# Ascend-Research/HeadPoseEstimation-WHENet

Hardware: AMD Instinct MI355X
Metric: head crops/sec (224x224) (higher is better)
Workload: dtype f16

## Files before the change

headposeestimation-whenet_amd/csrc/capi.cpp:

```cpp
#include <algorithm>
#include <chrono>
#include <cstdio>
#include <cstring>
#include <fstream>
#include <memory>
#include <mutex>
#include <new>
#include <exception>
#include <string>
#include <thread>
#include <utility>
#include <vector>

#include "engine.h"
#include "engine_internal.h"

constexpr int MAX_INFLIGHT_ENGINES = 4;
struct whenet_ctx {
    whenet::Engine* engine = nullptr;
    std::vector<whenet::Engine*> replicas;
    std::vector<char> snapshot;
    int device_id = 0, dtype = WHENET_F32;
    int inflight = 1;
    size_t next = 0;
    int fanout_min = 256, fanout_chunk = 128, fanout_stage = 2, fanout_depth = 2;
    int fanout_calib_calls = 0;
    double fanout_calib_rate[2] = {0.0, 0.0};
    int fanout_chosen = -1;
    std::vector<whenet::Engine*> fan;
    int fanout_engines = 2;
    std::vector<std::pair<std::string, long>> options;
    whenet::Engine& at(size_t i) { return i == 0 ? *engine : *replicas[i - 1]; }
    whenet::Engine& fan_at(size_t i) {
        if (i == 0) return *engine;
        if (i - 1 < replicas.size()) return *replicas[i - 1];
        return *fan[i - 1 - replicas.size()];
    }
    int fan_count() {
        const int want = std::max(inflight, std::min(fanout_engines, 4));
        while (1 + int(replicas.size()) + int(fan.size()) < want) {
            std::unique_ptr<whenet::Engine> r(new whenet::Engine(snapshot.data(), snapshot.size(), device_id, dtype));
            for (const auto& kv : options) r->set_option(kv.first, kv.second);
            fan.push_back(r.release());
        }
        return want;
    }
    whenet::Engine& take() {
        whenet::Engine& e = at(next % size_t(inflight));
        next = (next + 1) % size_t(inflight);
        return e;
    }
};

namespace {

thread_local std::string g_create_error;

struct HostRegistry {
    std::mutex mu;
    std::vector<std::pair<uintptr_t, uintptr_t>> held;
    bool acquire(const void* p, size_t nbytes, hipError_t* err) {
        const uintptr_t page = 4096, lo = reinterpret_cast<uintptr_t>(p) & ~(page - 1),
                        hi = (reinterpret_cast<uintptr_t>(p) + nbytes + page - 1) & ~(page - 1);
        std::lock_guard<std::mutex> lock(mu);
        for (const auto& r : held)
            if (lo < r.second && r.first < hi) {
                *err = hipErrorUnknown;
                return false;
            }
        *err = hipHostRegister(const_cast<void*>(p), nbytes, hipHostRegisterDefault);
        if (*err != hipSuccess) {
            (void)hipGetLastError();
            return false;
        }
        held.emplace_back(lo, hi);
        return true;
    }
    void release(const void* p, size_t nbytes) {
        const uintptr_t page = 4096, lo = reinterpret_cast<uintptr_t>(p) & ~(page - 1),
                        hi = (reinterpret_cast<uintptr_t>(p) + nbytes + page - 1) & ~(page - 1);
        std::lock_guard<std::mutex> lock(mu);
        (void)hipHostUnregister(const_cast<void*>(p));
        for (size_t i = 0; i < held.size(); ++i)
            if (held[i].first == lo && held[i].second == hi) {
                held.erase(held.begin() + long(i));
                break;
            }
    }
};
HostRegistry g_host_registry;

template <typename F>
int guarded(whenet_t* h, F&& fn) {
    if (h == nullptr || h->engine == nullptr) return WHENET_EINVAL;
    try {
        fn(*h->engine);
        return WHENET_OK;
    } catch (const whenet::Error& e) {
        h->engine->last_error = e.what();
        return e.code;
    } catch (const std::bad_alloc&) {
        h->engine->last_error = "out of host memory";
        return WHENET_ENOMEM;
    } catch (const std::exception& e) {
        h->engine->last_error = e.what();
        return WHENET_EHIP;
    } catch (...) {
        h->engine->last_error = "unknown error";
        return WHENET_EHIP;
    }
}

int create_impl(const void* blob, size_t nbytes, int device_id, int dtype, whenet_t** out) {
    if (out == nullptr) return WHENET_EINVAL;
    *out = nullptr;
    try {
        std::unique_ptr<whenet::Engine> e(new whenet::Engine(blob, nbytes, device_id, dtype));
        whenet_t* h = new whenet_t;
        h->engine = e.release();
        h->snapshot.assign(static_cast<const char*>(blob), static_cast<const char*>(blob) + nbytes);
        h->device_id = device_id;
        h->dtype = dtype;
        *out = h;
        return WHENET_OK;
    } catch (const whenet::Error& e) {
        g_create_error = e.what();
        return e.code;
    } catch (const std::bad_alloc&) {
        g_create_error = "out of host memory";
        return WHENET_ENOMEM;
    } catch (const std::exception& e) {
        g_create_error = e.what();
        return WHENET_EHIP;
    } catch (...) {
        g_create_error = "unknown error";
        return WHENET_EHIP;
    }
}

}

extern "C" {
#pragma GCC visibility push(default)

int whenet_create(const char* snapshot_path, int device_id, int dtype, whenet_t** out) {
    if (snapshot_path == nullptr || out == nullptr) {
        g_create_error = "whenet_create: NULL argument";
        return WHENET_EINVAL;
    }
    std::vector<char> blob;
    try {
        std::ifstream f(snapshot_path, std::ios::binary | std::ios::ate);
        if (!f) {
            g_create_error = std::string("cannot open snapshot '") + snapshot_path + "'";
            return WHENET_ENOENT;
        }
        const std::streamoff sz = f.tellg();
        if (sz < 0 || !f.seekg(0) || uint64_t(sz) > (uint64_t(1) << 32)) {
            g_create_error = std::string("snapshot '") + snapshot_path + "' is not a readable regular file";
            return WHENET_EIO;
        }
        blob.resize(size_t(sz));
        if (sz > 0 && !f.read(blob.data(), std::streamsize(sz))) {
            g_create_error = std::string("cannot read snapshot '") + snapshot_path + "'";
            return WHENET_EIO;
        }
    } catch (const std::bad_alloc&) {
        g_create_error = "out of host memory";
        return WHENET_ENOMEM;
    } catch (const std::exception& e) {
        g_create_error = std::string("cannot read snapshot '") + snapshot_path + "': " + e.what();
        return WHENET_EIO;
    } catch (...) {
        g_create_error = std::string("cannot read snapshot '") + snapshot_path + "'";
        return WHENET_EIO;
    }
    return create_impl(blob.data(), blob.size(), device_id, dtype, out);
}

int whenet_create_from_memory(const void* snapshot, size_t nbytes, int device_id, int dtype, whenet_t** out) {
    if (snapshot == nullptr || out == nullptr) {
        g_create_error = "whenet_create_from_memory: NULL argument";
        return WHENET_EINVAL;
    }
    return create_impl(snapshot, nbytes, device_id, dtype, out);
}

int whenet_create_postproc(int device_id, whenet_t** out) {
    if (out == nullptr) {
        g_create_error = "whenet_create_postproc: NULL argument";
        return WHENET_EINVAL;
    }
    *out = nullptr;
    try {
        std::unique_ptr<whenet::Engine> e(new whenet::Engine(device_id));
        whenet_t* h = new whenet_t;
        h->engine = e.release();
        h->device_id = device_id;
        *out = h;
        return WHENET_OK;
    } catch (const whenet::Error& e) {
        g_create_error = e.what();
        return e.code;
    } catch (const std::bad_alloc&) {
        g_create_error = "out of host memory";
        return WHENET_ENOMEM;
    } catch (const std::exception& e) {
        g_create_error = e.what();
        return WHENET_EHIP;
    } catch (...) {
        g_create_error = "unknown error";
        return WHENET_EHIP;
    }
}

void whenet_destroy(whenet_t* h) {
    if (h == nullptr) return;
    try {
        for (whenet::Engine* e : h->replicas) delete e;
        for (whenet::Engine* e : h->fan) delete e;
        delete h->engine;
    } catch (...) {
    }
    delete h;
}

const char* whenet_last_error(const whenet_t* h) {
    if (h == nullptr || h->engine == nullptr) return g_create_error.c_str();
    return h->engine->last_error.c_str();
}

int whenet_get_info(const whenet_t* h, whenet_info_t* out) {
    if (h == nullptr || h->engine == nullptr || out == nullptr) return WHENET_EINVAL;
    h->engine->get_info(out);
    return WHENET_OK;
}

int whenet_set_option(whenet_t* h, const char* key, long value) {
    if (key == nullptr) return WHENET_EINVAL;
    return guarded(h, [&](whenet::Engine& e) {
        const std::string k = key;
        if (k == "inflight") {
            WHENET_REQUIRE(value >= 1 && value <= MAX_INFLIGHT_ENGINES, WHENET_EINVAL, "inflight must be 1..4");
            WHENET_REQUIRE(!h->snapshot.empty() || value == 1, WHENET_EINVAL, "inflight: this handle has no network");
            e.release_aux_streams();
            for (whenet::Engine* r : h->replicas) r->release_aux_streams();
            for (whenet::Engine* r : h->fan) delete r;
            h->fan.clear();
            while (int(h->replicas.size()) + 1 > value) {
                delete h->replicas.back();
                h->replicas.pop_back();
            }
            while (int(h->replicas.size()) + 1 < value) {
                std::unique_ptr<whenet::Engine> r(
                    new whenet::Engine(h->snapshot.data(), h->snapshot.size(), h->device_id, h->dtype));
                for (const auto& kv : h->options) r->set_option(kv.first, kv.second);
                h->replicas.push_back(r.release());
            }
            h->inflight = int(value);
            h->next = 0;
            const long lanes = value > 1 ? 1 : 2;
            e.set_option("device_lanes", lanes);
            for (whenet::Engine* r : h->replicas) r->set_option("device_lanes", lanes);
            e.set_option("concurrent", value > 1);
            for (whenet::Engine* r : h->replicas) r->set_option("concurrent", value > 1);
            return;
        }
        if (k == "fanout_min" || k == "fanout_chunk" || k == "fanout_stage" || k == "fanout_depth" || k == "fanout_engines") {
            if (k == "fanout_engines") {
                WHENET_REQUIRE(value >= 1 && value <= MAX_INFLIGHT_ENGINES, WHENET_EINVAL, "fanout_engines must be 1..4");
                h->fanout_engines = int(value);
                for (whenet::Engine* r : h->fan) delete r;
                h->fan.clear();
                return;
            }
            if (k == "fanout_min") {
                WHENET_REQUIRE(value >= 0, WHENET_EINVAL, "fanout_min must be >= 0 (0 = never)");
                h->fanout_min = int(std::min<long>(value, 1 << 30));
            } else if (k == "fanout_chunk") {
                WHENET_REQUIRE(value >= 1 && value <= 4096, WHENET_EINVAL, "fanout_chunk must be 1..4096");
                h->fanout_chunk = int(value);
            } else if (k == "fanout_stage") {
                WHENET_REQUIRE(value >= -1 && value <= 3, WHENET_EINVAL,
                               "fanout_stage must be -1 (calibrate 0 against 1), 0 (pinned staging), 1 (the runtime's pageable path) or 2 (registered, default)");
                h->fanout_stage = int(value);
                h->fanout_calib_calls = 0;
                h->fanout_calib_rate[0] = h->fanout_calib_rate[1] = 0.0;
            } else {
                WHENET_REQUIRE(value >= 1 && value <= WHENET_MAX_INFLIGHT, WHENET_EINVAL, "fanout_depth must be 1..4");
                h->fanout_depth = int(value);
            }
            return;
        }
        e.set_option(k, value);
        for (whenet::Engine* r : h->replicas) r->set_option(k, value);
        for (whenet::Engine* r : h->fan) r->set_option(k, value);
        h->options.emplace_back(k, value);
    });
}

int whenet_forward_u8(whenet_t* h, const uint8_t* crops, int n, float* ypr, int32_t* argmax, float* logits) {
    return guarded(h, [&](whenet::Engine& e) {
        bool pending = e.has_pending();
        for (whenet::Engine* r : h->replicas) pending = pending || r->has_pending();
        if (h->fanout_min <= 0 || n < h->fanout_min || n <= h->fanout_chunk || pending || h->snapshot.empty()) {
            e.forward_host(crops, n, ypr, argmax, logits);
            return;
        }
        WHENET_REQUIRE(crops != nullptr && ypr != nullptr, WHENET_EINVAL, "crops and ypr must not be NULL");
        const int chunk = h->fanout_chunk;
        int stage = h->fanout_stage;
        const bool calibrating = stage < 0;
        if (calibrating)
            stage = h->fanout_calib_calls < 6 ? 1 - (h->fanout_calib_calls & 1) : (h->fanout_calib_rate[1] >= h->fanout_calib_rate[0] ? 1 : 0);
        const auto t_start = std::chrono::steady_clock::now();
        const int nfan = h->fan_count();
        const int lanes = nfan > 1 ? 1 : 2;
        if (stage == 2 || stage == 3) {
            const bool shared_copy_stream = stage == 2;
            whenet::detail::DeviceGuard guard(h->device_id);
            const size_t nbytes = size_t(n) * 150528;
            hipError_t re = hipSuccess;
            const bool registered = g_host_registry.acquire(crops, nbytes, &re);
            if (registered || re == hipErrorHostMemoryAlreadyRegistered) {
                h->fanout_chosen = stage;
                struct Pending { int eng, ticket, off; };
                std::vector<Pending> q;
                size_t head = 0;
                std::vector<int> outstanding(size_t(nfan), 0);
                const hipStream_t copy_on = shared_copy_stream ? h->engine->copy_stream_handle() : nullptr;
                hipEvent_t prev = nullptr;
                auto collect_head = [&] {
                    const Pending& p = q[head++];
                    const size_t o = size_t(p.off);
                    h->fan_at(size_t(p.eng)).collect(p.ticket, ypr + o * 3, argmax ? argmax + o * 3 : nullptr, logits ? logits + o * 252 : nullptr);
                    --outstanding[size_t(p.eng)];
                };
                std::exception_ptr err;
                try {
                    int off = 0, c = 0;
                    while (off < n) {
                        const int want = c < 2 && chunk >= 32 ? chunk / 2 : chunk;
                        const int cnt = std::min(want, n - off), ei = c % nfan;
                        while (outstanding[size_t(ei)] >= h->fanout_depth) collect_head();
                        whenet::Engine& eng = h->fan_at(size_t(ei));
                        const int ticket = eng.submit(crops + size_t(off) * 150528, cnt, 1, lanes, copy_on, shared_copy_stream ? nullptr : prev);
                        if (!shared_copy_stream) prev = eng.copied_event(ticket);
                        q.push_back(Pending{ei, ticket, off});
                        ++outstanding[size_t(ei)];
                        off += cnt;
                        ++c;
                    }
                    while (head < q.size()) collect_head();
                } catch (...) {
                    err = std::current_exception();
                    for (int i = 0; i < nfan; ++i) {
                        try { h->fan_at(size_t(i)).abandon_submissions(); } catch (...) {}
                    }
                }
                if (registered) g_host_registry.release(crops, nbytes);
                if (err) std::rethrow_exception(err);
                return;
            }
            stage = 1;
        }
        h->fanout_chosen = stage;
        const int nthreads = nfan;
        const int nchunks = (n + chunk - 1) / chunk;
        std::vector<std::exception_ptr> errs;
        errs.resize(static_cast<size_t>(nthreads));
        auto drive = [&](int t) {
            whenet::Engine& eng = h->fan_at(size_t(t));
            struct Pending { int ticket, off; };
            std::vector<Pending> q;
            size_t head = 0;
            auto collect_one = [&] {
                const Pending& p = q[head++];
                const size_t o = size_t(p.off);
                eng.collect(p.ticket, ypr + o * 3, argmax ? argmax + o * 3 : nullptr, logits ? logits + o * 252 : nullptr);
            };
            try {
                for (int c = t; c < nchunks; c += nthreads) {
                    if (q.size() - head >= size_t(h->fanout_depth)) collect_one();
                    const int off = c * chunk, cnt = std::min(chunk, n - off);
                    q.push_back(Pending{eng.submit(crops + size_t(off) * 150528, cnt, stage, lanes), off});
                }
                while (head < q.size()) collect_one();
            } catch (...) {
                errs[size_t(t)] = std::current_exception();
                try {
                    eng.abandon_submissions();
                } catch (...) {
                }
            }
        };
        std::vector<std::thread> workers;
        workers.reserve(size_t(nthreads));
        int started = 1;
        try {
            for (int t = 1; t < nthreads; ++t, ++started) workers.emplace_back(drive, t);
        } catch (...) {
        }
        drive(0);
        for (int t = started; t < nthreads; ++t) drive(t);
        for (std::thread& w : workers) w.join();
        for (const std::exception_ptr& ep : errs)
            if (ep) std::rethrow_exception(ep);
        if (calibrating && h->fanout_calib_calls < 6) {
            if (h->fanout_calib_calls >= 2) {
                const double sec = std::chrono::duration<double>(std::chrono::steady_clock::now() - t_start).count();
                h->fanout_calib_rate[stage] = std::max(h->fanout_calib_rate[stage], double(n) / (sec > 0 ? sec : 1e-9));
            }
            ++h->fanout_calib_calls;
        }
    });
}

int whenet_forward_f32(whenet_t* h, const float* image, int n, float* ypr, int32_t* argmax, float* logits) {
    return guarded(h, [&](whenet::Engine& e) { e.forward_host_f32(image, n, ypr, argmax, logits); });
}

int whenet_forward_u8_device(whenet_t* h, const uint8_t* d_crops, int n, float* d_ypr, int32_t* d_argmax,
                             float* d_logits, void* stream) {
    return guarded(h, [&](whenet::Engine& e) {
        whenet::Engine& eng = (stream != nullptr) ? e : h->take();
        eng.forward_device(d_crops, n, d_ypr, d_argmax, d_logits, static_cast<hipStream_t>(stream));
    });
}

int whenet_sync(whenet_t* h) {
    return guarded(h, [&](whenet::Engine& e) {
        e.sync();
        for (whenet::Engine* r : h->replicas) r->sync();
        for (whenet::Engine* r : h->fan) r->sync();
    });
}

int whenet_submit_u8(whenet_t* h, const uint8_t* crops, int n, int* ticket) {
    if (ticket == nullptr) return WHENET_EINVAL;
    return guarded(h, [&](whenet::Engine&) {
        const size_t idx = h->next % size_t(h->inflight);
        *ticket = h->take().submit(crops, n) * MAX_INFLIGHT_ENGINES + int(idx);
    });
}

int whenet_frame_rects(int frame_h, int frame_w, const float* bboxes, int k, int32_t* rects) {
    if (frame_h <= 0 || frame_w <= 0 || k < 0 || (k > 0 && (bboxes == nullptr || rects == nullptr))) return WHENET_EINVAL;
    for (int i = 0; i < k; ++i) whenet::frame_box_rect(frame_h, frame_w, bboxes + 4 * i, rects + 4 * i);
    return WHENET_OK;
}

int whenet_normalise_table(float lut[768]) {
    if (lut == nullptr) return WHENET_EINVAL;
    whenet::normalise_table(reinterpret_cast<float (*)[256]>(lut));
    return WHENET_OK;
}

int whenet_submit_frame(whenet_t* h, const uint8_t* frame, int frame_h, int frame_w, int channel_order,
                        const int32_t* rects, int k, int* ticket) {
    if (ticket == nullptr || (channel_order != WHENET_RGB && channel_order != WHENET_BGR)) return WHENET_EINVAL;
    return guarded(h, [&](whenet::Engine&) {
        const size_t idx = h->next % size_t(h->inflight);
        *ticket = h->take().submit_frame(frame, frame_h, frame_w, channel_order == WHENET_BGR, rects, k) *
                      MAX_INFLIGHT_ENGINES + int(idx);
    });
}

int whenet_op_crop_resize(whenet_t* h, const uint8_t* frame, int frame_h, int frame_w, int channel_order,
                          const int32_t* rects, int k, uint8_t* crops) {
    if (channel_order != WHENET_RGB && channel_order != WHENET_BGR) return WHENET_EINVAL;
    return guarded(h, [&](whenet::Engine& e) {
        e.op_crop_resize(frame, frame_h, frame_w, channel_order == WHENET_BGR, rects, k, crops);
    });
}

int whenet_yolo_eval(whenet_t* h, const float* const* feats, const int* grid_h, const int* grid_w, int num_layers,
                     const float* anchors, int num_anchors, int num_classes, float image_h, float image_w,
                     float score_threshold, float iou_threshold, int max_boxes, float* boxes, float* scores,
                     int32_t* classes, int32_t* index, int* count, float* all_boxes, float* all_scores) {
    if (count == nullptr) return WHENET_EINVAL;
    return guarded(h, [&](whenet::Engine& e) {
        *count = e.yolo_eval(feats, grid_h, grid_w, num_layers, anchors, num_anchors, num_classes, image_h, image_w,
                             score_threshold, iou_threshold, max_boxes, boxes, scores, classes, index, all_boxes,
                             all_scores);
    });
}

int whenet_collect(whenet_t* h, int ticket, float* ypr, int32_t* argmax, float* logits) {
    return guarded(h, [&](whenet::Engine&) {
        const int idx = ticket % MAX_INFLIGHT_ENGINES;
        WHENET_REQUIRE(ticket >= 0 && idx < h->inflight, WHENET_EINVAL, "unknown ticket " + std::to_string(ticket));
        h->at(size_t(idx)).collect(ticket / MAX_INFLIGHT_ENGINES, ypr, argmax, logits);
    });
}

int whenet_profile(whenet_t* h, const uint8_t* d_crops, int n, int iters, whenet_launch_stat_t* stats, int cap,
                   int* count) {
    return guarded(h, [&](whenet::Engine& e) {
        for (whenet::Engine* r : h->replicas) r->sync();
        const int c = e.profile(d_crops, n, iters, stats, cap);
        if (count) *count = c;
    });
}

int whenet_op_stem(whenet_t* h, const uint8_t* crops, int n, float* out) {
    return guarded(h, [&](whenet::Engine& e) { e.op_stem(crops, n, out); });
}

int whenet_op_block(whenet_t* h, int index, const float* in, int n, float* expand_out, float* dw_out, float* gate,
                    float* out) {
    return guarded(h, [&](whenet::Engine& e) { e.op_block(index, in, n, expand_out, dw_out, gate, out); });
}

int whenet_op_block_range(whenet_t* h, int first, int last, const float* in, int n, float* out) {
    return guarded(h, [&](whenet::Engine& e) { e.op_block_range(first, last, in, n, out); });
}

int whenet_op_head(whenet_t* h, const float* in, int n, float* feat, float* logits, float* ypr, int32_t* argmax) {
    return guarded(h, [&](whenet::Engine& e) { e.op_head(in, n, feat, logits, ypr, argmax); });
}

int whenet_op_decode(whenet_t* h, const float* logits, int n, float* ypr, int32_t* argmax) {
    return guarded(h, [&](whenet::Engine& e) { e.op_decode(logits, n, ypr, argmax); });
}

int whenet_block_spec(int index, int32_t out[8]) {
    if (out == nullptr) return WHENET_EINVAL;
    try {
        const auto blocks = whenet::make_blocks();
        if (index < 1 || index > int(blocks.size())) return WHENET_EINVAL;
        const whenet::BlockSpec& b = blocks[size_t(index - 1)];
        const int32_t v[8] = {b.k, b.s, b.expand, b.cin, b.cout, b.h_in, b.h_out, b.se_reduced()};
        std::memcpy(out, v, sizeof(v));
        return WHENET_OK;
    } catch (...) {
        return WHENET_ENOMEM;
    }
}

int whenet_dw_plan(int dtype, int index, int32_t out[12]) {
    if (out == nullptr || (dtype != WHENET_F32 && dtype != WHENET_F16)) return WHENET_EINVAL;
    try {
        const auto blocks = whenet::make_blocks();
        if (index < 1 || index > int(blocks.size())) return WHENET_EINVAL;
        const whenet::BlockSpec& b = blocks[size_t(index - 1)];
        const whenet::DwPlan p = whenet::plan_dw(dtype, b.k, b.s, b.h_in, b.h_out, b.cexp());
        const int32_t v[12] = {p.threads, p.CV, p.TH, p.NSX, p.tiles_x, p.tiles_y, p.chunks, p.IH, p.IW,
                               int32_t(p.lds_bytes), b.pad_before(), b.cexp()};
        std::memcpy(out, v, sizeof(v));
        return WHENET_OK;
    } catch (...) {
        return WHENET_EINVAL;
    }
}

int whenet_front_plan(int dtype, int index, int32_t out[12]) {
    if (out == nullptr || (dtype != WHENET_F32 && dtype != WHENET_F16)) return WHENET_EINVAL;
    try {
        const auto blocks = whenet::make_blocks();
        if (index < 2 || index > int(blocks.size())) return WHENET_EINVAL;
        const whenet::BlockSpec& b = blocks[size_t(index - 1)];
        const whenet::FrontPlan p = whenet::plan_front(dtype, b.k, b.s, b.h_in, b.h_out, b.cexp());
        const int32_t v[12] = {p.threads, p.CC, p.TH, p.NSX, p.tiles_x, p.tiles_y, p.chunks, p.EH, p.EW,
                               int32_t(p.lds_bytes), p.w_off, b.cexp()};
        std::memcpy(out, v, sizeof(v));
        return WHENET_OK;
    } catch (...) {
        return WHENET_EINVAL;
    }
}

int whenet_device_alloc(whenet_t* h, size_t nbytes, void** d_ptr) {
    if (d_ptr == nullptr) return WHENET_EINVAL;
    return guarded(h, [&](whenet::Engine& e) { *d_ptr = e.dev_alloc(nbytes); });
}

int whenet_device_free(whenet_t* h, void* d_ptr) {
    return guarded(h, [&](whenet::Engine& e) { e.dev_free(d_ptr); });
}

int whenet_memcpy_h2d(whenet_t* h, void* d_dst, const void* src, size_t nbytes) {
    return guarded(h, [&](whenet::Engine& e) { e.h2d(d_dst, src, nbytes); });
}

int whenet_memcpy_d2h(whenet_t* h, void* dst, const void* d_src, size_t nbytes) {
    return guarded(h, [&](whenet::Engine& e) { e.d2h(dst, d_src, nbytes); });
}
// ... 4 lines not shown
```

headposeestimation-whenet_amd/csrc/engine.cpp:

```cpp
#include "engine_internal.h"

#include <mutex>

#include <algorithm>
#include <cstdlib>
#include <cmath>
#include <cstring>

namespace whenet {

using namespace detail;

void* Engine::upload_bytes(const void* p, size_t nbytes) {
    void* d = nullptr;
    WHENET_HIP_CHECK(hipMalloc(&d, nbytes ? nbytes : 16));
    weight_allocs_.push_back(d);
    if (nbytes) WHENET_HIP_CHECK(hipMemcpy(d, p, nbytes, hipMemcpyHostToDevice));
    return d;
}

template <typename T> T* Engine::upload(const std::vector<T>& v) {
    return static_cast<T*>(upload_bytes(v.data(), v.size() * sizeof(T)));
}

DevPw Engine::upload_pw(const HostPw& h) {
    DevPw d;
    d.K = h.K;
    d.N = h.N;
    d.KS = h.KS;
    d.NTILES = h.NTILES;
    d.wp = upload_bytes(h.packed.data(), h.packed.size());
    if (!h.packed_split.empty()) {
        d.wps = upload_bytes(h.packed_split.data(), h.packed_split.size());
        d.KSs = h.KS_split;
        d.wsi = h.wsi;
    }
    d.wdense = upload(h.dense);
    d.bias = upload(h.bias);
    return d;
}

Engine::Engine(const void* snapshot, size_t nbytes, int device_id, int dtype)
    : device_(device_id), dtype_(dtype == WHENET_F32S ? WHENET_F32 : dtype), split_(dtype == WHENET_F32S) {
    HostModel m = build_host_model(parse_snapshot(snapshot, nbytes), dtype_, split_);
    params_backbone_ = m.params_backbone;
    params_heads_ = m.params_heads;
    n_tensors_ = m.n_tensors;

    open_device(device_id);
    DeviceGuard guard(device_);
    has_model_ = true;

    d_lut_ = static_cast<float*>(upload_bytes(&m.lut[0][0], sizeof(m.lut)));
    d_stem_w_ = upload(m.stem_w);
    d_stem_b_ = upload(m.stem_b);
    {
        StemDwTable t;
        build_stemdw_table(m.stem_w.data(), &m.lut[0][0], &t);
        d_stemdw_tab_ = static_cast<StemDwTable*>(upload_bytes(&t, sizeof(t)));
    }
    for (const HostBlock& hb : m.blocks) {
        DevBlock b;
        b.spec = hb.spec;
        if (hb.spec.has_expand()) b.expand = upload_pw(hb.expand);
        b.dw.k = hb.dw.k;
        b.dw.C = hb.dw.C;
        b.dw.w = upload(hb.dw.w);
        b.dw.bias = upload(hb.dw.bias);
        b.dw.plan = plan_dw(dtype_, hb.spec.k, hb.spec.s, hb.spec.h_in, hb.spec.h_out, hb.dw.C);
        b.se.C = hb.se.C;
        b.se.R = hb.se.R;
        b.se.w1t = upload(hb.se.w1t);
        b.se.b1 = upload(hb.se.b1);
        b.se.w2 = upload(hb.se.w2);
        b.se.w2c = upload(hb.se.w2c);
        b.se.b2 = upload(hb.se.b2);
        if (split_ && !hb.se.excite.packed_split.empty()) {
            b.se.w2p = upload_bytes(hb.se.excite.packed_split.data(), hb.se.excite.packed_split.size());
            b.se.KSr = hb.se.excite.KS_split;
            b.se.w2_wsi = hb.se.excite.wsi;
        } else if (dtype_ == WHENET_F16 && !hb.se.excite.packed.empty()) {
            b.se.w2p = upload_bytes(hb.se.excite.packed.data(), hb.se.excite.packed.size());
            b.se.KSr = hb.se.excite.KS;
        }
        b.project = upload_pw(hb.project);
        partial_per_crop_ = std::max(partial_per_crop_, size_t(b.dw.plan.ntiles()) * b.dw.C);
        if (hb.spec.has_expand()) {
            b.fplan = plan_front(dtype_, hb.spec.k, hb.spec.s, hb.spec.h_in, hb.spec.h_out, hb.dw.C);
            partial_per_crop_ = std::max(partial_per_crop_, size_t(b.fplan.ntiles()) * b.dw.C);
            partial_per_crop_ = std::max(partial_per_crop_, size_t(b.fplan.ntiles()) * size_t(b.fplan.chunks) *
                                                                size_t(se_padded_r(b.se.R)));
            if (dtype_ == WHENET_F16) {
                b.f2plan = plan_front2(hb.spec.k, hb.spec.s, hb.spec.h_in, hb.spec.h_out, hb.dw.C);
                b.f2_preferred = front2_preferred(hb.spec.k, hb.spec.s, hb.spec.h_in, hb.dw.C);
                b.dw.wt = upload(pack_dw_toeplitz(hb.dw.w, hb.spec.k, hb.spec.s, hb.dw.C, b.f2plan.xs));
                partial_per_crop_ = std::max(partial_per_crop_, size_t(b.f2plan.ntiles()) * b.dw.C);
                partial_per_crop_ = std::max(partial_per_crop_, size_t(b.f2plan.ntiles()) * size_t(b.f2plan.chunks) *
                                                                    size_t(se_padded_r(b.se.R)));
            }
            if (split_ && front2s_supported(hb.spec.k, hb.spec.s, hb.spec.h_in, hb.spec.cin)) {
                b.f2s_supported = true;
                b.f2splan = plan_front2s(hb.spec.k, hb.spec.s, hb.spec.h_in, hb.spec.h_out, hb.dw.C, &b.f2s_tm);
                b.f2s_preferred = front2s_preferred(hb.spec.k, hb.spec.s, hb.spec.h_in, hb.dw.C);
                b.dw.wts = upload(pack_dw_toeplitz_s(hb.dw.w, hb.spec.k, hb.spec.s, hb.dw.C, b.f2s_tm, &b.dw.wts_wsi));
                partial_per_crop_ = std::max(partial_per_crop_, size_t(b.f2splan.ntiles()) * size_t(b.f2splan.chunks) *
                                                                    size_t(se_padded_r(b.se.R)));
            }
            b.f7_supported = front7_supported(hb.spec.k, hb.spec.s, hb.spec.h_in, hb.spec.cin);
            if (b.f7_supported) {
                if (dtype_ == WHENET_F16) b.dw.wt7 = upload(pack_dw_toeplitz(hb.dw.w, hb.spec.k, 1, hb.dw.C, 4 - hb.spec.k / 2));
                b.f7_chunks = front7_plan_for(dtype_, hb.spec.cin, hb.dw.C, 64).chunks;
                partial_per_crop_ = std::max(partial_per_crop_, size_t(b.f7_chunks) * size_t(se_padded_r(b.se.R)));
            }
        }
        if (mb7_supported(dtype_, hb.spec.k, hb.spec.s, hb.spec.h_in, hb.spec.cin, hb.dw.C, hb.se.R, hb.spec.cout, hb.spec.has_skip())) {
            std::vector<half_t> w1p, w2p;
            pack_mb7_se(hb.se.w1t, hb.se.w2, hb.se.C, hb.se.R, &w1p, &w2p);
            b.mb7.wds = upload(pack_mb7_taps(hb.dw.w, hb.spec.k, hb.dw.C));
            b.mb7.w1p = upload(w1p);
            b.mb7.w2p = upload(w2p);
            b.mb7.ok = true;
        }
        blocks_.push_back(b);
    }
    head_ = upload_pw(m.head);
    fold12_pw_ = upload_pw(m.fold12);
    d_fold12_w32_ = upload(m.fold12_w32);
    d_dense_w_ = upload(m.dense_w);
    d_dense_b_ = upload(m.dense_b);
    WHENET_HIP_CHECK(hipDeviceSynchronize());
}

void Engine::open_device(int device_id) {
    int count = 0;
    hipError_t e = hipGetDeviceCount(&count);
    if (e != hipSuccess || count <= 0)
        throw Error(WHENET_ENODEV, std::string("no HIP device visible (") + hipGetErrorString(e) +
                                       "); libwhenet_hip has no CPU fallback");
    WHENET_REQUIRE(device_id >= 0 && device_id < count, WHENET_ENODEV,
                   "device_id " + std::to_string(device_id) + " out of range (" + std::to_string(count) + " devices)");
    DeviceGuard guard(device_id);
    WHENET_HIP_CHECK(hipGetDeviceProperties(&prop_, device_id));
    WHENET_REQUIRE(std::strstr(prop_.gcnArchName, "gfx950") != nullptr, WHENET_ENODEV,
                   std::string("device is ") + prop_.gcnArchName + "; this library carries gfx950 code only");
    num_cus_ = prop_.multiProcessorCount;

    WHENET_HIP_CHECK(hipStreamCreateWithFlags(&stream_, hipStreamNonBlocking));
    WHENET_HIP_CHECK(hipEventCreateWithFlags(&fork_ev_, hipEventDisableTiming));
    for (int i = 0; i < MAX_LANES - 1; ++i) {
        hipEvent_t ev = nullptr;
        WHENET_HIP_CHECK(hipEventCreateWithFlags(&ev, hipEventDisableTiming));
        join_ev_.push_back(ev);
    }
}

Engine::Engine(int device_id) : device_(device_id), dtype_(WHENET_F32) { open_device(device_id); }

void Engine::require_model() const {
    WHENET_REQUIRE(has_model_, WHENET_EINVAL, "this handle was created without a network (whenet_create_postproc)");
}

Engine::~Engine() {
    (void)hipSetDevice(device_);
    if (stream_) (void)hipStreamSynchronize(stream_);
    if (copy_stream_) (void)hipStreamSynchronize(copy_stream_);
    for (auto& kv : graphs_) (void)hipGraphExecDestroy(kv.second);
    graphs_.clear();
    auto free_slot_buffers = [](Slot& s) {
        if (s.h_in) (void)hipHostFree(s.h_in);
        if (s.h_ypr) (void)hipHostFree(s.h_ypr);
        if (s.h_amax) (void)hipHostFree(s.h_amax);
        if (s.h_logits) (void)hipHostFree(s.h_logits);
        if (s.d_in) (void)hipFree(s.d_in);
        if (s.d_ypr) (void)hipFree(s.d_ypr);
        if (s.d_amax) (void)hipFree(s.d_amax);
        if (s.d_logits) (void)hipFree(s.d_logits);
        if (s.h_frame) (void)hipHostFree(s.h_frame);
        if (s.d_frame) (void)hipFree(s.d_frame);
        if (s.h_plan) (void)hipHostFree(s.h_plan);
        if (s.d_plan) (void)hipFree(s.d_plan);
        if (s.copied) (void)hipEventDestroy(s.copied);
        if (s.done) (void)hipEventDestroy(s.done);
    };
    for (Slot& s : slots_) free_slot_buffers(s);
    free_slot_buffers(host_slot_);
    if (hout_ypr_) (void)hipHostFree(hout_ypr_);
    if (hout_amax_) (void)hipHostFree(hout_amax_);
    if (hout_logits_) (void)hipHostFree(hout_logits_);
    void* arena[] = {x0_, x1_, e_, d_, hc_, partial_, gate_, hcount_, in_u8_, o_ypr_, o_amax_, o_logits_, in_f32_, yolo_scratch_};
    for (void* p : arena)
        if (p) (void)hipFree(p);
    for (void* p : weight_allocs_) (void)hipFree(p);
    for (hipStream_t st : lane_streams_) { (void)hipStreamSynchronize(st); (void)hipStreamDestroy(st); }
    for (hipEvent_t ev : join_ev_) (void)hipEventDestroy(ev);
    if (fork_ev_) (void)hipEventDestroy(fork_ev_);
    if (stream_) (void)hipStreamDestroy(stream_);
    if (copy_stream_) (void)hipStreamDestroy(copy_stream_);
}

void Engine::set_option(const std::string& key, long value) {
    DeviceGuard guard(device_);
    if (key == "graph") {
        use_graph_ = value != 0;
    } else if (key == "pw_impl") {
        WHENET_REQUIRE(value == 0 || value == 1, WHENET_EINVAL, "pw_impl must be 0 (MFMA) or 1 (check kernel)");
        pw_impl_ = int(value);
        sync();
        drop_graphs();
    } else if (key == "fuse_front") {
        fuse_front_ = value != 0;
        sync();
        drop_graphs();
    } else if (key == "se_fuse") {
        WHENET_REQUIRE(value >= 0 && value <= 3, WHENET_EINVAL,
                       "se_fuse must be 0 (never), 1 (where the prologue form pays), 2 (prologue form on every block) or 3 (1 + the matrix-core form on blocks 7-16, default)");
        se_fuse_ = int(value);
        sync();
        drop_graphs();
    } else if (key == "front_impl") {
        WHENET_REQUIRE(value >= 0 && value <= 2, WHENET_EINVAL,
                       "front_impl must be 0 (front.hip everywhere), 1 (per layer, default) or 2 (front2.hip / front2s.hip wherever they exist)");
        front_impl_ = int(value);
        sync();
        drop_graphs();
    } else if (key == "f2s_mask") {
        WHENET_REQUIRE(value >= -1 && value < (1 << 17), WHENET_EINVAL, "f2s_mask must be -1 or a bit mask of blocks 2..12");
        f2s_mask_ = int(value);
        sync();
        drop_graphs();
    } else if (key == "head_fuse") {
        head_fuse_ = value != 0;
        sync();
        drop_graphs();
    } else if (key == "concurrent") {
        xcd_always_ = value != 0;
        sync();
        drop_graphs();
    } else if (key == "xcd_map") {
        WHENET_REQUIRE(value >= 0 && value <= 7, WHENET_EINVAL, "xcd_map must be a bit mask 0..7 (1 = front / front2, 2 = front7, 4 = head7)");
        xcd_map_ = int(value);
        sync();
        drop_graphs();
    } else if (key == "mb7") {
        mb7_ = value != 0;
        sync();
        drop_graphs();
    } else if (key == "front7") {
        front7_ = value != 0;
        sync();
        drop_graphs();
    } else if (key == "fold12") {
        fold12_ = value != 0;
        sync();
        drop_graphs();
    } else if (key == "stem_fuse") {
        stem_fuse_ = value != 0;
        sync();
        drop_graphs();
    } else if (key == "poison") {
        poison_ = value != 0;
    } else if (key == "lanes" || key == "device_lanes") {
        WHENET_REQUIRE(value >= 1 && value <= MAX_LANES, WHENET_EINVAL, "lanes must be 1..8");
        lanes_ = int(value);
        if (key == "lanes") host_lanes_ = int(value);
        sync();
        drop_graphs();
    } else if (key == "split_heads") {
        split_heads_ = value != 0;
        sync();
        drop_graphs();
    } else if (key == "lane_graphs") {
        lane_graphs_ = value != 0;
        sync();
        drop_graphs();
    } else if (key == "pw_staged") {
        pw_staged_ = value != 0;
        sync();
        drop_graphs();
    } else if (key == "split_pw") {
        WHENET_REQUIRE(split_ || value == 0, WHENET_EINVAL, "split_pw: the handle was not created as WHENET_F32S");
        split_pw_ = value != 0;
        sync();
        drop_graphs();
    } else if (key == "host_pinned_max") {
        WHENET_REQUIRE(value >= 0 && value <= 4096, WHENET_EINVAL, "host_pinned_max must be 0..4096");
        sync();
        host_pinned_max_ = int(value);
    } else if (key == "se_fuse_tiny") {
        WHENET_REQUIRE(value >= 0 && value <= 64, WHENET_EINVAL, "se_fuse_tiny must be 0..64");
        se_fuse_tiny_ = int(value);
        sync();
        drop_graphs();
    } else if (key == "host_lanes") {
        WHENET_REQUIRE(value >= 1 && value <= MAX_LANES, WHENET_EINVAL, "host_lanes must be 1..8");
        host_lanes_ = int(value);
    } else if (key == "min_lane_crops") {
        WHENET_REQUIRE(value >= 1, WHENET_EINVAL, "min_lane_crops must be >= 1");
        min_lane_crops_ = int(value);
        sync();
        drop_graphs();
    } else if (key == "repeat") {
        WHENET_REQUIRE(value >= 1 && value <= 16, WHENET_EINVAL, "repeat must be 1..16");
        repeat_ = int(value);
        sync();
        drop_graphs();
    } else {
        throw Error(WHENET_EINVAL, "unknown option '" + key + "'");
    }
}

void Engine::get_info(whenet_info_t* out) const {
    std::memset(out, 0, sizeof(*out));
    out->abi_version = WHENET_ABI_VERSION;
    out->dtype = dtype_;
    out->device_id = device_;
    out->compute_units = num_cus_;
    out->params_backbone = params_backbone_;
    out->params_heads = params_heads_;
    out->n_tensors = n_tensors_;
    {
        int k = 1 + 2;
        for (const DevBlock& b : blocks_) {
            const BlockSchedule bs = block_schedule(b);
            if (bs.use_mb7) { k += 1; continue; }
            k += bs.fused ? 1 : (b.spec.has_expand() ? 2 : 1);
            k += bs.se_fused ? 1 : 2;
        }
        if (fold12_active()) k -= 1;
        if (stem_fuse_active()) k -= 1;
        out->n_kernels_per_forward = k;
    }
    out->macs_per_crop = 384857312;
    out->arena_bytes = int64_t(arena_bytes_);
    out->capacity = cap_;
    out->graph_enabled = use_graph_ ? 1 : 0;
    copy_name(out->device_name, sizeof(out->device_name), prop_.name);
    copy_name(out->arch, sizeof(out->arch), prop_.gcnArchName);
}

void Engine::drop_graphs() {
    for (auto& kv : graphs_) (void)hipGraphExecDestroy(kv.second);
    graphs_.clear();
}

void Engine::release_arena() {
    void** arena[] = {&x0_, &x1_, &e_, &d_, &hc_, reinterpret_cast<void**>(&partial_), reinterpret_cast<void**>(&gate_), reinterpret_cast<void**>(&hcount_),
                      reinterpret_cast<void**>(&in_u8_), reinterpret_cast<void**>(&o_ypr_),
                      reinterpret_cast<void**>(&o_amax_), reinterpret_cast<void**>(&o_logits_)};
    for (void** p : arena) {
        if (*p) (void)hipFree(*p);
        *p = nullptr;
    }
    cap_ = 0;
    arena_bytes_ = 0;
}

void Engine::ensure_capacity(int n) {
    WHENET_REQUIRE(n >= 1, WHENET_EINVAL, "n must be >= 1");
    if (n <= cap_) return;
    WHENET_HIP_CHECK(hipStreamSynchronize(stream_));
    drop_graphs();
    release_arena();
    const size_t N = size_t(n), es = esz();
    size_t total = 0;
    auto alloc = [&](size_t bytes) {
        void* p = nullptr;
        hipError_t e = hipMalloc(&p, bytes);
        if (e != hipSuccess) {
            release_arena();
            throw Error(WHENET_ENOMEM, "activation arena for n=" + std::to_string(n) + ": " + hipGetErrorString(e));
        }
        total += bytes;
        return p;
    };
    x0_ = alloc(N * X_ELEMS * es);
    x1_ = alloc(N * X_ELEMS * es);
    e_ = alloc(N * E_ELEMS * es);
    d_ = alloc(N * D_ELEMS * es);
    hc_ = alloc(N * HC_ELEMS * es);
    partial_ = static_cast<float*>(alloc(N * partial_per_crop_ * sizeof(float)));
    gate_ = static_cast<float*>(alloc(N * 1152 * sizeof(float)));
    hcount_ = static_cast<unsigned*>(alloc(N * sizeof(unsigned)));
    WHENET_HIP_CHECK(hipMemsetAsync(hcount_, 0, N * sizeof(unsigned), stream_));
    WHENET_HIP_CHECK(hipStreamSynchronize(stream_));
    in_u8_ = static_cast<uint8_t*>(alloc(N * IN_BYTES));
    o_ypr_ = static_cast<float*>(alloc(N * 3 * sizeof(float)));
    o_amax_ = static_cast<int32_t*>(alloc(N * 3 * sizeof(int32_t)));
    o_logits_ = static_cast<float*>(alloc(N * N_LOGITS * sizeof(float)));
    cap_ = n;
    arena_bytes_ = total;
}

namespace {

struct Rec {
    LaunchRecorder* rec;
    hipStream_t s;
    int repeat = 1;
    template <typename F>
    void operator()(const std::string& layer, const char* kind, const std::string& kernel, double bytes, double flops,
                    F&& fn) {
        if (!rec) {
            for (int i = 0; i < repeat; ++i) fn();
            return;
        }
        if (rec->first_pass) {
            LaunchRecorder::Entry e;
            e.layer = layer;
            e.kind = kind;
            e.kernel = kernel;
            e.bytes = bytes;
            e.flops = flops;
            WHENET_HIP_CHECK(hipEventCreate(&e.stop));
            rec->entries.push_back(e);
        }
        LaunchRecorder::Entry& e = rec->entries.at(rec->cursor++);
        fn();
        WHENET_HIP_CHECK(hipEventRecord(e.stop, s));
    }
};

}

Engine::BlockSchedule Engine::block_schedule(const DevBlock& b, int n) const {
    BlockSchedule r;
    r.fused = fuse_front_ && b.spec.has_expand() && pw_impl_ == 0;
    r.use_f7 = r.fused && front_impl_ == 1 && front7_ && b.f7_supported;
    r.use_mb7 = r.use_f7 && mb7_ && dtype_ == WHENET_F16 && b.mb7.ok;
    r.use_f2 = r.fused && !r.use_f7 && dtype_ == WHENET_F16 && (front_impl_ == 2 || (front_impl_ == 1 && b.f2_preferred));
    const bool f2s_pick = f2s_mask_ >= 0 ? ((f2s_mask_ >> b.spec.index) & 1) != 0 : b.f2s_preferred;
    r.use_f2s = r.fused && !r.use_f7 && split_ && split_pw_ && b.f2s_supported && b.expand.wps != nullptr &&
                (front_impl_ == 2 || (front_impl_ == 1 && f2s_pick));
    r.se_in_front = r.fused;
    r.se_ntiles = r.use_f7 ? 1 : (r.use_f2 ? b.f2plan.ntiles() : (r.use_f2s ? b.f2splan.ntiles() : (r.fused ? b.fplan.ntiles() : b.dw.plan.ntiles())));
    r.se_chunks = r.use_f7 ? b.f7_chunks : (r.use_f2 ? b.f2plan.chunks : (r.use_f2s ? b.f2splan.chunks : b.fplan.chunks));
    const bool se_pays = b.project.K < 320 && r.se_ntiles * r.se_chunks <= 24;
    const bool tiny = !single_stage_call_ && n > 0 && n <= se_fuse_tiny_ && b.project.K < 1152;
    r.se_mfma = r.se_in_front && pw_impl_ == 0 && se_fuse_ == 3 && pw_staged_ && b.project.K >= 320 && b.se.w2p != nullptr &&
                (dtype_ == WHENET_F16 || (split_ && split_pw_));
    r.se_fused = r.se_in_front && pw_impl_ == 0 && (se_fuse_ == 2 || r.se_mfma || ((se_fuse_ == 1 || se_fuse_ == 3) && (se_pays || tiny)));
    return r;
}

bool Engine::fold12_active() const {
    if (!(fold12_ && fuse_front_ && pw_impl_ == 0 && blocks_.size() >= 2)) return false;
    if (dtype_ == WHENET_F16) return front_impl_ == 2 || (front_impl_ == 1 && blocks_[1].f2_preferred);
    const BlockSchedule b2 = block_schedule(blocks_[1]);
    return split_ && split_pw_ && fold12_pw_.wps != nullptr && b2.fused && !b2.use_f2s && !b2.use_f7;
}

bool Engine::stem_fuse_active() const {
    if (!(stem_fuse_ && !blocks_.empty())) return false;
    const DevBlock& b = blocks_[0];
    return !b.spec.has_expand() && !b.spec.has_skip() &&
           stemdw_supported(dtype_, b.dw.plan, b.spec.k, b.spec.s, b.spec.h_in, b.spec.cexp());
}

void* Engine::enqueue_blocks(int first, int last, const View& v, void* cur, int n, hipStream_t s, LaunchRecorder* rec,
                             bool b1_dw_done) {
    const bool fold = fold12_active() && first <= 1 && last >= 2;
    for (int i = first; i <= last; ++i) {
        void* nxt = (cur == v.x0) ? v.x1 : v.x0;
        enqueue_block(blocks_[size_t(i - 1)], v, cur, nxt, n, s, rec, fold && i <= 2 ? i : 0, b1_dw_done && i == 1);
        cur = nxt;
    }
    return cur;
}

void Engine::enqueue_block(const DevBlock& b, const View& v, const void* in, void* out, int n, hipStream_t s,
                           LaunchRecorder* rec, int fold, bool dw_done) {
    Rec R{rec, s, repeat_};
    const BlockSpec& sp = b.spec;
    const std::string p = "b" + std::to_string(sp.index);
    const double es = double(esz());
    const int hw_in = sp.h_in * sp.h_in, hw_out = sp.h_out * sp.h_out;
    const int cexp = sp.cexp();
    const void* dw_in = in;
    const BlockSchedule bs = block_schedule(b, n);
    const bool fused = bs.fused, use_f2 = bs.use_f2, se_in_front = bs.se_in_front, se_fused = bs.se_fused;
    const int se_ntiles = bs.se_ntiles, se_chunks = bs.se_chunks;
    WHENET_REQUIRE(fold == 0 || (fold == 1 && !fused && sp.index == 1) ||
                       (fold == 2 && sp.index == 2 && (use_f2 || (split_ && fused && !bs.use_f2s && !bs.use_f7))), WHENET_EINVAL,
                   "fold12: block outside the folded pair");
    if (bs.use_mb7) {
        WHENET_REQUIRE(fold == 0, WHENET_EINVAL, "mb7: block outside the 7 x 7 stage");
        Mb7Args a{};
        a.x = in;
        a.wep = b.expand.wp;
        a.be = b.expand.bias;
        a.wds = b.mb7.wds;
        a.bd = b.dw.bias;
        a.w1p = b.mb7.w1p;
        a.b1 = b.se.b1;
        a.w2p = b.mb7.w2p;
        a.b2 = b.se.b2;
        a.wpp = b.project.wp;
        a.bp = b.project.bias;
        a.out = out;
        if (single_stage_call_) {
            a.dbg_dw = v.d;
            a.dbg_gate = v.gate;
        }
        a.k = sp.k;
        a.Cout = sp.cout;
        a.skip = sp.has_skip();
        a.n = n;
        R(p + "/mbconv", "mbconv", kernel_name_mb7(sp.k, sp.cout, a.skip).c_str(),
          double(n) * (hw_in * sp.cin * (a.skip ? 2 : 1) + hw_out * sp.cout) * es,
          2.0 * n * (double(hw_in) * sp.cin * cexp + double(hw_out) * sp.k * sp.k * cexp + double(hw_out) * cexp * sp.cout),
          [&] { launch_mb7(a, s); });
        return;
    }
    if (bs.use_f7) {
        Front7Args a{};
        a.dtype = dtype_;
        a.x = in;
        a.wep = b.expand.wp;
        a.be = b.expand.bias;
        a.wdt = dtype_ == WHENET_F16 ? static_cast<const void*>(b.dw.wt7) : static_cast<const void*>(b.dw.w);
        a.bd = b.dw.bias;
        a.out = v.d;
        a.rpart = v.partial;
        a.w1t = b.se.w1t;
        a.R = b.se.R;
        a.k = sp.k;
        a.Cin = sp.cin;
        a.Cexp = cexp;
        a.NTe = b.expand.NTILES;
        a.split = split_ && split_pw_ && b.expand.wps != nullptr;
        a.weps = b.expand.wps;
        a.wsi = b.expand.wsi;
        a.n = n;
        a.xcd_grouped = xcd_grouped(2, n);
        a.plan = front7_plan_for(dtype_, sp.cin, cexp, n);
        R(p + "/front", "front", kernel_name_front7(dtype_, sp.k, a.plan, a.split).c_str(), double(n) * (hw_in * sp.cin + hw_out * cexp) * es,
          2.0 * n * (double(hw_in) * sp.cin * cexp + double(hw_out) * sp.k * sp.k * cexp), [&] { launch_front7(a, s); });
    } else if (use_f2) {
        Front2Args a{};
        a.x = in;
        a.wep = b.expand.wp;
        a.be = b.expand.bias;
        a.wdt = b.dw.wt;
        a.bd = b.dw.bias;
        a.out = v.d;
        a.rpart = v.partial;
        a.w1t = b.se.w1t;
        a.R = b.se.R;
        a.k = sp.k;
        a.s = sp.s;
        a.H = sp.h_in;
        a.Ho = sp.h_out;
        a.Cin = sp.cin;
        a.Cexp = cexp;
        a.pad = sp.pad_before();
        a.KSe = b.expand.KS;
        a.NTe = b.expand.NTILES;
        if (fold == 2) {
            a.wep = d_fold12_w32_;
            a.be = fold12_pw_.bias;
            a.Cin = fold12_pw_.K;
            a.KSe = fold12_pw_.KS;
            a.NTe = fold12_pw_.NTILES;
            a.in_gate = static_cast<const float*>(v.gate);
        }
        a.n = n;
        a.xcd_grouped = xcd_grouped(1, n);
        a.plan = b.f2plan;
        a.plan.threads = front2_threads(b.f2plan, n);
        R(p + "/front", "front", kernel_name_front2(sp.k, sp.s, a.KSe, a.plan.threads, a.plan.xs, a.in_gate != nullptr).c_str(),
          double(n) * (hw_in * a.Cin + hw_out * cexp) * es,
          2.0 * n * (double(hw_in) * a.Cin * cexp + double(hw_out) * sp.k * sp.k * cexp), [&] { launch_front2(a, s); });
    } else if (bs.use_f2s) {
        Front2sArgs a{};
        a.x = in;
        a.weps = b.expand.wps;
        a.be = b.expand.bias;
        a.wdt = b.dw.wts;
        a.bd = b.dw.bias;
        a.out = v.d;
        a.rpart = v.partial;
        a.w1t = b.se.w1t;
        a.R = b.se.R;
        a.k = sp.k;
        a.s = sp.s;
        a.H = sp.h_in;
        a.Ho = sp.h_out;
        a.Cin = sp.cin;
        a.Cexp = cexp;
        a.pad = sp.pad_before();
        a.KSe = b.expand.KSs;
        a.NTe = b.expand.NTILES;
        a.wsi = b.expand.wsi;
        a.wsi_d = b.dw.wts_wsi;
        a.tm = b.f2s_tm;
        a.n = n;
        a.plan = b.f2splan;
        R(p + "/front", "front", kernel_name_front2s(sp.k, sp.s, a.KSe, a.plan.threads, a.tm, false).c_str(),
          double(n) * (hw_in * sp.cin + hw_out * cexp) * es,
          2.0 * n * (double(hw_in) * sp.cin * cexp + double(hw_out) * sp.k * sp.k * cexp), [&] { launch_front2s(a, s); });
    } else if (fused) {
        FrontArgs a{};
        a.x = in;
        a.wep = b.expand.wp;
        a.be = b.expand.bias;
        a.wd = b.dw.w;
        a.bd = b.dw.bias;
        a.out = v.d;
        a.rpart = v.partial;
        a.w1t = b.se.w1t;
        a.R = b.se.R;
        a.k = sp.k;
        a.s = sp.s;
        a.H = sp.h_in;
        a.Ho = sp.h_out;
        a.Cin = sp.cin;
        a.Cexp = cexp;
        a.pad = sp.pad_before();
        a.KSe = b.expand.KS;
        a.NTe = b.expand.NTILES;
        a.split = split_ && split_pw_ && b.expand.wps != nullptr;
        a.weps = b.expand.wps;
        a.KSes = b.expand.KSs;
        a.wsi = b.expand.wsi;
        if (fold == 2) {
            a.weps = fold12_pw_.wps;
            a.be = fold12_pw_.bias;
            a.Cin = fold12_pw_.K;
            a.KSe = fold12_pw_.KS;
            a.KSes = fold12_pw_.KSs;
            a.NTe = fold12_pw_.NTILES;
            a.wsi = fold12_pw_.wsi;
            a.in_gate = static_cast<const float*>(v.gate);
        }
        a.n = n;
        a.xcd_grouped = xcd_grouped(1, n);
        a.plan = b.fplan;
        a.plan.threads = front_threads(b.fplan, n);
        R(p + "/front", "front", kernel_name_front(dtype_, sp.k, sp.s, a.plan.threads).c_str(), double(n) * (hw_in * a.Cin + hw_out * cexp) * es,
          2.0 * n * (double(hw_in) * a.Cin * cexp + double(hw_out) * sp.k * sp.k * cexp),
          [&] { launch_front(a, dtype_, s); });
    } else if (sp.has_expand()) {
        PwArgs a{};
        a.a = in;
        a.wp = b.expand.wp;
        a.wdense = b.expand.wdense;
        a.bias = b.expand.bias;
        a.out = v.e;
        a.M = n * hw_in;
        a.K = b.expand.K;
        a.N = b.expand.N;
        a.KS = b.expand.KS;
        a.NTILES = b.expand.NTILES;
        set_split(a, b.expand);
        a.HW = hw_in;
        a.act = ACT_SWISH;
        R(p + "/expand", "pw", kernel_name_pw(a, dtype_, pw_impl_, num_cus_).c_str(), double(a.M) * (a.K + a.N) * es,
          2.0 * a.M * a.K * a.N, [&] { launch_pw(a, dtype_, pw_impl_, num_cus_, s); });
        dw_in = v.e;
    }
    if (!fused && !dw_done) {
        DwArgs a{};
        a.in = dw_in;
        a.out = fold == 1 ? out : v.d;
        a.w = b.dw.w;
        a.bias = b.dw.bias;
        a.partial = v.partial;
        a.k = sp.k;
        a.s = sp.s;
        a.H = sp.h_in;
        a.Ho = sp.h_out;
        a.C = cexp;
        a.pad = sp.pad_before();
        a.n = n;
        a.plan = b.dw.plan;
        R(p + "/dw", "dw", kernel_name_dw(dtype_, sp.k, sp.s), double(n) * (hw_in + hw_out) * cexp * es,
          2.0 * n * hw_out * sp.k * sp.k * cexp, [&] { launch_dw(a, dtype_, s); });
    }
    SeFuse sef{};
    if (se_fused) {
        sef.rpart = v.partial;
        sef.b1 = b.se.b1;
        sef.w2c = b.se.w2c;
        sef.b2 = b.se.b2;
        sef.np = se_ntiles * se_chunks;
        sef.R = b.se.R;
        sef.RP = se_padded_r(b.se.R);
        sef.inv_hw = 1.0f / float(hw_out);
        if (bs.se_mfma) {
            sef.w2p = b.se.w2p;
            sef.KSr = b.se.KSr;
            sef.w2_wsi = b.se.w2_wsi;
        }
    } else if (se_in_front) {
        SeExciteArgs a{};
        a.rpart = v.partial;
        a.np = se_ntiles * se_chunks;
        a.inv_hw = 1.0f / float(hw_out);
        a.b1 = b.se.b1;
        a.w2c = b.se.w2c;
        a.b2 = b.se.b2;
        a.gate = v.gate;
        a.gate_f16 = dtype_ == WHENET_F16;
        a.C = b.se.C;
        a.R = b.se.R;
        a.n = n;
        R(p + "/se", "se", ("whenet_se_excite_kernel<" + std::to_string(se_padded_r(a.R)) + ">").c_str(),
          double(n) * (a.np * se_padded_r(a.R) + a.C) * 4.0 + double(a.C) * se_padded_r(a.R) * 4.0, 2.0 * n * a.C * a.R,
          [&] { launch_se_excite(a, s); });
    } else {
        SeArgs a{};
        a.partial = v.partial;
        a.ntiles = se_ntiles;
        a.inv_hw = 1.0f / float(hw_out);
        a.w1t = b.se.w1t;
        a.b1 = b.se.b1;
        a.w2c = b.se.w2c;
        a.b2 = b.se.b2;
        a.gate = v.gate;
        a.gate_f16 = dtype_ == WHENET_F16 && fold != 1;
        a.C = b.se.C;
        a.R = b.se.R;
        a.n = n;
        R(p + "/se", "se", ("whenet_se_kernel<" + std::to_string(se_padded_r(a.R)) + ">").c_str(), double(n) * (a.ntiles + 1) * a.C * 4.0 + 2.0 * a.C * a.R * 4.0,
          4.0 * n * a.C * a.R, [&] { launch_se(a, s); });
    }
    if (fold != 1) {
        PwArgs a{};
        a.a = v.d;
        a.wp = b.project.wp;
        a.wdense = b.project.wdense;
        a.bias = b.project.bias;
        a.gate = se_fused ? nullptr : v.gate;
        a.se = sef;
        a.res = sp.has_skip() ? in : nullptr;
        a.out = out;
        a.M = n * hw_out;
        a.K = b.project.K;
        a.N = b.project.N;
        a.KS = b.project.KS;
        a.NTILES = b.project.NTILES;
        set_split(a, b.project);
        a.HW = hw_out;
        a.act = ACT_NONE;
        R(p + "/project", "pw", kernel_name_pw(a, dtype_, pw_impl_, num_cus_).c_str(),
          double(a.M) * (a.K + a.N + (sp.has_skip() ? a.N : 0)) * es, 2.0 * a.M * a.K * a.N,
          [&] { launch_pw(a, dtype_, pw_impl_, num_cus_, s); });
    }
}

void Engine::enqueue_forward(const View& v, const uint8_t* d_in, int n, float* d_ypr, int32_t* d_amax, float* d_logits,
                             hipStream_t s, LaunchRecorder* rec, const float* d_in_f32) {
    Rec R{rec, s, repeat_};
    const double es = double(esz());
    const bool stemdw = stem_fuse_active() && d_in_f32 == nullptr;
    if (stemdw) {
        const DevBlock& b1 = blocks_[0];
        const bool fold = fold12_active() && blocks_.size() >= 2;
        StemDwArgs a{};
        a.dtype = dtype_;
        a.w = d_stem_w_;
        a.lut = d_lut_;
        a.in = d_in;
        a.out = fold ? v.x1 : v.d;
        a.tab = d_stemdw_tab_;
        a.bias = d_stem_b_;
        a.wd = b1.dw.w;
        a.bd = b1.dw.bias;
        a.partial = v.partial;
        a.n = n;
        R("stem+b1/dw", "stem", kernel_name_stemdw(dtype_), double(n) * (IN_BYTES + X_ELEMS * es), 2.0 * n * (10838016.0 + 112.0 * 112 * 9 * 32),
          [&] { launch_stemdw(a, s); });
    } else {
        StemArgs a{d_in, v.x0, d_stem_w_, d_stem_b_, d_lut_, n};
        a.in_f32 = d_in_f32;
        R("stem", "stem", kernel_name_stem(dtype_), double(n) * (IN_BYTES + X_ELEMS * es), 2.0 * n * 10838016.0,
          [&] { launch_stem(a, dtype_, s); });
    }
    void* cur = enqueue_blocks(1, int(blocks_.size()), v, v.x0, n, s, rec, stemdw);
    const bool fuse_head = head_fuse_ && pw_impl_ == 0 && split_heads_ && head7_supported(dtype_, head_.K, head_.N, 49) &&
                           partial_per_crop_ >= size_t(heads_split()) * N_LOGITS;
    if (fuse_head) {
        Head7Args a{};
        a.dtype = dtype_;
        a.x = cur;
        a.wep = head_.wp;
        a.bias = head_.bias;
        a.feat = reinterpret_cast<float*>(v.hc);
        a.K = head_.K;
        a.N = head_.N;
        a.NTILES = head_.NTILES;
        a.split = split_ && split_pw_ && head_.wps != nullptr;
        a.weps = head_.wps;
        a.wsi = head_.wsi;
        a.n = n;
        a.xcd_grouped = xcd_grouped(4, n);
        R("head", "pw", kernel_name_head7(dtype_, n, a.split).c_str(), double(n) * (49.0 * a.K * es + a.N * 4.0), 2.0 * n * 49.0 * a.K * a.N,
          [&] { launch_head7(a, s); });
        HeadsArgs hargs{};
        hargs.feat_in = reinterpret_cast<const float*>(v.hc);
        hargs.w = d_dense_w_;
        hargs.b = d_dense_b_;
        hargs.logits = d_logits;
        hargs.ypr = d_ypr;
        hargs.argmax = d_amax;
        hargs.n = n;
        R("heads", "heads", "whenet_heads_split_kernel<float, true>", double(n) * ((FEAT + N_LOGITS + 6) * 4.0) + double(FEAT) * N_LOGITS * 4.0,
          2.0 * n * FEAT * N_LOGITS, [&] { launch_heads_split(hargs, v.partial, v.hcount, dtype_, s); });
        return;
    }
    {
        PwArgs a{};
        a.a = cur;
        a.wp = head_.wp;
        a.wdense = head_.wdense;
        a.bias = head_.bias;
        a.out = v.hc;
        a.M = n * 49;
        a.K = head_.K;
        a.N = head_.N;
        a.KS = head_.KS;
        a.NTILES = head_.NTILES;
        set_split(a, head_);
        a.HW = 49;
        a.act = ACT_SWISH;
        R("head", "pw", kernel_name_pw(a, dtype_, pw_impl_, num_cus_).c_str(), double(a.M) * (a.K + a.N) * es,
          2.0 * a.M * a.K * a.N, [&] { launch_pw(a, dtype_, pw_impl_, num_cus_, s); });
    }
    {
        HeadsArgs a{};
        a.x = v.hc;
        a.w = d_dense_w_;
        a.b = d_dense_b_;
        a.logits = d_logits;
        a.ypr = d_ypr;
        a.argmax = d_amax;
        a.n = n;
        const bool split = split_heads_ && partial_per_crop_ >= size_t(heads_split()) * N_LOGITS;
        const std::string hname = std::string(split ? "whenet_heads_split_kernel<" : "whenet_heads_kernel<") +
                                  (dtype_ == WHENET_F16 ? "_Float16" : "float") + (split ? ", false>" : ">");
        R("heads", "heads", hname.c_str(),
          double(n) * (HC_ELEMS * es + (N_LOGITS + 6) * 4.0) + double(FEAT) * N_LOGITS * 4.0, 2.0 * n * FEAT * N_LOGITS,
          [&] {
              if (split) launch_heads_split(a, v.partial, v.hcount, dtype_, s);
              else launch_heads(a, dtype_, s);
          });
    }
}

hipStream_t Engine::lane_stream(int i) {
    while (int(lane_streams_.size()) <= i) {
        hipStream_t st = nullptr;
        WHENET_HIP_CHECK(hipStreamCreateWithFlags(&st, hipStreamNonBlocking));
        lane_streams_.push_back(st);
    }
    return lane_streams_[size_t(i)];
}

void Engine::release_aux_streams() {
    DeviceGuard guard(device_);
    sync();
    drop_graphs();
    for (hipStream_t st : lane_streams_) (void)hipStreamDestroy(st);
    lane_streams_.clear();
    if (copy_stream_) (void)hipStreamDestroy(copy_stream_);
    copy_stream_ = nullptr;
}

hipStream_t Engine::copy_stream() {
    if (!copy_stream_) WHENET_HIP_CHECK(hipStreamCreateWithFlags(&copy_stream_, hipStreamNonBlocking));
    return copy_stream_;
}

Engine::View Engine::view(int crop_off) const {
    const size_t o = size_t(crop_off), es = esz();
    View v;
    v.x0 = static_cast<char*>(x0_) + o * X_ELEMS * es;
    v.x1 = static_cast<char*>(x1_) + o * X_ELEMS * es;
    v.e = static_cast<char*>(e_) + o * E_ELEMS * es;
    v.d = static_cast<char*>(d_) + o * D_ELEMS * es;
    v.hc = static_cast<char*>(hc_) + o * HC_ELEMS * es;
    v.partial = partial_ + o * partial_per_crop_;
    v.hcount = hcount_ + o;
    v.gate = gate_ + o * 1152;
    return v;
}

int Engine::lanes_for(int n, int want) const {
    int lanes = want > 0 ? std::min(want, MAX_LANES) : lanes_;
    while (lanes > 1 && n / lanes < min_lane_crops_) --lanes;
    return lanes;
}

void Engine::enqueue_lanes(const uint8_t* d_in, int n, float* d_ypr, int32_t* d_amax, float* d_logits, hipStream_t s, int want) {
    const int lanes = lanes_for(n, want);
    if (lanes <= 1) {
        enqueue_forward(view(0), d_in, n, d_ypr, d_amax, d_logits, s, nullptr);
        return;
    }
    WHENET_HIP_CHECK(hipEventRecord(fork_ev_, s));
    int off = 0;
    for (int i = 0; i < lanes; ++i) {
        const int cnt = n / lanes + (i < n % lanes ? 1 : 0);
        hipStream_t st = (i == 0) ? s : lane_stream(i - 1);
        if (i > 0) WHENET_HIP_CHECK(hipStreamWaitEvent(st, fork_ev_, 0));
        enqueue_forward(view(off), d_in + size_t(off) * IN_BYTES, cnt, d_ypr + size_t(off) * 3,
                        d_amax ? d_amax + size_t(off) * 3 : nullptr, d_logits ? d_logits + size_t(off) * N_LOGITS : nullptr,
                        st, nullptr);
        if (i > 0) {
            WHENET_HIP_CHECK(hipEventRecord(join_ev_[size_t(i - 1)], st));
            WHENET_HIP_CHECK(hipStreamWaitEvent(s, join_ev_[size_t(i - 1)], 0));
        }
        off += cnt;
    }
}

template <typename F>
hipGraphExec_t Engine::cached_graph(const GraphKey& key, hipStream_t s, F&& fn) {
    auto it = graphs_.find(key);
    if (it != graphs_.end()) return it->second;
    if (graphs_.size() >= size_t(MAX_GRAPHS)) {
        sync_streams(s);
        WHENET_HIP_CHECK(hipStreamSynchronize(stream_));
        drop_graphs();
    }
    hipGraph_t graph = nullptr;
    WHENET_HIP_CHECK(hipStreamBeginCapture(s, hipStreamCaptureModeRelaxed));
    try {
        fn();
    } catch (...) {
        (void)hipStreamEndCapture(s, &graph);
        if (graph) (void)hipGraphDestroy(graph);
        throw;
    }
    WHENET_HIP_CHECK(hipStreamEndCapture(s, &graph));
    hipGraphExec_t exec = nullptr;
    hipError_t e = hipGraphInstantiate(&exec, graph, nullptr, nullptr, 0);
    (void)hipGraphDestroy(graph);
    if (e != hipSuccess) throw Error(WHENET_EHIP, std::string("hipGraphInstantiate: ") + hipGetErrorString(e));
    graphs_.emplace(key, exec);
    return exec;
}

void Engine::poison_arena(int n, hipStream_t s) {
    const size_t N = size_t(n), es = esz();
    WHENET_HIP_CHECK(hipMemsetAsync(x0_, 0xff, N * X_ELEMS * es, s));
    WHENET_HIP_CHECK(hipMemsetAsync(x1_, 0xff, N * X_ELEMS * es, s));
    WHENET_HIP_CHECK(hipMemsetAsync(e_, 0xff, N * E_ELEMS * es, s));
    WHENET_HIP_CHECK(hipMemsetAsync(d_, 0xff, N * D_ELEMS * es, s));
    WHENET_HIP_CHECK(hipMemsetAsync(hc_, 0xff, N * HC_ELEMS * es, s));
    WHENET_HIP_CHECK(hipMemsetAsync(partial_, 0xff, N * partial_per_crop_ * sizeof(float), s));
    WHENET_HIP_CHECK(hipMemsetAsync(gate_, 0xff, N * 1152 * sizeof(float), s));
}

void Engine::run_forward(const uint8_t* d_in, int n, float* d_ypr, int32_t* d_amax, float* d_logits, hipStream_t s, int want) {
    if (poison_) poison_arena(n, s);
    if (!use_graph_) {
        enqueue_lanes(d_in, n, d_ypr, d_amax, d_logits, s, want);
        return;
    }
    const int lanes = lanes_for(n, want);
    if (lanes > 1) (void)lane_stream(lanes - 2);
    if (lane_graphs_ && lanes > 1) {
        WHENET_HIP_CHECK(hipEventRecord(fork_ev_, s));
        int off = 0;
        for (int i = 0; i < lanes; ++i) {
            const int cnt = n / lanes + (i < n % lanes ? 1 : 0);
            hipStream_t st = (i == 0) ? s : lane_stream(i - 1);
            const uint8_t* in_i = d_in + size_t(off) * IN_BYTES;
            float* ypr_i = d_ypr + size_t(off) * 3;
            int32_t* am_i = d_amax ? d_amax + size_t(off) * 3 : nullptr;
            float* lg_i = d_logits ? d_logits + size_t(off) * N_LOGITS : nullptr;
            hipGraphExec_t g = cached_graph(GraphKey{cnt, off, in_i, ypr_i, am_i, lg_i}, st, [&] {
                enqueue_forward(view(off), in_i, cnt, ypr_i, am_i, lg_i, st, nullptr);
            });
            if (i > 0) WHENET_HIP_CHECK(hipStreamWaitEvent(st, fork_ev_, 0));
            WHENET_HIP_CHECK(hipGraphLaunch(g, st));
            if (i > 0) {
                WHENET_HIP_CHECK(hipEventRecord(join_ev_[size_t(i - 1)], st));
                WHENET_HIP_CHECK(hipStreamWaitEvent(s, join_ev_[size_t(i - 1)], 0));
            }
            off += cnt;
        }
        return;
    }
    hipGraphExec_t g = cached_graph(GraphKey{n, -lanes, d_in, d_ypr, d_amax, d_logits}, s,
                                    [&] { enqueue_lanes(d_in, n, d_ypr, d_amax, d_logits, s, lanes); });
    WHENET_HIP_CHECK(hipGraphLaunch(g, s));
}

void Engine::forward_device(const uint8_t* d_crops, int n, float* d_ypr, int32_t* d_argmax, float* d_logits,
                            hipStream_t stream) {
    DeviceGuard guard(device_);
    require_model();
    WHENET_REQUIRE(d_crops != nullptr && d_ypr != nullptr, WHENET_EINVAL, "crops and ypr must not be NULL");
    WHENET_REQUIRE((reinterpret_cast<uintptr_t>(d_crops) & 3) == 0, WHENET_EINVAL, "crops must be 4-byte aligned");
    ensure_capacity(n);
    run_forward(d_crops, n, d_ypr, d_argmax, d_logits, stream ? stream : stream_);
}

void Engine::forward_host(const uint8_t* crops, int n, float* ypr, int32_t* argmax, float* logits) {
    DeviceGuard guard(device_);
    require_model();
    WHENET_REQUIRE(crops != nullptr && ypr != nullptr, WHENET_EINVAL, "crops and ypr must not be NULL");
    ensure_capacity(n);
    const size_t N = size_t(n);
    if (n <= host_pinned_max_) {
        Slot& sl = host_slot_;
        ensure_slot(sl, std::max(n, std::min(host_pinned_max_, 16)));
        std::memcpy(sl.h_in, crops, N * IN_BYTES);
        WHENET_HIP_CHECK(hipMemcpyAsync(sl.d_in, sl.h_in, N * IN_BYTES, hipMemcpyHostToDevice, stream_));
        run_forward(sl.d_in, n, sl.d_ypr, sl.d_amax, sl.d_logits, stream_, host_lanes_);
        WHENET_HIP_CHECK(hipMemcpyAsync(sl.h_ypr, sl.d_ypr, N * 3 * sizeof(float), hipMemcpyDeviceToHost, stream_));
        if (argmax) WHENET_HIP_CHECK(hipMemcpyAsync(sl.h_amax, sl.d_amax, N * 3 * sizeof(int32_t), hipMemcpyDeviceToHost, stream_));
        if (logits)
            WHENET_HIP_CHECK(hipMemcpyAsync(sl.h_logits, sl.d_logits, N * N_LOGITS * sizeof(float), hipMemcpyDeviceToHost, stream_));
        WHENET_HIP_CHECK(hipStreamSynchronize(stream_));
        std::memcpy(ypr, sl.h_ypr, N * 3 * sizeof(float));
        if (argmax) std::memcpy(argmax, sl.h_amax, N * 3 * sizeof(int32_t));
        if (logits) std::memcpy(logits, sl.h_logits, N * N_LOGITS * sizeof(float));
        return;
    }
    ensure_host_out(n);
    WHENET_HIP_CHECK(hipMemcpyAsync(in_u8_, crops, N * IN_BYTES, hipMemcpyHostToDevice, stream_));
    run_forward(in_u8_, n, o_ypr_, o_amax_, o_logits_, stream_, host_lanes_);
    WHENET_HIP_CHECK(hipMemcpyAsync(hout_ypr_, o_ypr_, N * 3 * sizeof(float), hipMemcpyDeviceToHost, stream_));
    if (argmax) WHENET_HIP_CHECK(hipMemcpyAsync(hout_amax_, o_amax_, N * 3 * sizeof(int32_t), hipMemcpyDeviceToHost, stream_));
    if (logits)
        WHENET_HIP_CHECK(hipMemcpyAsync(hout_logits_, o_logits_, N * N_LOGITS * sizeof(float), hipMemcpyDeviceToHost, stream_));
    WHENET_HIP_CHECK(hipStreamSynchronize(stream_));
    std::memcpy(ypr, hout_ypr_, N * 3 * sizeof(float));
    if (argmax) std::memcpy(argmax, hout_amax_, N * 3 * sizeof(int32_t));
    if (logits) std::memcpy(logits, hout_logits_, N * N_LOGITS * sizeof(float));
}

void Engine::ensure_host_out(int n) {
    if (n <= hout_cap_) return;
    static std::mutex mu;
    std::lock_guard<std::mutex> lock(mu);
    WHENET_HIP_CHECK(hipStreamSynchronize(stream_));
    if (hout_ypr_) (void)hipHostFree(hout_ypr_);
    if (hout_amax_) (void)hipHostFree(hout_amax_);
    if (hout_logits_) (void)hipHostFree(hout_logits_);
    hout_ypr_ = nullptr; hout_amax_ = nullptr; hout_logits_ = nullptr;
    hout_cap_ = 0;
    const size_t N = size_t(std::max(n, 256));
    WHENET_HIP_CHECK(hipHostMalloc(reinterpret_cast<void**>(&hout_ypr_), N * 3 * sizeof(float), hipHostMallocDefault));
    WHENET_HIP_CHECK(hipHostMalloc(reinterpret_cast<void**>(&hout_amax_), N * 3 * sizeof(int32_t), hipHostMallocDefault));
    WHENET_HIP_CHECK(hipHostMalloc(reinterpret_cast<void**>(&hout_logits_), N * N_LOGITS * sizeof(float), hipHostMallocDefault));
    hout_cap_ = int(N);
}

void Engine::forward_host_f32(const float* x, int n, float* ypr, int32_t* argmax, float* logits) {
    DeviceGuard guard(device_);
    require_model();
    WHENET_REQUIRE(x != nullptr && ypr != nullptr, WHENET_EINVAL, "image and ypr must not be NULL");
    ensure_capacity(n);
    const size_t N = size_t(n);
    if (n > in_f32_cap_) {
        WHENET_HIP_CHECK(hipStreamSynchronize(stream_));
        if (in_f32_) (void)hipFree(in_f32_);
        in_f32_ = nullptr;
        in_f32_cap_ = 0;
        hipError_t e = hipMalloc(reinterpret_cast<void**>(&in_f32_), N * IN_BYTES * sizeof(float));
        if (e != hipSuccess) throw Error(WHENET_ENOMEM, std::string("float input buffer: ") + hipGetErrorString(e));
        in_f32_cap_ = n;
    }
    if (poison_) {
        poison_arena(n, stream_);
        WHENET_HIP_CHECK(hipMemsetAsync(in_f32_, 0xff, size_t(in_f32_cap_) * IN_BYTES * sizeof(float), stream_));
    }
    WHENET_HIP_CHECK(hipMemcpyAsync(in_f32_, x, N * IN_BYTES * sizeof(float), hipMemcpyHostToDevice, stream_));
    enqueue_forward(view(0), nullptr, n, o_ypr_, o_amax_, o_logits_, stream_, nullptr, in_f32_);
    WHENET_HIP_CHECK(hipMemcpyAsync(ypr, o_ypr_, N * 3 * sizeof(float), hipMemcpyDeviceToHost, stream_));
    if (argmax) WHENET_HIP_CHECK(hipMemcpyAsync(argmax, o_amax_, N * 3 * sizeof(int32_t), hipMemcpyDeviceToHost, stream_));
    if (logits)
        WHENET_HIP_CHECK(hipMemcpyAsync(logits, o_logits_, N * N_LOGITS * sizeof(float), hipMemcpyDeviceToHost, stream_));
    WHENET_HIP_CHECK(hipStreamSynchronize(stream_));
}

void Engine::sync_streams(hipStream_t s) {
    WHENET_HIP_CHECK(hipStreamSynchronize(s));
    for (hipStream_t st : lane_streams_) WHENET_HIP_CHECK(hipStreamSynchronize(st));
}

void Engine::sync() {
    DeviceGuard guard(device_);
    WHENET_HIP_CHECK(hipStreamSynchronize(stream_));
    if (copy_stream_) WHENET_HIP_CHECK(hipStreamSynchronize(copy_stream_));
    for (hipStream_t st : lane_streams_) WHENET_HIP_CHECK(hipStreamSynchronize(st));
}

void Engine::ensure_slot(Slot& s, int n) {
    if (!s.copied) {
        WHENET_HIP_CHECK(hipEventCreateWithFlags(&s.copied, hipEventDisableTiming));
        WHENET_HIP_CHECK(hipEventCreateWithFlags(&s.done, hipEventDisableTiming));
    }
    if (n <= s.capacity) return;
    if (s.h_in) (void)hipHostFree(s.h_in);
// ... 165 lines not shown
```

headposeestimation-whenet_amd/csrc/engine.h:

```cpp
#pragma once

#include <map>
#include <memory>
#include <string>
#include <tuple>
#include <vector>

#include "common.h"
#include "kernels.h"
#include "snapshot.h"

namespace whenet {

struct DevPw {
    int K = 0, N = 0, KS = 0, NTILES = 0;
    void* wp = nullptr;
    void* wps = nullptr;
    int KSs = 0;
    float wsi = 1.0f;
    float* wdense = nullptr;
    float* bias = nullptr;
};
struct DevDw {
    int k = 0, C = 0;
    float* w = nullptr;
    float* bias = nullptr;
    half_t* wt = nullptr;
    half_t* wt7 = nullptr;
    float* wts = nullptr;
    float wts_wsi = 1.0f;
    DwPlan plan;
};
struct DevSe {
    int C = 0, R = 0;
    float *w1t = nullptr, *b1 = nullptr, *w2 = nullptr, *b2 = nullptr;
    float* w2c = nullptr;
    void* w2p = nullptr;
    int KSr = 0;
    float w2_wsi = 1.0f;
};
struct DevMb7 {
    bool ok = false;
    half_t *wds = nullptr, *w1p = nullptr, *w2p = nullptr;
};
struct DevBlock {
    BlockSpec spec;
    DevPw expand;
    DevDw dw;
    FrontPlan fplan;
    Front2Plan f2plan;
    bool f2_preferred = false;
    Front2Plan f2splan;
    int f2s_tm = 2;
    bool f2s_supported = false, f2s_preferred = false;
    bool f7_supported = false;
    int f7_chunks = 1;
    DevSe se;
    DevPw project;
    DevMb7 mb7;
};

struct LaunchRecorder {
    struct Entry {
        std::string layer, kind, kernel;
        double bytes = 0, flops = 0;
        hipEvent_t stop = nullptr;
        double total_ms = 0;
    };
    std::vector<Entry> entries;
    hipEvent_t start = nullptr;
    size_t cursor = 0;
    bool first_pass = true;
};

constexpr int MAX_LANES = 8;

class Engine {
  public:
    Engine(const void* snapshot, size_t nbytes, int device_id, int dtype);
    explicit Engine(int device_id);
    ~Engine();
    Engine(const Engine&) = delete;
    Engine& operator=(const Engine&) = delete;

    void set_option(const std::string& key, long value);
    void get_info(whenet_info_t* out) const;

    void forward_host(const uint8_t* crops, int n, float* ypr, int32_t* argmax, float* logits);
    void forward_host_f32(const float* x, int n, float* ypr, int32_t* argmax, float* logits);
    void forward_device(const uint8_t* d_crops, int n, float* d_ypr, int32_t* d_argmax, float* d_logits,
                        hipStream_t stream);
    void sync();
    void release_aux_streams();
    int submit(const uint8_t* crops, int n, int stage = 0, int want_lanes = 0, hipStream_t copy_on = nullptr, hipEvent_t copy_after = nullptr);
    hipStream_t copy_stream_handle();
    hipEvent_t copied_event(int ticket) const;
    void abandon_submissions();
    bool has_pending() const {
        for (const Slot& s : slots_)
            if (s.busy) return true;
        return false;
    }
    int submit_frame(const uint8_t* frame, int fh, int fw, int swap_rb, const int32_t* rects, int k);
    void op_crop_resize(const uint8_t* frame, int fh, int fw, int swap_rb, const int32_t* rects, int k,
                        uint8_t* crops_out);
    void collect(int ticket, float* ypr, int32_t* argmax, float* logits);
    int profile(const uint8_t* d_crops, int n, int iters, whenet_launch_stat_t* stats, int cap);

    void op_stem(const uint8_t* crops, int n, float* out);
    int yolo_eval(const float* const* feats, const int* grid_h, const int* grid_w, int num_layers, const float* anchors,
                  int num_anchors, int num_classes, float image_h, float image_w, float score_threshold,
                  float iou_threshold, int max_boxes, float* boxes, float* scores, int32_t* classes, int32_t* index,
                  float* all_boxes, float* all_scores);
    void op_block(int index, const float* in, int n, float* expand_out, float* dw_out, float* gate, float* out);
    void op_block_range(int first, int last, const float* in, int n, float* out);
    void op_head(const float* in, int n, float* feat, float* logits, float* ypr, int32_t* argmax);
    void op_decode(const float* logits, int n, float* ypr, int32_t* argmax);

    void* dev_alloc(size_t nbytes);
    void dev_free(void* p);
    void h2d(void* d, const void* s, size_t nbytes);
    void d2h(void* d, const void* s, size_t nbytes);

    std::string last_error;

  private:
    struct Slot {
        int capacity = 0, n = 0, ticket = -1;
        bool busy = false;
        uint8_t* h_in = nullptr;
        uint8_t* d_in = nullptr;
        float *h_ypr = nullptr, *d_ypr = nullptr;
        int32_t *h_amax = nullptr, *d_amax = nullptr;
        float *h_logits = nullptr, *d_logits = nullptr;
        hipEvent_t copied = nullptr, done = nullptr;
        size_t frame_cap = 0;
        uint8_t *h_frame = nullptr, *d_frame = nullptr;
        int plan_cap = 0;
        int32_t *h_plan = nullptr, *d_plan = nullptr;
    };

    template <typename T> T* upload(const std::vector<T>& v);
    void* upload_bytes(const void* p, size_t nbytes);
    DevPw upload_pw(const HostPw& h);
    void set_split(PwArgs& a, const DevPw& w) const {
        a.staged = pw_staged_;
        a.split = split_ && split_pw_ && w.wps != nullptr;
        a.wps = w.wps;
        a.KSs = w.KSs;
        a.wsi = w.wsi;
    }
    bool split_ = false;
    bool split_pw_ = true;
    bool pw_staged_ = true;
    void ensure_capacity(int n);
    void release_arena();
    void drop_graphs();
    size_t esz() const { return dtype_ == WHENET_F16 ? 2 : 4; }

    struct View {
        void *x0, *x1, *e, *d, *hc;
        float *partial, *gate;
        unsigned* hcount;
    };
    View view(int crop_off) const;
    void enqueue_forward(const View& v, const uint8_t* d_in, int n, float* d_ypr, int32_t* d_amax, float* d_logits,
                         hipStream_t s, LaunchRecorder* rec, const float* d_in_f32 = nullptr);
    void enqueue_block(const DevBlock& b, const View& v, const void* in, void* out, int n, hipStream_t s,
                       LaunchRecorder* rec, int fold = 0, bool dw_done = false);
    void* enqueue_blocks(int first, int last, const View& v, void* cur, int n, hipStream_t s, LaunchRecorder* rec,
                         bool b1_dw_done = false);
    bool stem_fuse_active() const;
    bool fold12_active() const;
    struct BlockSchedule {
        bool fused = false, use_f2 = false, use_f2s = false, use_f7 = false, se_in_front = false, se_fused = false, se_mfma = false;
        bool use_mb7 = false;
        int se_ntiles = 1, se_chunks = 1;
    };
    BlockSchedule block_schedule(const DevBlock& b, int n = 0) const;
    int se_fuse_tiny_ = 0;
    int f2s_mask_ = -1;
    bool single_stage_call_ = false;
    int lanes_for(int n, int want) const;
    void enqueue_lanes(const uint8_t* d_in, int n, float* d_ypr, int32_t* d_amax, float* d_logits, hipStream_t s, int want = 0);
    void run_forward(const uint8_t* d_in, int n, float* d_ypr, int32_t* d_amax, float* d_logits, hipStream_t s, int want = 0);
    void poison_arena(int n, hipStream_t s);
    void ensure_slot(Slot& s, int n);
    hipStream_t lane_stream(int i);
    using GraphKey = std::tuple<int, int, const void*, void*, void*, void*>;
    template <typename F>
    hipGraphExec_t cached_graph(const GraphKey& key, hipStream_t s, F&& fn);
    void sync_streams(hipStream_t s);
    hipStream_t copy_stream();
    void ensure_slot_frame(Slot& s, size_t frame_bytes, int k);
    Slot* free_slot();

    void open_device(int device_id);
    void require_model() const;
    bool has_model_ = false;
    int device_ = 0, dtype_ = WHENET_F32, num_cus_ = 256;
    bool use_graph_ = true;
    int pw_impl_ = 0;
    int repeat_ = 1;
    bool split_heads_ = true;
    bool fuse_front_ = true;
    int se_fuse_ = 1;
    int front_impl_ = 1;
    bool poison_ = false;
    bool head_fuse_ = true;
    bool front7_ = true;
    bool mb7_ = false;
    int xcd_map_ = 7;
    bool xcd_always_ = false;
    bool xcd_grouped(int bit, int n) const {
        return (xcd_map_ & bit) != 0 && (xcd_always_ || n >= 128);
    }
    bool stem_fuse_ = true;
    bool fold12_ = true;
    int lanes_ = 2;
    bool lane_graphs_ = false;
    int min_lane_crops_ = 16;
    int host_lanes_ = 2;
    std::vector<hipStream_t> lane_streams_;
    std::vector<hipEvent_t> join_ev_;
    hipEvent_t fork_ev_ = nullptr;
    hipStream_t stream_ = nullptr, copy_stream_ = nullptr;
    hipDeviceProp_t prop_{};
    int64_t params_backbone_ = 0, params_heads_ = 0;
    int n_tensors_ = 0;

    std::vector<void*> weight_allocs_;
    float *d_lut_ = nullptr, *d_stem_w_ = nullptr, *d_stem_b_ = nullptr;
    StemDwTable* d_stemdw_tab_ = nullptr;
    std::vector<DevBlock> blocks_;
    DevPw head_;
    DevPw fold12_pw_;
    float* d_fold12_w32_ = nullptr;
    float *d_dense_w_ = nullptr, *d_dense_b_ = nullptr;

    int cap_ = 0;
    size_t arena_bytes_ = 0;
    void *x0_ = nullptr, *x1_ = nullptr, *e_ = nullptr, *d_ = nullptr, *hc_ = nullptr;
    float *partial_ = nullptr, *gate_ = nullptr;
    unsigned* hcount_ = nullptr;
    uint8_t* in_u8_ = nullptr;
    float* in_f32_ = nullptr;
    int in_f32_cap_ = 0;
    float* o_ypr_ = nullptr;
    int32_t* o_amax_ = nullptr;
    float* o_logits_ = nullptr;
    size_t partial_per_crop_ = 0;
    unsigned char* yolo_scratch_ = nullptr;
    size_t yolo_scratch_bytes_ = 0;
    std::vector<int> yolo_counts_;

    std::map<GraphKey, hipGraphExec_t> graphs_;

    Slot slots_[WHENET_MAX_INFLIGHT];
    Slot host_slot_;
    float* hout_ypr_ = nullptr;
    int32_t* hout_amax_ = nullptr;
    float* hout_logits_ = nullptr;
    int hout_cap_ = 0;
    void ensure_host_out(int n);
    int host_pinned_max_ = 8;
    int next_ticket_ = 0;
};

}
```

headposeestimation-whenet_amd/csrc/front7.hip:

```cpp
#include "device_math.h"
#include "kernels.h"
#include "stamps.h"

#include <atomic>
#include <string>
#include <type_traits>

namespace whenet {

namespace {

constexpr int HW7 = 7;

struct F7Params {
    const void* x;
    const void* wep;
    const float* be;
    const void* wdt;
    const float* bd;
    void* out;
    float* rpart;
    const float* w1t;
    int n, Cin, Cexp, NTe, R, RPse;
    int off_w, off_stage, off_red, off_sum;
    float wsi;
    int chunks, ngroups, xcd;
};

template <int K, int KS, int G, int CC, int NTHR>
__global__ __launch_bounds__(NTHR) void whenet_front7_kernel(const F7Params p) {
    constexpr int NWAVE = NTHR / 64;
    constexpr int PAD = K / 2;
    constexpr int ROWS = HW7;
    constexpr int NT = CC / 32, NCB = CC / 16;
    constexpr int nrow = G * ROWS;
    constexpr int nstrip = (nrow + 3) / 4;

    extern __shared__ __attribute__((aligned(16))) unsigned char smem[];
    unsigned char* E = smem;
    const half8* Wl = reinterpret_cast<const half8*>(smem + p.off_w);

    const int tid = threadIdx.x;
    const int lane = tid & 63;
    const int wave = __builtin_amdgcn_readfirstlane(tid >> 6);
    const int g = lane >> 5, lm = lane & 31;
    const int Cin = p.Cin;
    int grp, chunk;
    xcd_unit(int(blockIdx.x), p.ngroups, p.chunks, grp, chunk, p.xcd != 0);
    const int c0 = chunk * CC;
    const int crop0 = grp * G;
    const int nlast = p.n - 1;

    STAMP(0);
    constexpr int nwv = KS * NT * 64;
    constexpr int WV = (nwv + NTHR - 1) / NTHR;
    half8 wstage[WV];
    {
        const half8* src = reinterpret_cast<const half8*>(p.wep);
#pragma unroll
        for (int i = 0; i < WV; ++i) {
            const int v = tid + i * NTHR;
            if (v < nwv) {
                const int ks = v / (NT * 64), r = v - ks * (NT * 64);
                wstage[i] = src[(size_t(ks) * p.NTe + (c0 >> 5)) * 64 + r];
            }
        }
    }
    auto a_offset = [&](int strip) -> unsigned {
        int R = strip * 4 + (lm >> 3);
        R = R < nrow ? R : nrow - 1;
        const int cr = (R * 37) >> 8;
        const int row = R - cr * 7;
        int gc = crop0 + cr;
        gc = gc < nlast ? gc : nlast;
        int px = lm & 7;
        px = px < 7 ? px : 6;
        return unsigned((gc * 49 + row * 7 + px) * Cin + g * 8) * 2u;
    };
    const unsigned char* xb = reinterpret_cast<const unsigned char*>(p.x);
    half8 a[KS];
    constexpr bool SPLIT = nstrip * NT <= NWAVE;
    int strip = SPLIT ? (wave < nstrip * NT ? wave % nstrip : nstrip) : wave;
    const int t_lo = SPLIT ? wave / nstrip : 0, t_hi = SPLIT ? t_lo + 1 : NT;
    constexpr bool STG = !SPLIT && nstrip <= NWAVE && nstrip * 4032 <= (G + 3) / 4 * NCB * ROWS * 64 * 16 && KS % 4 == 0;
    if (strip < nstrip) {
        if constexpr (STG) {
            constexpr int PX = 28, SEG = KS / 4;
            constexpr int rowb = KS * 32;
            unsigned char* sa = E + wave * 4032;
            const size_t last = size_t(p.n) * 49 * rowb - 16;
            const size_t base = (size_t(crop0) * 49 + size_t(strip) * PX) * rowb;
            half8 raw[SEG][4];
#pragma unroll
            for (int t = 0; t < SEG; ++t)
#pragma unroll
                for (int i = 0; i < 4; ++i) {
                    int idx = i * 64 + lane;
                    idx = idx < PX * 8 ? idx : PX * 8 - 1;
                    size_t off = base + size_t(idx >> 3) * rowb + t * 128 + (idx & 7) * 16;
                    off = off < last ? off : last;
                    raw[t][i] = *reinterpret_cast<const half8*>(xb + off);
                }
            int pf = (lm >> 3) * 7 + ((lm & 7) < 7 ? (lm & 7) : 6);
            const int rlim = nrow - strip * 4;
            if ((lm >> 3) >= rlim) pf = (rlim - 1) * 7 + 6;
#pragma unroll
            for (int t = 0; t < SEG; ++t) {
#pragma unroll
                for (int i = 0; i < 4; ++i) {
                    const int idx = i * 64 + lane;
                    if (idx < PX * 8) *reinterpret_cast<half8*>(sa + (idx >> 3) * 144 + (idx & 7) * 16) = raw[t][i];
                }
#pragma unroll
                for (int u = 0; u < 4; ++u) a[t * 4 + u] = *reinterpret_cast<const half8*>(sa + pf * 144 + u * 32 + g * 16);
            }
        } else {
            const unsigned off = a_offset(strip);
#pragma unroll
            for (int ks = 0; ks < KS; ++ks) a[ks] = *reinterpret_cast<const half8*>(xb + off + ks * 32);
        }
    }
    float bias_t[NT];
#pragma unroll
    for (int t = 0; t < NT; ++t) bias_t[t] = p.be[c0 + t * 32 + lm];
    {
        half8* dst = reinterpret_cast<half8*>(smem + p.off_w);
#pragma unroll
        for (int i = 0; i < WV; ++i) {
            const int v = tid + i * NTHR;
            if (v < nwv) dst[v] = wstage[i];
        }
    }
    lds_barrier();
    STAMP(1);

    for (; strip < nstrip; strip += NWAVE) {
        const bool more = strip + NWAVE < nstrip;
#pragma unroll
        for (int t = 0; t < NT; ++t) {
            if (t < t_lo || t >= t_hi) continue;
            float16v acc;
#pragma unroll
            for (int r = 0; r < 16; ++r) acc[r] = bias_t[t];
#pragma unroll
            for (int ks = 0; ks < KS; ++ks)
                acc = __builtin_amdgcn_mfma_f32_32x32x16_f16(a[ks], Wl[(ks * NT + t) * 64 + lane], acc, 0, 0, 0);
            const int ch = t * 32 + lm, cb = ch >> 4, cl = ch & 15;
#pragma unroll
            for (int qq = 0; qq < 4; ++qq) {
                const int R = strip * 4 + qq;
                if (R < nrow) {
                    const int cr = (R * 37) >> 8, row = R - cr * 7;
                    const int jq = cr >> 2, j = cr & 3;
                    const float2v y0 = swish2(float2v{acc[4 * qq], acc[4 * qq + 1]});
                    const float2v y1 = swish2(float2v{acc[4 * qq + 2], acc[4 * qq + 3]});
                    half4 o;
                    o[0] = half_t(y0[0]);
                    o[1] = half_t(y0[1]);
                    o[2] = half_t(y1[0]);
                    o[3] = g ? half_t(0) : half_t(y1[1]);
                    unsigned char* ep = E + ((((jq * NCB + cb) * ROWS + row) * 64 + j * 16 + (cl ^ (j << 2))) << 4) + g * 8;
                    *reinterpret_cast<half4*>(ep) = o;
                }
            }
        }
        if (more) {
            const unsigned off = a_offset(strip + NWAVE);
#pragma unroll
            for (int ks = 0; ks < KS; ++ks) a[ks] = *reinterpret_cast<const half8*>(xb + off + ks * 32);
        }
    }
    STAMP(2);

    constexpr int NJQ = (G + 3) / 4;
    constexpr int nitem = NJQ * NCB * 2;
    const int cl = lane >> 2, j = lane & 3;
    half4 A[K][2];
    float bdv = 0.f;
    auto load_taps = [&](int it) {
        const int xgl = it & 1, cb = (it >> 1) % NCB;
        const half4* src = reinterpret_cast<const half4*>(p.wdt) + (size_t((c0 >> 4) + cb) * K * 3 + (1 - xgl)) * 64 + lane;
#pragma unroll
        for (int ky = 0; ky < K; ++ky) {
            A[ky][0] = src[(ky * 3) * 64];
            A[ky][1] = src[(ky * 3 + 1) * 64];
        }
        bdv = p.bd[c0 + cb * 16 + cl];
    };
    int it = wave;
    if (it < nitem) load_taps(it);
    constexpr int W1Q = CC / 16;
    float4v w1v[W1Q];
    {
        const int jo = (tid >> 2) & 63, q = tid & 3;
        const float* wrow = p.w1t + size_t(jo < p.R ? jo : p.R - 1) * p.Cexp + c0 + q * (CC / 4);
#pragma unroll
        for (int i = 0; i < W1Q; ++i) w1v[i] = *reinterpret_cast<const float4v*>(wrow + 4 * i);
    }
    lds_barrier();
    STAMP(3);

    unsigned char* stg = smem + p.off_stage + wave * 2048;
    float* s_red = reinterpret_cast<float*>(smem + p.off_red);
    float* s_sum = reinterpret_cast<float*>(smem + p.off_sum);
    const int unit = j * 16 + (cl ^ (j << 2));
    const int jP = (lane >> 1) & 3, iP = (lane >> 3) & 3, hP = lane & 1, rP = lane >> 5;
    unsigned char* outb = reinterpret_cast<unsigned char*>(p.out);
    const unsigned row_bytes = unsigned(HW7) * unsigned(p.Cexp) * 2u;

    for (; it < nitem; it += NWAVE) {
        const int xgl = it & 1, cbq = it >> 1, cb = cbq % NCB, jq = cbq / NCB;
        const unsigned char* bp = E + ((((jq * NCB + cb) * ROWS) * 64 + unit) << 4);
        float4v acc[ROWS];
#pragma unroll
        for (int r = 0; r < ROWS; ++r) acc[r] = float4v{bdv, bdv, bdv, bdv};
#pragma unroll
        for (int er = 0; er < ROWS; ++er) {
            const half8 v = *reinterpret_cast<const half8*>(bp + er * 1024);
            const half4 b0 = {v[0], v[1], v[2], v[3]}, b1 = {v[4], v[5], v[6], v[7]};
#pragma unroll
            for (int ky = 0; ky < K; ++ky) {
                const int d = er - ky + PAD;
                if (d >= 0 && d < ROWS) {
                    acc[d] = __builtin_amdgcn_mfma_f32_4x4x4f16(A[ky][0], b0, acc[d], 0, 0, 0);
                    acc[d] = __builtin_amdgcn_mfma_f32_4x4x4f16(A[ky][1], b1, acc[d], 0, 0, 0);
                }
            }
        }
        if (it + NWAVE < nitem) load_taps(it + NWAVE);
        const int cr = jq * 4 + j;
        const bool okc = cr < G && crop0 + cr < p.n;
        float m[4];
#pragma unroll
        for (int i = 0; i < 4; ++i) m[i] = (okc && 4 * xgl + i < HW7) ? 1.f : 0.f;
        const int crP = jq * 4 + jP, oxP = 4 * xgl + iP;
        const bool okP = crP < G && crop0 + crP < p.n && oxP < HW7;
        const unsigned obase = (unsigned(crop0 + crP) * 49u + unsigned(rP) * 7u + unsigned(oxP)) * unsigned(p.Cexp) * 2u +
                               unsigned(c0 + cb * 16 + hP * 8) * 2u;
        float2v sum2 = {0.f, 0.f};
        const float2v m01 = {m[0], m[1]}, m23 = {m[2], m[3]};
        unsigned char* sw = stg + j * 32 + cl * 2;
#pragma unroll
        for (int half = 0; half < 2; ++half) {
            const int r0 = half * 4, nr = half ? 3 : 4;
#pragma unroll
            for (int r = 0; r < nr; ++r) {
                const float2v y01 = swish2(float2v{acc[r0 + r][0], acc[r0 + r][1]});
                const float2v y23 = swish2(float2v{acc[r0 + r][2], acc[r0 + r][3]});
                sum2 = y01 * m01 + sum2;
                sum2 = y23 * m23 + sum2;
                *reinterpret_cast<half_t*>(sw + (r * 4 + 0) * 128) = half_t(y01[0]);
                *reinterpret_cast<half_t*>(sw + (r * 4 + 1) * 128) = half_t(y01[1]);
                *reinterpret_cast<half_t*>(sw + (r * 4 + 2) * 128) = half_t(y23[0]);
                *reinterpret_cast<half_t*>(sw + (r * 4 + 3) * 128) = half_t(y23[1]);
            }
            wave_lds_sync();
#pragma unroll
            for (int pp = 0; pp < 2; ++pp) {
                const int rl = 2 * pp + rP;
                const half8 v = *reinterpret_cast<const half8*>(stg + (pp * 64 + lane) * 16);
                if (okP && rl < nr) *reinterpret_cast<half8*>(outb + obase + unsigned(r0 + 2 * pp) * row_bytes) = v;
            }
            wave_lds_sync();
        }
        if (cr < G) s_red[(cr * 2 + xgl) * CC + cb * 16 + cl] = sum2[0] + sum2[1];
    }
    STAMP(4);
    lds_barrier();
    STAMP(5);

#pragma unroll
    for (int i0 = 0; i0 < G * CC; i0 += NTHR) {
        const int i = i0 + tid;
        if (i < G * CC) {
            const int cr = i / CC, c = i % CC;
            s_sum[i] = s_red[(cr * 2) * CC + c] + s_red[(cr * 2 + 1) * CC + c];
        }
    }
    lds_barrier();
    {
        const int jo = (tid >> 2) & 63, q = tid & 3;
        for (int cr = tid >> 8; cr < G; cr += NTHR / 256) {
            float accr = 0.0f;
            if (jo < p.R) {
                const float* sp = s_sum + cr * CC + q * (CC / 4);
#pragma unroll
                for (int i = 0; i < W1Q; ++i) {
                    const float4v sv = *reinterpret_cast<const float4v*>(sp + 4 * i);
#pragma unroll
                    for (int e = 0; e < 4; ++e) accr = fmaf(sv[e], w1v[i][e], accr);
                }
            }
            const float pair = accr + quad_xor1(accr);
            const float tot = pair + quad_xor2(pair);
            if (q == 0 && jo < p.RPse && crop0 + cr < p.n)
                p.rpart[(size_t(crop0 + cr) * p.chunks + chunk) * p.RPse + jo] = (jo < p.R) ? tot : 0.0f;
        }
    }
    STAMP(6);
}

template <int K, int KS8, int G, int CC, int NTHR, bool SP = false>
__global__ __launch_bounds__(NTHR) void whenet_front7_f32_kernel(const F7Params p) {
    constexpr int NWAVE = NTHR / 64;
    constexpr int PAD = K / 2;
    constexpr int ROWS = HW7;
    constexpr int NT = CC / 32, NCB = CC / 16;
    constexpr int nrow = G * ROWS;
    constexpr int nstrip = (nrow + 3) / 4;

    extern __shared__ __attribute__((aligned(16))) unsigned char smem[];
    unsigned char* E = smem;
    const float4v* Wl = reinterpret_cast<const float4v*>(smem + p.off_w);

    const int tid = threadIdx.x;
    const int lane = tid & 63;
    const int wave = __builtin_amdgcn_readfirstlane(tid >> 6);
    const int g = lane >> 5, lm = lane & 31;
    const int Cin = p.Cin;
    int grp, chunk;
    xcd_unit(int(blockIdx.x), p.ngroups, p.chunks, grp, chunk, p.xcd != 0);
    const int c0 = chunk * CC;
    const int crop0 = grp * G;
    const int nlast = p.n - 1;

    constexpr int nwv = KS8 * NT * 64;
    constexpr int WV = (nwv + NTHR - 1) / NTHR;
    constexpr int KS16 = KS8 / 2;
    float4v wstage[WV];
    {
        const float4v* src = reinterpret_cast<const float4v*>(p.wep);
        const size_t w_lo = size_t(KS16) * p.NTe * 64;
#pragma unroll
        for (int i = 0; i < WV; ++i) {
            const int v = tid + i * NTHR;
            if (v < nwv) {
                if constexpr (SP) {
                    const int l = v & 63, h = (v >> 6) & 1, kt = v >> 7, ks = kt / NT, t = kt % NT;
                    wstage[i] = src[(h ? w_lo : 0) + (size_t(ks) * p.NTe + (c0 >> 5) + t) * 64 + l];
                } else {
                    const int ks = v / (NT * 64), r = v % (NT * 64);
                    wstage[i] = src[(size_t(ks) * p.NTe + (c0 >> 5)) * 64 + r];
                }
            }
        }
    }
    auto a_offset = [&](int strip) -> unsigned {
        int R = strip * 4 + (lm >> 3);
        R = R < nrow ? R : nrow - 1;
        const int cr = (R * 37) >> 8;
        const int row = R - cr * 7;
        int gc = crop0 + cr;
        gc = gc < nlast ? gc : nlast;
        int px = lm & 7;
        px = px < 7 ? px : 6;
        return unsigned((gc * 49 + row * 7 + px) * Cin + g * (SP ? 8 : 4)) * 4u;
    };
    const unsigned char* xb = reinterpret_cast<const unsigned char*>(p.x);
    using OPS = PwOps<float, true>;
    float4v a[SP ? 1 : KS8];
    OPS::P ap[SP ? KS16 : 1];
    auto load_rows = [&](unsigned off) {
        if constexpr (SP) {
            OPS::A raw[KS16];
#pragma unroll
            for (int ks = 0; ks < KS16; ++ks) raw[ks] = OPS::load_a(reinterpret_cast<const float*>(xb + off + ks * 64));
#pragma unroll
            for (int ks = 0; ks < KS16; ++ks) ap[ks] = OPS::prep(raw[ks]);
        } else {
#pragma unroll
            for (int ks = 0; ks < KS8; ++ks) a[ks] = *reinterpret_cast<const float4v*>(xb + off + ks * 32);
        }
    };
    constexpr bool SPLIT = nstrip * NT <= NWAVE;
    int strip = SPLIT ? (wave < nstrip * NT ? wave % nstrip : nstrip) : wave;
    const int t_lo = SPLIT ? wave / nstrip : 0, t_hi = SPLIT ? t_lo + 1 : NT;
    constexpr bool STG = !SPLIT && nstrip <= NWAVE && KS8 % 4 == 0;
    if (strip < nstrip) {
        if constexpr (STG) {
            constexpr int PX = 28, SEG = KS8 / 4;
            constexpr int rowb = KS8 * 32;
            unsigned char* sa = E + wave * 4032;
            const size_t last = size_t(p.n) * 49 * rowb - 16;
            const size_t base = (size_t(crop0) * 49 + size_t(strip) * PX) * rowb;
            int pf = (lm >> 3) * 7 + ((lm & 7) < 7 ? (lm & 7) : 6);
            const int rlim = nrow - strip * 4;
            if ((lm >> 3) >= rlim) pf = (rlim - 1) * 7 + 6;
            OPS::A rawsp[SP ? KS16 : 1];
#pragma unroll
            for (int t0 = 0; t0 < SEG; t0 += 3) {
                float4v raw[3][4];
#pragma unroll
                for (int tt = 0; tt < 3; ++tt)
#pragma unroll
                    for (int i = 0; i < 4; ++i) {
                        int idx = i * 64 + lane;
                        idx = idx < PX * 8 ? idx : PX * 8 - 1;
                        size_t off = base + size_t(idx >> 3) * rowb + (t0 + tt) * 128 + (idx & 7) * 16;
                        off = off < last ? off : last;
                        raw[tt][i] = *reinterpret_cast<const float4v*>(xb + off);
                    }
#pragma unroll
                for (int tt = 0; tt < 3; ++tt) {
                    const int t = t0 + tt;
#pragma unroll
                    for (int i = 0; i < 4; ++i) {
                        const int idx = i * 64 + lane;
                        if (idx < PX * 8) *reinterpret_cast<float4v*>(sa + (idx >> 3) * 144 + (idx & 7) * 16) = raw[tt][i];
                    }
                    if constexpr (SP) {
#pragma unroll
                        for (int u = 0; u < 2; ++u) {
                            rawsp[t * 2 + u].x0 = *reinterpret_cast<const float4v*>(sa + pf * 144 + u * 64 + g * 32);
                            rawsp[t * 2 + u].x1 = *reinterpret_cast<const float4v*>(sa + pf * 144 + u * 64 + g * 32 + 16);
                        }
                    } else {
#pragma unroll
                        for (int u = 0; u < 4; ++u) a[t * 4 + u] = *reinterpret_cast<const float4v*>(sa + pf * 144 + u * 32 + g * 16);
                    }
                }
            }
            if constexpr (SP) {
#pragma unroll
                for (int ks = 0; ks < KS16; ++ks) ap[ks] = OPS::prep(rawsp[ks]);
            }
        } else {
            load_rows(a_offset(strip));
        }
    }
    float bias_t[NT];
#pragma unroll
    for (int t = 0; t < NT; ++t) bias_t[t] = p.be[c0 + t * 32 + lm];
    {
        float4v* dst = reinterpret_cast<float4v*>(smem + p.off_w);
#pragma unroll
        for (int i = 0; i < WV; ++i) {
            const int v = tid + i * NTHR;
            if (v < nwv) dst[v] = wstage[i];
        }
    }
    lds_barrier();

    for (; strip < nstrip; strip += NWAVE) {
        const bool more = strip + NWAVE < nstrip;
#pragma unroll
        for (int t = 0; t < NT; ++t) {
            if (t < t_lo || t >= t_hi) continue;
            float16v acc;
#pragma unroll
            for (int r = 0; r < 16; ++r) acc[r] = 0.0f;
            if constexpr (SP) {
#pragma unroll
                for (int ks = 0; ks < KS16; ++ks) {
                    const half8 whi = __builtin_bit_cast(half8, Wl[((ks * NT + t) * 2) * 64 + lane]);
                    const half8 wlo = __builtin_bit_cast(half8, Wl[((ks * NT + t) * 2 + 1) * 64 + lane]);
                    acc = __builtin_amdgcn_mfma_f32_32x32x16_f16(ap[ks].hi, wlo, acc, 0, 0, 0);
                    acc = __builtin_amdgcn_mfma_f32_32x32x16_f16(ap[ks].lo, whi, acc, 0, 0, 0);
                    acc = __builtin_amdgcn_mfma_f32_32x32x16_f16(ap[ks].hi, whi, acc, 0, 0, 0);
                }
            } else {
#pragma unroll
                for (int ks = 0; ks < KS8; ++ks) {
                    const float4v w = Wl[(ks * NT + t) * 64 + lane];
#pragma unroll
                    for (int u = 0; u < 4; ++u) acc = __builtin_amdgcn_mfma_f32_32x32x2f32(a[ks][u], w[u], acc, 0, 0, 0);
                }
            }
            const float bias = bias_t[t];
            const int ch = t * 32 + lm, cb = ch >> 4, cl = ch & 15;
#pragma unroll
            for (int qq = 0; qq < 4; ++qq) {
                const int R = strip * 4 + qq;
                if (R < nrow) {
                    const int cr = (R * 37) >> 8, row = R - cr * 7;
                    const int jq = cr >> 2, j = cr & 3;
                    float4v o;
#pragma unroll
                    for (int r = 0; r < 4; ++r) o[r] = conv_swish<float>(SP ? fmaf(acc[4 * qq + r], p.wsi, bias) : acc[4 * qq + r] + bias);
                    if (g) o[3] = 0.f;
                    unsigned char* ep = E + ((((jq * NCB + cb) * ROWS + row) * 64 + j * 16 + (cl ^ (j << 2))) << 5) + g * 16;
                    *reinterpret_cast<float4v*>(ep) = o;
                }
            }
        }
        if (more) load_rows(a_offset(strip + NWAVE));
    }

    constexpr int NJQ = (G + 3) / 4;
    constexpr int nitem = NJQ * NCB * 2;
    const int cl = lane >> 2, j = lane & 3;
    float wt[K * K];
    float bdv = 0.f;
    auto load_taps = [&](int it) {
        const int cb = (it >> 1) % NCB;
        const float* src = reinterpret_cast<const float*>(p.wdt) + c0 + cb * 16 + cl;
#pragma unroll
        for (int q = 0; q < K * K; ++q) wt[q] = src[size_t(q) * p.Cexp];
        bdv = p.bd[c0 + cb * 16 + cl];
    };
    int it = wave;
    if (it < nitem) load_taps(it);
    constexpr int W1Q = CC / 16;
    float4v w1v[W1Q];
    {
        const int jo = (tid >> 2) & 63, q = tid & 3;
        const float* wrow = p.w1t + size_t(jo < p.R ? jo : p.R - 1) * p.Cexp + c0 + q * (CC / 4);
#pragma unroll
        for (int i = 0; i < W1Q; ++i) w1v[i] = *reinterpret_cast<const float4v*>(wrow + 4 * i);
    }
    lds_barrier();

    float* s_red = reinterpret_cast<float*>(smem + p.off_red);
    float* s_sum = reinterpret_cast<float*>(smem + p.off_sum);
    const int unit = j * 16 + (cl ^ (j << 2));
    float* outp = reinterpret_cast<float*>(p.out);

    for (; it < nitem; it += NWAVE) {
        const int xgl = it & 1, cbq = it >> 1, cb = cbq % NCB, jq = cbq / NCB;
        const unsigned char* bp = E + ((((jq * NCB + cb) * ROWS) * 64 + unit) << 5);
        float acc[ROWS][4];
#pragma unroll
        for (int r = 0; r < ROWS; ++r)
#pragma unroll
            for (int i = 0; i < 4; ++i) acc[r][i] = 0.f;
        auto rows = [&](auto xg) {
            constexpr int XG = decltype(xg)::value;
#pragma unroll
            for (int er = 0; er < ROWS; ++er) {
                const float4v lo = *reinterpret_cast<const float4v*>(bp + er * 2048);
                const float4v hi = *reinterpret_cast<const float4v*>(bp + er * 2048 + 16);
                const float in[8] = {lo[0], lo[1], lo[2], lo[3], hi[0], hi[1], hi[2], hi[3]};
#pragma unroll
                for (int ky = 0; ky < K; ++ky) {
                    const int d = er - ky + PAD;
                    if (d >= 0 && d < ROWS) {
#pragma unroll
                        for (int i = 0; i < 4; ++i)
#pragma unroll
                            for (int kx = 0; kx < K; ++kx) {
                                const int px = 4 * XG + i + kx - PAD;
                                if (px >= 0 && px < HW7) acc[d][i] = fmaf(in[px], wt[ky * K + kx], acc[d][i]);
                            }
                    }
                }
            }
        };
        if (xgl == 0) rows(std::integral_constant<int, 0>{});
        else rows(std::integral_constant<int, 1>{});
        const float bd_this = bdv;
        if (it + NWAVE < nitem) load_taps(it + NWAVE);
        const int cr = jq * 4 + j;
        const bool okc = cr < G && crop0 + cr < p.n;
        float sum = 0.f;
        float* ob = outp + (size_t(crop0 + cr) * 49 + 4 * xgl) * p.Cexp + c0 + cb * 16 + cl;
#pragma unroll
        for (int r = 0; r < ROWS; ++r)
#pragma unroll
            for (int i = 0; i < 4; ++i) {
                const float y = conv_swish<float>(acc[r][i] + bd_this);
                if (okc && 4 * xgl + i < HW7) {
                    sum += y;
                    ob[size_t(r * 7 + i) * p.Cexp] = y;
                }
            }
        if (cr < G) s_red[(cr * 2 + xgl) * CC + cb * 16 + cl] = okc ? sum : 0.f;
    }
    lds_barrier();

#pragma unroll
    for (int i0 = 0; i0 < G * CC; i0 += NTHR) {
        const int i = i0 + tid;
        if (i < G * CC) {
            const int cr = i / CC, c = i % CC;
            s_sum[i] = s_red[(cr * 2) * CC + c] + s_red[(cr * 2 + 1) * CC + c];
        }
    }
    lds_barrier();
    {
        const int jo = (tid >> 2) & 63, q = tid & 3;
        for (int cr = tid >> 8; cr < G; cr += NTHR / 256) {
            float accr = 0.0f;
            if (jo < p.R) {
                const float* sp = s_sum + cr * CC + q * (CC / 4);
#pragma unroll
                for (int i = 0; i < W1Q; ++i) {
                    const float4v sv = *reinterpret_cast<const float4v*>(sp + 4 * i);
#pragma unroll
                    for (int e = 0; e < 4; ++e) accr = fmaf(sv[e], w1v[i][e], accr);
                }
            }
            const float pair = accr + quad_xor1(accr);
            const float tot = pair + quad_xor2(pair);
            if (q == 0 && jo < p.RPse && crop0 + cr < p.n)
                p.rpart[(size_t(crop0 + cr) * p.chunks + chunk) * p.RPse + jo] = (jo < p.R) ? tot : 0.0f;
        }
    }
}

struct OncePerDevice7 {
    std::atomic<bool> done[64];
    OncePerDevice7() { for (auto& d : done) d.store(false, std::memory_order_relaxed); }
};

template <int K, int KS, int G, int CC, int NTHR, bool F32, bool SP = false>
void launch_f7(const Front7Args& a, hipStream_t stream) {
    const Front7Plan& pl = a.plan;
    F7Params p{};
    p.x = a.x;
    p.wep = SP ? a.weps : a.wep;
    p.wsi = a.wsi;
    p.be = a.be;
    p.wdt = a.wdt;
    p.bd = a.bd;
    p.out = a.out;
    p.rpart = a.rpart;
    p.w1t = a.w1t;
    p.n = a.n;  p.Cin = a.Cin;  p.Cexp = a.Cexp;  p.NTe = a.NTe;
    p.R = a.R;  p.RPse = (a.R + 3) & ~3;
    p.off_w = pl.off_w;  p.off_stage = pl.off_stage;  p.off_red = pl.off_red;  p.off_sum = pl.off_sum;
    WHENET_REQUIRE(pl.lds_bytes <= 160 * 1024, WHENET_EINVAL, "front7: the tile plan needs more than 160 KB of LDS");
    static OncePerDevice7 attr;
    int dev = 0;
    WHENET_HIP_CHECK(hipGetDevice(&dev));
    auto kern = [] {
        if constexpr (F32) return &whenet_front7_f32_kernel<K, KS, G, CC, NTHR, SP>;
        else return &whenet_front7_kernel<K, KS, G, CC, NTHR>;
    }();
    if (dev >= 0 && dev < 64 && !attr.done[dev].load(std::memory_order_acquire)) {
        WHENET_HIP_CHECK(hipFuncSetAttribute(reinterpret_cast<const void*>(kern), hipFuncAttributeMaxDynamicSharedMemorySize, 160 * 1024));
        attr.done[dev].store(true, std::memory_order_release);
    }
    p.chunks = pl.chunks;  p.ngroups = ceil_div(a.n, pl.G);  p.xcd = a.xcd_grouped ? 1 : 0;
    hipLaunchKernelGGL(kern, dim3(unsigned(p.chunks) * unsigned(p.ngroups)), dim3(NTHR), pl.lds_bytes, stream, p);
    WHENET_HIP_CHECK(hipGetLastError());
}

}

Front7Plan make_front7_plan(int dtype, int Cin, int Cexp, int G, int CC, int threads) {
    WHENET_REQUIRE((threads == 256 || threads == 512) && G >= 1 && G <= 8 && (CC == 32 || CC == 64 || CC == 128) && Cexp % CC == 0 &&
                       Cin % 16 == 0,
                   WHENET_EINVAL, "front7: bad tile plan");
    Front7Plan p;
    p.threads = threads;
    p.G = G;
    p.CC = CC;
    p.chunks = Cexp / CC;
    const bool f32 = dtype == WHENET_F32;
    const int njq = (G + 3) / 4, ncb = CC / 16, ks = Cin / (f32 ? 8 : 16), nt = CC / 32;
    const size_t e_bytes = size_t(njq) * ncb * HW7 * 64 * (f32 ? 32 : 16);
    p.off_w = int(e_bytes);
    const int w_bytes = ks * nt * 1024, stage_bytes = f32 ? 0 : (threads / 64) * 2048;
    p.off_stage = p.off_w;
    p.off_red = p.off_w + (w_bytes > stage_bytes ? w_bytes : stage_bytes);
    p.off_sum = p.off_red + G * 2 * CC * 4;
    p.lds_bytes = size_t(p.off_sum) + size_t(G) * CC * 4;
    return p;
}

Front7Plan front7_plan_for(int dtype, int Cin, int Cexp, int n) {
    const int G = (dtype == WHENET_F32 && n == 1) ? 1 : (n <= 16 ? 2 : 4);
    return make_front7_plan(dtype, Cin, Cexp, G, 64, 512);
}

bool front7_supported(int k, int s, int H, int Cin) { return (k == 3 || k == 5) && s == 1 && H == HW7 && Cin == 192; }

void launch_front7(const Front7Args& a, hipStream_t stream) {
    WHENET_REQUIRE(front7_supported(a.k, 1, HW7, a.Cin) && a.w1t != nullptr && a.R >= 1 && a.R <= 64 && a.n >= 1, WHENET_EINVAL,
                   "front7: 7 x 7 maps, 3x3 / 5x5 stride-1 kernels, Cin = 192, squeeze-excite reduce conv in the kernel");
    const int key = ((a.k * 10 + a.plan.G) * 1000 + a.plan.CC) * 1000 + a.plan.threads;
    if (a.dtype == WHENET_F32) {
        switch (key) {
#define F7_CASE32(K, G, CC, T) case ((K * 10 + G) * 1000 + CC) * 1000 + T: \
        if (a.split) launch_f7<K, 24, G, CC, T, true, true>(a, stream); else launch_f7<K, 24, G, CC, T, true>(a, stream); break;
            F7_CASE32(5, 4, 64, 512) F7_CASE32(3, 4, 64, 512)
            F7_CASE32(5, 2, 64, 512) F7_CASE32(3, 2, 64, 512)
            F7_CASE32(5, 1, 64, 512) F7_CASE32(3, 1, 64, 512)
#undef F7_CASE32
            default: throw Error(WHENET_EINVAL, "front7: no f32 instantiation for this (kernel, G, CC, lanes) plan");
        }
        return;
    }
    switch (key) {
#define F7_CASE(K, G, CC, T) case ((K * 10 + G) * 1000 + CC) * 1000 + T: launch_f7<K, 12, G, CC, T, false>(a, stream); break;
        F7_CASE(5, 4, 64, 512) F7_CASE(3, 4, 64, 512)
        F7_CASE(5, 2, 64, 512) F7_CASE(3, 2, 64, 512)
#ifdef WHENET_FRONT7_ALL_PLANS
        F7_CASE(5, 4, 64, 256) F7_CASE(3, 4, 64, 256)
        F7_CASE(5, 4, 32, 256) F7_CASE(3, 4, 32, 256)
        F7_CASE(5, 4, 32, 512) F7_CASE(3, 4, 32, 512)
        F7_CASE(5, 2, 64, 256) F7_CASE(3, 2, 64, 256)
        F7_CASE(5, 2, 32, 256) F7_CASE(3, 2, 32, 256)
        F7_CASE(5, 8, 32, 512) F7_CASE(3, 8, 32, 512)
        F7_CASE(5, 8, 64, 512) F7_CASE(3, 8, 64, 512)
        F7_CASE(5, 4, 128, 512) F7_CASE(3, 4, 128, 512)
        F7_CASE(5, 1, 64, 256) F7_CASE(3, 1, 64, 256)
#endif
#undef F7_CASE
        default: throw Error(WHENET_EINVAL, "front7: no instantiation for this (kernel, G, CC, lanes) plan");
    }
}

std::string kernel_name_front7(int dtype, int k, const Front7Plan& p, bool split) {
    return std::string(dtype == WHENET_F32 ? "whenet_front7_f32_kernel<" : "whenet_front7_kernel<") + std::to_string(k) +
           (dtype == WHENET_F32 ? ", 24, " : ", 12, ") + std::to_string(p.G) + ", " + std::to_string(p.CC) + ", " +
           std::to_string(p.threads) + (dtype == WHENET_F32 ? (split ? ", true>" : ", false>") : ">");
}

}
```

headposeestimation-whenet_amd/csrc/head7.hip:

```cpp
#include "device_math.h"
#include "kernels.h"

#include <atomic>
#include <string>

namespace whenet {

namespace {

constexpr int H7_K = 320, H7_KS = H7_K / 16, H7_HW = 49, H7_NC = 64, H7_NT = H7_NC / 32;

template <int G, int NTHR>
__global__ __launch_bounds__(NTHR) void whenet_head7_kernel(const half_t* __restrict__ x, const half_t* __restrict__ wep,
                                                            const float* __restrict__ bias, float* __restrict__ feat, int n,
                                                            int NTILES, int N, int xcd) {
    constexpr int NWAVE = NTHR / 64;
    constexpr int nstrip = 2 * G;
    constexpr int KS = H7_KS, NT = H7_NT, NC = H7_NC;
    extern __shared__ __attribute__((aligned(16))) unsigned char smem[];
    const half8* Wl = reinterpret_cast<const half8*>(smem);
    float* s_gap = reinterpret_cast<float*>(smem + KS * NT * 1024);

    const int tid = threadIdx.x;
    const int lane = tid & 63;
    const int wave = __builtin_amdgcn_readfirstlane(tid >> 6);
    const int g = lane >> 5, lm = lane & 31;
    int grp, chunk;
    xcd_unit(int(blockIdx.x), (n + G - 1) / G, N / NC, grp, chunk, xcd != 0);
    const int c0 = chunk * NC;
    const int crop0 = grp * G;
    const int nlast = n - 1;

    constexpr int nwv = KS * NT * 64;
    constexpr int WV = (nwv + NTHR - 1) / NTHR;
    half8 wstage[WV];
    {
        const half8* src = reinterpret_cast<const half8*>(wep);
#pragma unroll
        for (int i = 0; i < WV; ++i) {
            const int v = tid + i * NTHR;
            if (v < nwv) {
                const int ks = v / (NT * 64), r = v % (NT * 64);
                wstage[i] = src[(size_t(ks) * NTILES + (c0 >> 5)) * 64 + r];
            }
        }
    }
    constexpr bool SPLIT = nstrip * NT <= NWAVE;
    const int strip = SPLIT ? (wave < nstrip * NT ? wave % nstrip : nstrip) : wave;
    const int t_lo = SPLIT ? wave / nstrip : 0, t_hi = SPLIT ? t_lo + 1 : NT;
    half8 a[KS];
    if (strip < nstrip) {
        int gc = crop0 + (strip >> 1);
        gc = gc < nlast ? gc : nlast;
        int px = (strip & 1) * 32 + lm;
        px = px < H7_HW ? px : H7_HW - 1;
        const unsigned char* xr = reinterpret_cast<const unsigned char*>(x) + (size_t(gc) * H7_HW + px) * (H7_K * 2) + g * 16;
#pragma unroll
        for (int ks = 0; ks < KS; ++ks) a[ks] = *reinterpret_cast<const half8*>(xr + ks * 32);
    }
    float bias_t[NT];
#pragma unroll
    for (int t = 0; t < NT; ++t) bias_t[t] = bias[c0 + t * 32 + lm];
    {
        half8* dst = reinterpret_cast<half8*>(smem);
#pragma unroll
        for (int i = 0; i < WV; ++i) {
            const int v = tid + i * NTHR;
            if (v < nwv) dst[v] = wstage[i];
        }
    }
    lds_barrier();

    if (strip < nstrip) {
#pragma unroll
        for (int t = 0; t < NT; ++t) {
            if (t < t_lo || t >= t_hi) continue;
            float16v acc;
#pragma unroll
            for (int r = 0; r < 16; ++r) acc[r] = bias_t[t];
#pragma unroll
            for (int ks = 0; ks < KS; ++ks)
                acc = __builtin_amdgcn_mfma_f32_32x32x16_f16(a[ks], Wl[(ks * NT + t) * 64 + lane], acc, 0, 0, 0);
            float sum = 0.f;
#pragma unroll
            for (int qq = 0; qq < 4; ++qq) {
                const float2v y0 = swish2(float2v{acc[4 * qq], acc[4 * qq + 1]});
                const float2v y1 = swish2(float2v{acc[4 * qq + 2], acc[4 * qq + 3]});
                const float y[4] = {y0[0], y0[1], y1[0], y1[1]};
#pragma unroll
                for (int r = 0; r < 4; ++r) {
                    const int px = (strip & 1) * 32 + 8 * qq + 4 * g + r;
                    sum += (px < H7_HW) ? y[r] : 0.f;
                }
            }
            s_gap[(strip * 2 + g) * NC + t * 32 + lm] = sum;
        }
    }
    lds_barrier();
#pragma unroll
    for (int i0 = 0; i0 < G * NC; i0 += NTHR) {
        const int i = i0 + tid;
        if (i < G * NC) {
            const int cr = i / NC, c = i % NC;
            if (crop0 + cr < n && c0 + c < N) {
                const float* s0 = s_gap + ((2 * cr) * 2) * NC + c;
                feat[size_t(crop0 + cr) * N + c0 + c] = ((s0[0] + s0[NC]) + (s0[2 * NC] + s0[3 * NC])) * (1.0f / 49.0f);
            }
        }
    }
}

constexpr int H7F_KS = H7_K / 8, H7F_NC = 32, H7F_KG = 5, H7F_NGRP = H7F_KS / H7F_KG;

template <int G, bool SP>
__global__ __launch_bounds__(128 * G) void whenet_head7_f32_kernel(const float* __restrict__ x, const float* __restrict__ wep,
                                                                   const float* __restrict__ bias, float* __restrict__ feat, int n,
                                                                   int NTILES, int N, float wsi, int xcd) {
    constexpr int NTHR = 128 * G, nstrip = 2 * G, NC = H7F_NC, KG = H7F_KG;
    constexpr int KS = SP ? H7_K / 16 : H7F_KS;
    constexpr int NGRP = KS / KG;
    constexpr int KF = SP ? 16 : 8;
    (void)nstrip;
    extern __shared__ __attribute__((aligned(16))) unsigned char smem[];
    const float4v* Wl = reinterpret_cast<const float4v*>(smem);
    float* s_gap = reinterpret_cast<float*>(smem + H7F_KS * 1024);

    const int tid = threadIdx.x;
    const int lane = tid & 63;
    const int strip = __builtin_amdgcn_readfirstlane(tid >> 6);
    const int g = lane >> 5, lm = lane & 31;
    int grp, chunk;
    xcd_unit(int(blockIdx.x), (n + G - 1) / G, N / NC, grp, chunk, xcd != 0);
    const int c0 = chunk * NC;
    const int crop0 = grp * G;

    constexpr int nwv = H7F_KS * 64;
    static_assert(nwv % NTHR == 0, "weight staging: whole vectors per lane");
    constexpr int WV = nwv / NTHR;
    float4v wstage[WV];
    {
        const float4v* src = reinterpret_cast<const float4v*>(wep);
        const size_t w_lo = size_t(KS) * NTILES * 64;
#pragma unroll
        for (int i = 0; i < WV; ++i) {
            const int v = tid + i * NTHR;
            if constexpr (SP) wstage[i] = src[(((v >> 6) & 1) ? w_lo : 0) + (size_t(v >> 7) * NTILES + (c0 >> 5)) * 64 + (v & 63)];
            else wstage[i] = src[(size_t(v >> 6) * NTILES + (c0 >> 5)) * 64 + (v & 63)];
        }
    }
    int gc = crop0 + (strip >> 1);
    gc = gc < n - 1 ? gc : n - 1;
    int pxl = (strip & 1) * 32 + lm;
    pxl = pxl < H7_HW ? pxl : H7_HW - 1;
    const float* xr = x + (size_t(gc) * H7_HW + pxl) * H7_K + g * (KF / 2);
    using OPS = PwOps<float, SP>;
    using AF = typename OPS::A;
    AF a0[KG], a1[KG];
    auto load_group = [&](AF (&a)[KG], int grp) {
#pragma unroll
        for (int u = 0; u < KG; ++u) a[u] = OPS::load_a(xr + (grp * KG + u) * KF);
    };
    load_group(a0, 0);
    const float bias_v = bias[c0 + lm];
    {
        float4v* dst = reinterpret_cast<float4v*>(smem);
#pragma unroll
        for (int i = 0; i < WV; ++i) dst[tid + i * NTHR] = wstage[i];
    }
    lds_barrier();

    float16v acc;
#pragma unroll
    for (int r = 0; r < 16; ++r) acc[r] = 0.f;
    auto compute = [&](const AF (&a)[KG], int grp) {
#pragma unroll
        for (int u = 0; u < KG; ++u) {
            if constexpr (SP) {
                const half8 whi = __builtin_bit_cast(half8, Wl[((grp * KG + u) * 2) * 64 + lane]);
                const half8 wlo = __builtin_bit_cast(half8, Wl[((grp * KG + u) * 2 + 1) * 64 + lane]);
                const typename OPS::P pa = OPS::prep(a[u]);
                acc = __builtin_amdgcn_mfma_f32_32x32x16_f16(pa.hi, wlo, acc, 0, 0, 0);
                acc = __builtin_amdgcn_mfma_f32_32x32x16_f16(pa.lo, whi, acc, 0, 0, 0);
                acc = __builtin_amdgcn_mfma_f32_32x32x16_f16(pa.hi, whi, acc, 0, 0, 0);
            } else {
                const float4v w = Wl[(grp * KG + u) * 64 + lane];
#pragma unroll
                for (int t = 0; t < 4; ++t) acc = __builtin_amdgcn_mfma_f32_32x32x2f32(a[u].v[t], w[t], acc, 0, 0, 0);
            }
        }
    };
#pragma unroll
    for (int grp = 0; grp < NGRP; grp += 2) {
        load_group(a1, grp + 1);
        __builtin_amdgcn_sched_barrier(0);
        compute(a0, grp);
        __builtin_amdgcn_sched_barrier(0);
        if (grp + 2 < NGRP) load_group(a0, grp + 2);
        __builtin_amdgcn_sched_barrier(0);
        compute(a1, grp + 1);
        __builtin_amdgcn_sched_barrier(0);
    }
    float sum = 0.f;
#pragma unroll
    for (int r = 0; r < 16; ++r) {
        const int px = (strip & 1) * 32 + 8 * (r >> 2) + 4 * g + (r & 3);
        const float y = conv_swish<float>(SP ? fmaf(acc[r], wsi, bias_v) : acc[r] + bias_v);
        sum += (px < H7_HW) ? y : 0.f;
    }
    s_gap[(strip * 2 + g) * NC + lm] = sum;
    lds_barrier();
    if (tid < G * NC) {
        const int cr = tid / NC, c = tid % NC;
        if (crop0 + cr < n && c0 + c < N) {
            const float* s0 = s_gap + ((2 * cr) * 2) * NC + c;
            feat[size_t(crop0 + cr) * N + c0 + c] = ((s0[0] + s0[NC]) + (s0[2 * NC] + s0[3 * NC])) * (1.0f / 49.0f);
        }
    }
}

template <int G>
void launch_h7_f32(const Head7Args& a, hipStream_t stream) {
    const size_t lds = size_t(H7F_KS) * 1024 + size_t(2 * G) * 2 * H7F_NC * 4;
    if (a.split)
        hipLaunchKernelGGL((whenet_head7_f32_kernel<G, true>), dim3(unsigned(a.N / H7F_NC) * unsigned(ceil_div(a.n, G))), dim3(128 * G), lds, stream,
                           static_cast<const float*>(a.x), static_cast<const float*>(a.weps), a.bias, a.feat, a.n, a.NTILES, a.N, a.wsi, a.xcd_grouped ? 1 : 0);
    else
        hipLaunchKernelGGL((whenet_head7_f32_kernel<G, false>), dim3(unsigned(a.N / H7F_NC) * unsigned(ceil_div(a.n, G))), dim3(128 * G), lds, stream,
                           static_cast<const float*>(a.x), static_cast<const float*>(a.wep), a.bias, a.feat, a.n, a.NTILES, a.N, 1.0f, a.xcd_grouped ? 1 : 0);
    WHENET_HIP_CHECK(hipGetLastError());
}

template <int G>
void launch_h7(const Head7Args& a, hipStream_t stream) {
    constexpr int NTHR = 512;
    const size_t lds = size_t(H7_KS) * H7_NT * 1024 + size_t(2 * G) * 2 * H7_NC * 4;
    hipLaunchKernelGGL((whenet_head7_kernel<G, NTHR>), dim3(unsigned(a.N / H7_NC) * unsigned(ceil_div(a.n, G))), dim3(NTHR), lds, stream,
                       static_cast<const half_t*>(a.x), static_cast<const half_t*>(a.wep), a.bias, a.feat, a.n, a.NTILES, a.N, a.xcd_grouped ? 1 : 0);
    WHENET_HIP_CHECK(hipGetLastError());
}

}

bool head7_supported(int dtype, int K, int N, int HW) {
    return (dtype == WHENET_F16 || dtype == WHENET_F32) && K == H7_K && HW == H7_HW && N % H7_NC == 0;
}

void launch_head7(const Head7Args& a, hipStream_t stream) {
    WHENET_REQUIRE(head7_supported(a.dtype, a.K, a.N, 49) && a.n >= 1 && a.x && a.wep && a.bias && a.feat, WHENET_EINVAL,
                   "head7: the 320 -> N (multiple of 64) head conv on 7 x 7 maps");
    if (a.dtype == WHENET_F16) {
        if (a.n <= 16) launch_h7<2>(a, stream);
        else launch_h7<4>(a, stream);
    } else {
        if (a.n <= 16) launch_h7_f32<2>(a, stream);
        else launch_h7_f32<4>(a, stream);
    }
}

std::string kernel_name_head7(int dtype, int n, bool split) {
    if (dtype == WHENET_F16) return std::string("whenet_head7_kernel<") + (n <= 16 ? "2" : "4") + ", 512>";
    return std::string("whenet_head7_f32_kernel<") + (n <= 16 ? "2" : "4") + (split ? ", true>" : ", false>");
}

}
```

headposeestimation-whenet_amd/csrc/kernels.h:

```cpp
#pragma once

#include <string>
#include <vector>

#include "common.h"

namespace whenet {

struct StemArgs {
    const uint8_t* in;
    void* out;
    const float* w;
    const float* bias;
    const float* lut;
    int n;
    const float* in_f32 = nullptr;
};
void launch_stem(const StemArgs& a, int dtype, hipStream_t stream);

struct DwPlan {
    int threads = 256;
    int CV = 1;
    int TH = 1;
    int NSX = 1;
    int tiles_x = 1, tiles_y = 1, chunks = 1;
    int IH = 0, IW = 0;
    size_t lds_bytes = 0;
    int ntiles() const { return tiles_x * tiles_y; }
};
DwPlan plan_dw(int dtype, int k, int s, int H, int Ho, int C);

struct DwArgs {
    const void* in;
    void* out;
    const float* w;
    const float* bias;
    float* partial;
    int k, s, H, Ho, C, pad, n;
    DwPlan plan;
};
void launch_dw(const DwArgs& a, int dtype, hipStream_t stream);

struct SeArgs {
    const float* partial;
    int ntiles;
    float inv_hw;
    const float* w1t;
    const float* b1;
    const float* w2c;
    const float* b2;
    void* gate;
    int C, R, n;
    int gate_f16 = 0;
};
void launch_se(const SeArgs& a, hipStream_t stream);
struct SeExciteArgs {
    const float* rpart;
    int np;
    float inv_hw;
    const float* b1;
    const float* w2c;
    const float* b2;
    void* gate;
    int C, R, n;
    int gate_f16 = 0;
};
void launch_se_excite(const SeExciteArgs& a, hipStream_t stream);
int se_excite_split(int C);
int se_padded_r(int R);

enum { ACT_NONE = 0, ACT_SWISH = 1 };
struct SeFuse {
    const float* rpart = nullptr;
    const float* b1 = nullptr;
    const float* w2c = nullptr;
    const float* b2 = nullptr;
    int np = 0, R = 0, RP = 0;
    float inv_hw = 0.f;
    const void* w2p = nullptr;
    int KSr = 0;
    float w2_wsi = 1.0f;
};
struct PwArgs {
    const void* a;
    const void* wp;
    const float* wdense;
    const float* bias;
    const void* gate;
    const void* res;
    void* out;
    int M, K, N, KS, NTILES, HW, act;
    SeFuse se;
    bool split = false;
    const void* wps = nullptr;
    int KSs = 0;
    float wsi = 1.0f;
    bool staged = true;
};
void launch_pw(const PwArgs& a, int dtype, int impl, int num_cus, hipStream_t stream);

struct HeadsArgs {
    const void* x;
    const float* feat_in;
    const float* logits_in;
    const float* w;
    const float* b;
    float* feat;
    float* logits;
    float* ypr;
    int32_t* argmax;
    int n;
};
void launch_heads(const HeadsArgs& a, int dtype, hipStream_t stream);
void launch_heads_split(const HeadsArgs& a, float* part, unsigned* count, int dtype, hipStream_t stream);
int heads_split();

struct Head7Args {
    int dtype;
    const void* x;
    const void* wep;
    const float* bias;
    float* feat;
    int K, N, NTILES, n;
    bool split = false;
    const void* weps = nullptr;
    float wsi = 1.0f;
    bool xcd_grouped = false;
};
bool head7_supported(int dtype, int K, int N, int HW);
void launch_head7(const Head7Args& a, hipStream_t stream);
std::string kernel_name_head7(int dtype, int n, bool split = false);

struct StemDwTable {
    uint32_t lut[3 * 256];
    half8 whi[3][64], wlo[3][64];
};
void build_stemdw_table(const float* w , const float* lut , StemDwTable* out);

struct StemDwArgs {
    int dtype;
    const uint8_t* in;
    void* out;
    const StemDwTable* tab;
    const float* w;
    const float* lut;
    const float* bias;
    const float* wd;
    const float* bd;
    float* partial;
    int n;
};
bool stemdw_supported(int dtype, const DwPlan& p, int k, int s, int H, int C);
void launch_stemdw(const StemDwArgs& a, hipStream_t stream);
const char* kernel_name_stemdw(int dtype);

struct FrontPlan {
    int threads = 256;
    int CC = 32;
    int TH = 1, NSX = 1;
    int tiles_x = 1, tiles_y = 1, chunks = 1;
    int EH = 0, EW = 0;
    int EP = 0;
    int w_off = 0;
    size_t lds_bytes = 0;
    int ntiles() const { return tiles_x * tiles_y; }
};
FrontPlan plan_front(int dtype, int k, int s, int H, int Ho, int Cexp);
std::vector<FrontPlan> plan_front_candidates(int dtype, int k, int s, int H, int Ho, int Cexp,
                                             std::vector<double>* scores);
int front_threads(const FrontPlan& p, int n);
struct FrontArgs {
    const void* x;
    const void* wep;
    const float* be;
    const float* wd;
    const float* bd;
    void* out;
    float* rpart;
    const float* w1t;
    int R;
    int k, s, H, Ho, Cin, Cexp, pad, KSe, NTe, n;
    FrontPlan plan;
    bool split = false;
    const void* weps = nullptr;
    int KSes = 0;
    float wsi = 1.0f;
    const float* in_gate = nullptr;
    bool xcd_grouped = false;
};
void launch_front(const FrontArgs& a, int dtype, hipStream_t stream);
std::string kernel_name_front(int dtype, int k, int s, int threads);

struct Front2Plan {
    int threads = 256;
    int CC = 32;
    int TH = 7;
    int TXG = 1;
    int xs = 0;
    int tiles_x = 1, tiles_y = 1, chunks = 1;
    int EH = 0, EWp = 0;
    int RP = 0, CP = 0;
    int off_stage = 0, off_red = 0, off_sum = 0;
    size_t lds_bytes = 0;
    int ntiles() const { return tiles_x * tiles_y; }
};
Front2Plan make_front2_plan(int k, int s, int Ho, int Cexp, int CC, int TH, int TXG, int threads, int xs);
Front2Plan plan_front2(int k, int s, int H, int Ho, int Cexp);
std::vector<Front2Plan> plan_front2_candidates(int k, int s, int Ho, int Cexp);
int front2_threads(const Front2Plan& p, int n);
std::vector<half_t> pack_dw_toeplitz(const std::vector<float>& w, int k, int s, int C, int xs);
bool front2_preferred(int k, int s, int H, int Cexp);
struct Front2Args {
    const void* x;
    const void* wep;
    const float* be;
    const void* wdt;
    const float* bd;
    void* out;
    float* rpart;
    const float* w1t;
    const float* in_gate;
    int R;
    int k, s, H, Ho, Cin, Cexp, pad, KSe, NTe, n;
    Front2Plan plan;
    bool xcd_grouped = false;
};
void launch_front2(const Front2Args& a, hipStream_t stream);
std::string kernel_name_front2(int k, int s, int kse, int threads, int xs, bool gated);

struct Front2sArgs {
    const void* x;
    const void* weps;
    const float* be;
    const void* wdt;
    const float* bd;
    void* out;
    float* rpart;
    const float* w1t;
    int R;
    int k, s, H, Ho, Cin, Cexp, pad, KSe, NTe, n;
    float wsi = 1.0f;
    float wsi_d = 1.0f;
    int tm = 2;
    bool pre = false;
    Front2Plan plan;
};
bool front2s_supported(int k, int s, int H, int Cin);
bool front2s_preferred(int k, int s, int H, int Cexp);
Front2Plan make_front2s_plan(int k, int s, int Ho, int Cexp, int CC, int TH, int TXG, int threads);
Front2Plan plan_front2s(int k, int s, int H, int Ho, int Cexp, int* tm);
std::vector<Front2Plan> plan_front2s_candidates(int k, int s, int Ho, int Cexp);
std::vector<float> pack_dw_toeplitz_s(const std::vector<float>& w, int k, int s, int C, int tm, float* wsi);
void launch_front2s(const Front2sArgs& a, hipStream_t stream);
std::string kernel_name_front2s(int k, int s, int kse, int threads, int tm, bool pre);

struct Front7Plan {
    int threads = 512;
    int G = 4;
    int CC = 64;
    int chunks = 1;
    int off_w = 0, off_stage = 0, off_red = 0, off_sum = 0;
    size_t lds_bytes = 0;
};
Front7Plan make_front7_plan(int dtype, int Cin, int Cexp, int G, int CC, int threads);
Front7Plan front7_plan_for(int dtype, int Cin, int Cexp, int n);
bool front7_supported(int k, int s, int H, int Cin);
struct Front7Args {
    int dtype = WHENET_F16;
    const void* x;
    const void* wep;
    const float* be;
    const void* wdt;
    const float* bd;
    void* out;
    float* rpart;
    const float* w1t;
    int R;
    int k, Cin, Cexp, NTe, n;
    Front7Plan plan;
    bool split = false;
    const void* weps = nullptr;
    float wsi = 1.0f;
    bool xcd_grouped = false;
};
void launch_front7(const Front7Args& a, hipStream_t stream);
std::string kernel_name_front7(int dtype, int k, const Front7Plan& p, bool split = false);

struct Mb7Args {
    const void* x;
    const void* wep;
    const float* be;
    const void* wds;
    const float* bd;
    const void* w1p;
    const float* b1;
    const void* w2p;
    const float* b2;
    const void* wpp;
    const float* bp;
    void* out;
    void* dbg_dw = nullptr;
    void* dbg_gate = nullptr;
    int k, Cout, n;
    bool skip;
};
bool mb7_supported(int dtype, int k, int s, int H, int Cin, int Cexp, int R, int Cout, bool skip);
std::vector<half_t> pack_mb7_taps(const std::vector<float>& w , int k, int C);
void pack_mb7_se(const std::vector<float>& w1t , const std::vector<float>& w2 , int C, int R,
                 std::vector<half_t>* w1p, std::vector<half_t>* w2p);
void launch_mb7(const Mb7Args& a, hipStream_t stream);
std::string kernel_name_mb7(int k, int Cout, bool skip);

struct YoloLayer {
    const float* feats;
    int gh, gw;
    int first;
    float anchor[3][2];
};
struct YoloArgs {
    YoloLayer layer[3];
    int num_layers, num_classes, na;
    int N, NP;
    float input_h, input_w, image_h, image_w;
    float off_y, off_x, scale_y, scale_x;
    float score_thr, iou_thr;
    int max_boxes;
    float* boxes;
    float* all_scores;
    int* counts;
    unsigned long long* keys;
    float* out_boxes;
    float* out_scores;
    int* out_index;
    int* out_count;
};
void launch_yolo_eval(const YoloArgs& a, hipStream_t stream);
int yolo_max_select();

constexpr int CROP_PLAN_INTS = 8 + 6 * IMG;
void frame_box_rect(int frame_h, int frame_w, const float bbox[4], int32_t rect[4]);
void build_crop_plan(const int32_t rect[4], int32_t* plan);
void launch_crop_resize(const uint8_t* d_frame, int fw, int swap_rb, const int32_t* d_plan, int k, uint8_t* d_out,
                        hipStream_t stream);

void launch_empty(hipStream_t stream);
void launch_f32_to_act(const float* src, void* dst, size_t count, int dtype, hipStream_t stream);
void launch_act_to_f32(const void* src, float* dst, size_t count, int dtype, hipStream_t stream);

const char* kernel_name_stem(int dtype);
const char* kernel_name_dw(int dtype, int k, int s);
std::string kernel_name_pw(const PwArgs& a, int dtype, int impl, int num_cus);

}
```

headposeestimation-whenet_amd/csrc/pw.hip:

```cpp
#include "device_math.h"
#include "kernels.h"
#include "se_device.h"
#include "stamps.h"

#ifndef WHENET_PW_DEPTH
#define WHENET_PW_DEPTH 2
#endif

namespace whenet {

namespace {

template <typename T, int B2, bool RES, int ACT, bool SP>
__device__ __forceinline__ void splitk_combine_store(float16v (&acc)[B2][B2], float* s_red, int kpart, int lane, int mt, int nt0, int M,
                                                     int N, int NTILES, const float* __restrict__ bias, const T* __restrict__ res,
                                                     T* __restrict__ out, float wsi) {
    using OT = T __attribute__((ext_vector_type(4)));
    constexpr int MB = B2, NT = B2;
    constexpr int NACC = MB * NT * 16, SL = NACC / 4;
    const int g = lane >> 5;
    const int f0 = kpart * SL;
    const int own_tile = f0 >> 4, own_mb = own_tile / NT, own_t = own_tile % NT;
    const int own_row = (mt * MB + own_mb) * 32 + (lane & 31);
    const bool own_valid = own_row < M && nt0 + own_t < NTILES;
    OT rv[SL / 4];
    float4v bv[SL / 4];
#pragma unroll
    for (int i4 = 0; i4 < SL / 4; ++i4) {
        const int qq = ((f0 & 15) >> 2) + i4;
        const int n0 = (nt0 + own_t) * 32 + 8 * qq + 4 * g;
        const bool ok = own_valid && n0 < N;
        bv[i4] = ok ? *reinterpret_cast<const float4v*>(bias + n0) : float4v{0.f, 0.f, 0.f, 0.f};
        if constexpr (RES) rv[i4] = ok ? *reinterpret_cast<const OT*>(res + size_t(own_row) * N + n0) : OT{};
    }
    float own[SL];
#pragma unroll
    for (int dst = 0; dst < 4; ++dst) {
        if (dst == kpart) {
#pragma unroll
            for (int i = 0; i < SL; ++i) {
                const int f = dst * SL + i;
                own[i] = acc[(f >> 4) / NT][(f >> 4) % NT][f & 15];
            }
        } else {
            const int src = (kpart < dst) ? kpart : kpart - 1;
#pragma unroll
            for (int i = 0; i < SL; ++i) {
                const int f = dst * SL + i;
                s_red[((dst * 3 + src) * SL + i) * 64 + lane] = acc[(f >> 4) / NT][(f >> 4) % NT][f & 15];
            }
        }
    }
    lds_barrier();
    STAMP(3);
    float sum[SL];
#pragma unroll
    for (int src = 0; src < 4; ++src) {
        if (src == kpart) {
#pragma unroll
            for (int i = 0; i < SL; ++i) sum[i] = (src == 0) ? own[i] : sum[i] + own[i];
        } else {
            const int si = (src < kpart) ? src : src - 1;
#pragma unroll
            for (int i = 0; i < SL; ++i) {
                const float v = s_red[((kpart * 3 + si) * SL + i) * 64 + lane];
                sum[i] = (src == 0) ? v : sum[i] + v;
            }
        }
    }
    if (!own_valid) return;
#pragma unroll
    for (int i4 = 0; i4 < SL / 4; ++i4) {
        const int qq = ((f0 & 15) >> 2) + i4;
        const int n0 = (nt0 + own_t) * 32 + 8 * qq + 4 * g;
        if (n0 >= N) continue;
        OT o;
#pragma unroll
        for (int r = 0; r < 4; ++r) {
            float y = SP ? fmaf(sum[4 * i4 + r], wsi, bv[i4][r]) : sum[4 * i4 + r] + bv[i4][r];
            if constexpr (ACT == ACT_SWISH) y = conv_swish<T>(y);
            if constexpr (RES) y += float(rv[i4][r]);
            o[r] = T(y);
        }
        *reinterpret_cast<OT*>(out + size_t(own_row) * N + n0) = o;
    }
    STAMP(4);
}

template <typename T, int B2, int GM, bool RES, int ACT, bool SP = false>
__global__ __launch_bounds__(256, B2 == 2 ? 2 : 3) void whenet_pw_splitk_kernel(
    const T* __restrict__ A, const T* __restrict__ Wp, const float* __restrict__ bias, const T* __restrict__ gate,
    const T* __restrict__ res, T* __restrict__ out, int M, int K, int N, int KS, int NTILES, int HW, int MT, int NCH,
    const SeFuse se, float wsi) {
    constexpr bool GATE = GM != 0;
    using OPS = PwOps<T, SP>;
    constexpr int V = OPS::V;
    constexpr int SV = Vec<T>::V;
    using VT = typename Vec<T>::type;
    using OT = T __attribute__((ext_vector_type(4)));
    constexpr int MB = B2, NT = B2, SK = 4;
    constexpr int U = (B2 == 2) ? 2 : 4;
    constexpr int NACC = MB * NT * 16, SL = NACC / 4;
    __shared__ float s_red[4 * 3 * SL * 64];
    constexpr int GCROPS = MB + 1, GK = 1152;
    __shared__ __attribute__((aligned(16))) T s_gate[GATE ? GCROPS * GK : 8];
    __shared__ float s_r[GM == 2 ? GCROPS * 48 : 4];

    const int id = blockIdx.x;
    const int q = id >> 3;
    const int nch = q % NCH;
    const int mt = (id & 7) + 8 * (q / NCH);
    if (mt >= MT) return;
    STAMP(0);

    const int lane = threadIdx.x & 63;
    const int kpart = __builtin_amdgcn_readfirstlane(threadIdx.x >> 6);
    const int nt0 = nch * NT;
    const int g = lane >> 5;
    bool rvalid[MB];
    const T* ap[MB];
    const T* gp[MB];
    const int row_first = mt * MB * 32;
    const int crop_lo = row_first / HW;
#pragma unroll
    for (int mb = 0; mb < MB; ++mb) {
        const int row = (mt * MB + mb) * 32 + (lane & 31);
        rvalid[mb] = row < M;
        const int rowc = rvalid[mb] ? row : (M - 1);
        ap[mb] = A + size_t(rowc) * K + g * V;
        gp[mb] = GATE ? s_gate + (rowc / HW - crop_lo) * K + g * V : nullptr;
    }
    const int row_last = (row_first + MB * 32 < M ? row_first + MB * 32 : M) - 1;
    const int ncrop = row_last / HW - crop_lo + 1;
    constexpr int GV = GM == 1 ? (GCROPS * GK / SV + 255) / 256 : 1;
    VT gv[GV];
    if constexpr (GM == 1) {
        const VT* src = reinterpret_cast<const VT*>(gate + size_t(crop_lo) * K);
#pragma unroll
        for (int j = 0; j < GV; ++j) {
            const int i = int(threadIdx.x) + j * 256;
            gv[j] = src[i < ncrop * K / SV ? i : 0];
        }
    }
    const size_t w_lane = size_t(nt0) * 64 + lane;
    const size_t w_lo = size_t(KS) * NTILES * 64;

    float16v acc[MB][NT];
#pragma unroll
    for (int mb = 0; mb < MB; ++mb)
#pragma unroll
        for (int t = 0; t < NT; ++t)
#pragma unroll
            for (int r = 0; r < 16; ++r) acc[mb][t][r] = 0.0f;

    struct Ops {
        typename OPS::A a[U][MB];
        typename OPS::W w[U][NT];
    };
    auto issue = [&](int ks, Ops& o) {
#pragma unroll
        for (int u = 0; u < U; ++u) {
            const int k1 = ks + u * SK;
            const int k1c = k1 < KS ? k1 : KS - 1;
            const size_t wk = w_lane + size_t(k1c) * NTILES * 64;
#pragma unroll
            for (int t = 0; t < NT; ++t) o.w[u][t] = OPS::load_w(Wp, wk + (nt0 + t < NTILES ? t : 0) * 64, w_lo);
#pragma unroll
            for (int mb = 0; mb < MB; ++mb) o.a[u][mb] = OPS::load_a(ap[mb] + k1c * 2 * V);
        }
    };
    auto compute = [&](const Ops& o, int ks) {
#pragma unroll
        for (int u = 0; u < U; ++u) {
            const int k1 = ks + u * SK;
            if (k1 >= KS) continue;
#pragma unroll
            for (int mb = 0; mb < MB; ++mb) {
                typename OPS::A a = o.a[u][mb];
                if constexpr (GATE) OPS::gate(a, gp[mb] + k1 * 2 * V);
                const typename OPS::P pa = OPS::prep(a);
#pragma unroll
                for (int t = 0; t < NT; ++t)
                    if (nt0 + t < NTILES) OPS::step(o.w[u][t], pa, acc[mb][t]);
            }
        }
    };

    constexpr int D = WHENET_PW_DEPTH;
    Ops o[D];
#pragma unroll
    for (int d = 0; d < D - 1; ++d) issue(kpart + d * U * SK, o[d]);
    if constexpr (GM == 1) {
        VT* dst = reinterpret_cast<VT*>(s_gate);
#pragma unroll
        for (int j = 0; j < GV; ++j) {
            const int i = int(threadIdx.x) + j * 256;
            if (i < ncrop * K / SV) dst[i] = gv[j];
        }
        lds_barrier();
    }
    if constexpr (GM == 2) se_fused_to_lds<T, 256>(se, crop_lo, ncrop, K, s_gate, s_r);
    STAMP(1);
    for (int ks = kpart; ks < KS; ks += D * U * SK) {
#pragma unroll
        for (int d = 0; d < D; ++d) {
            issue(ks + (d + D - 1) * U * SK, o[(d + D - 1) % D]);
            compute(o[d], ks + d * U * SK);
        }
    }
    STAMP(2);

    splitk_combine_store<T, B2, RES, ACT, SP>(acc, s_red, kpart, lane, mt, nt0, M, N, NTILES, bias, res, out, wsi);
}

template <typename T, int B2, int GM, bool RES, int ACT, bool SP = false>
__global__ __launch_bounds__(256, B2 == 2 ? 2 : 3) void whenet_pw_splitk_staged_kernel(
    const T* __restrict__ A, const T* __restrict__ Wp, const float* __restrict__ bias, const T* __restrict__ gate,
    const T* __restrict__ res, T* __restrict__ out, int M, int K, int N, int KS, int NTILES, int HW, int MT, int NCH,
    const SeFuse se, float wsi) {
    constexpr bool GATE = GM != 0;
    using OPS = PwOps<T, SP>;
    constexpr int V = OPS::V;
    constexpr int SV = Vec<T>::V;
    using VT = typename Vec<T>::type;
    constexpr int MB = B2, NT = B2;
    constexpr int R = MB * 32;
    constexpr int KSB = 2 * V * int(sizeof(T));
    constexpr int KGS = 128 / KSB;
    constexpr int NLD = R / 8;
    constexpr int NACC = MB * NT * 16, SL = NACC / 4;
    constexpr int STAGE_BYTES = 4 * R * 128, RED_BYTES = 4 * 3 * SL * 64 * 4;
    __shared__ __attribute__((aligned(16))) unsigned char smem[STAGE_BYTES > RED_BYTES ? STAGE_BYTES : RED_BYTES];
    float* s_red = reinterpret_cast<float*>(smem);
    constexpr int GCROPS = MB + 1, GK = 1152;
    __shared__ __attribute__((aligned(16))) T s_gate[GATE ? GCROPS * GK : 8];
    __shared__ float s_r[GM == 2 ? GCROPS * 48 : 4];
    constexpr int GT = 128 / int(sizeof(T)) / 32;
    constexpr int KSRM = 3;
    constexpr int NIMG = SP ? 2 : 1;
    __shared__ __attribute__((aligned(16))) half_t s_rw[GM == 3 ? 4 * NIMG * 4 * 48 : 8];

    const int id = blockIdx.x;
    const int q = id >> 3;
    const int nch = q % NCH;
    const int mt = (id & 7) + 8 * (q / NCH);
    if (mt >= MT) return;

    const int lane = threadIdx.x & 63;
    const int kpart = __builtin_amdgcn_readfirstlane(threadIdx.x >> 6);
    const int nt0 = nch * NT;
    const int g = lane >> 5, j = lane & 31;
    const int row_first = mt * R;
    const int crop_lo = row_first / HW;
    const T* gp[MB];
#pragma unroll
    for (int mb = 0; mb < MB; ++mb) {
        const int row = row_first + mb * 32 + j;
        const int rowc = row < M ? row : (M - 1);
        gp[mb] = GATE ? s_gate + (rowc / HW - crop_lo) * K + g * V : nullptr;
    }
    const int row_last = (row_first + R < M ? row_first + R : M) - 1;
    const int ncrop = row_last / HW - crop_lo + 1;
    constexpr int GV = GM == 1 ? (GCROPS * GK / SV + 255) / 256 : 1;
    VT gv[GV];
    if constexpr (GM == 1) {
        const VT* src = reinterpret_cast<const VT*>(gate + size_t(crop_lo) * K);
#pragma unroll
        for (int jj = 0; jj < GV; ++jj) {
            const int i = int(threadIdx.x) + jj * 256;
            gv[jj] = src[i < ncrop * K / SV ? i : 0];
        }
    }
    const size_t w_lane = size_t(nt0) * 64 + lane;
    const size_t w_lo = size_t(KS) * NTILES * 64;

    const int lr = lane >> 3, lq = lane & 7;
    const int rowbytes = K * int(sizeof(T));
    const unsigned char* arow[NLD];
    int woff[NLD];
#pragma unroll
    for (int i = 0; i < NLD; ++i) {
        const int r = i * 8 + lr;
        const int row = row_first + r;
        arow[i] = reinterpret_cast<const unsigned char*>(A) + size_t(row < M ? row : M - 1) * rowbytes;
        woff[i] = r * 128 + ((lq ^ ((r ^ (r >> 3)) & 7)) << 4);
    }
    unsigned char* stg = smem + kpart * (R * 128);
    int rbase[MB], rswz[MB];
#pragma unroll
    for (int mb = 0; mb < MB; ++mb) {
        const int r = mb * 32 + j;
        rbase[mb] = r * 128;
        rswz[mb] = (r ^ (r >> 3)) & 7;
    }
    const int NG = (KS + KGS - 1) / KGS;

    float16v acc[MB][NT];
#pragma unroll
    for (int mb = 0; mb < MB; ++mb)
#pragma unroll
        for (int t = 0; t < NT; ++t)
#pragma unroll
            for (int r = 0; r < 16; ++r) acc[mb][t][r] = 0.0f;

    using WF = typename OPS::W;
    auto issue_a = [&](int gi, VT (&an)[NLD]) {
        const int gic = gi < NG ? gi : NG - 1;
        int off = gic * 128 + lq * 16;
        off = off < rowbytes - 16 ? off : rowbytes - 16;
#pragma unroll
        for (int i = 0; i < NLD; ++i) an[i] = *reinterpret_cast<const VT*>(arow[i] + off);
    };
    auto issue_w = [&](int gi, WF (&w)[KGS][NT]) {
#pragma unroll
        for (int s = 0; s < KGS; ++s) {
            const int k1 = gi * KGS + s;
            const int k1c = k1 < KS ? k1 : KS - 1;
            const size_t wk = w_lane + size_t(k1c) * NTILES * 64;
#pragma unroll
            for (int t = 0; t < NT; ++t) w[s][t] = OPS::load_w(Wp, wk + (nt0 + t < NTILES ? t : 0) * 64, w_lo);
        }
    };
    auto stage = [&](const VT (&an)[NLD]) {
#pragma unroll
        for (int i = 0; i < NLD; ++i) *reinterpret_cast<VT*>(stg + woff[i]) = an[i];
    };
    auto compute = [&](int gi, const WF (&w)[KGS][NT]) {
#pragma unroll
        for (int s = 0; s < KGS; ++s) {
            const int k1 = gi * KGS + s;
            if (k1 >= KS) continue;
#pragma unroll
            for (int mb = 0; mb < MB; ++mb) {
                typename OPS::A a;
                if constexpr (SP) {
                    const int q0 = s * 4 + g * 2;
                    a.x0 = *reinterpret_cast<const float4v*>(stg + rbase[mb] + ((q0 ^ rswz[mb]) << 4));
                    a.x1 = *reinterpret_cast<const float4v*>(stg + rbase[mb] + (((q0 + 1) ^ rswz[mb]) << 4));
                } else {
                    a.v = *reinterpret_cast<const VT*>(stg + rbase[mb] + (((s * 2 + g) ^ rswz[mb]) << 4));
                }
                if constexpr (GATE) OPS::gate(a, gp[mb] + k1 * 2 * V);
                const typename OPS::P pa = OPS::prep(a);
#pragma unroll
                for (int t = 0; t < NT; ++t)
                    if (nt0 + t < NTILES) OPS::step(w[s][t], pa, acc[mb][t]);
            }
        }
    };

    struct GW {
        half8 w[NIMG][KSRM][GT];
        float b2[GT];
    };
    const int NTse = K >> 5;
    const half8* w2img = reinterpret_cast<const half8*>(se.w2p);
    const size_t w2_lo = size_t(se.KSr) * NTse * 64;
    auto issue_g = [&](int gi, GW& gw) {
        if constexpr (GM == 3) {
            const int gic = gi < NG ? gi : NG - 1;
#pragma unroll
            for (int t = 0; t < GT; ++t) {
                const int tile = gic * GT + t, tilec = tile < NTse ? tile : NTse - 1;
#pragma unroll
                for (int ks = 0; ks < KSRM; ++ks) {
                    const size_t idx = (size_t(ks < se.KSr ? ks : se.KSr - 1) * NTse + tilec) * 64 + lane;
                    gw.w[0][ks][t] = w2img[idx];
                    if constexpr (SP) gw.w[1][ks][t] = w2img[w2_lo + idx];
                }
                gw.b2[t] = se.b2[tilec * 32 + j];
            }
        }
    };
    const half_t* rw_lane = s_rw + kpart * (NIMG * 4 * 48) + (((j >> 2) & 1) + 2 * (j >> 3)) * 48 + g * 8;
    const bool rw_has = (j & 3) == 0 && j < 16;
    auto rfrag = [&](int im, int ks) -> half8 {
        return rw_has ? *reinterpret_cast<const half8*>(rw_lane + im * (4 * 48) + ks * 16) : half8{0, 0, 0, 0, 0, 0, 0, 0};
    };
    auto gate_group = [&](int gi, const GW& gw) {
        if constexpr (GM == 3) {
            if (gi >= NG) return;
#pragma unroll
            for (int t = 0; t < GT; ++t) {
                const int tile = gi * GT + t;
                if (tile >= NTse) continue;
                float16v z;
#pragma unroll
                for (int r = 0; r < 16; ++r) z[r] = 0.0f;
#pragma unroll
                for (int ks = 0; ks < KSRM; ++ks) {
                    if (ks >= se.KSr) continue;
                    const half8 rhi = rfrag(0, ks);
                    if constexpr (SP) {
                        z = __builtin_amdgcn_mfma_f32_32x32x16_f16(rhi, gw.w[1][ks][t], z, 0, 0, 0);
                        z = __builtin_amdgcn_mfma_f32_32x32x16_f16(rfrag(1, ks), gw.w[0][ks][t], z, 0, 0, 0);
                    }
                    z = __builtin_amdgcn_mfma_f32_32x32x16_f16(rhi, gw.w[0][ks][t], z, 0, 0, 0);
                }
                const int ch = tile * 32 + j;
#pragma unroll
                for (int sl = 0; sl < 2; ++sl) {
                    const int c = 2 * sl + g;
                    if (c < ncrop) {
                        const float zz = SP ? fmaf(z[4 * sl], se.w2_wsi, gw.b2[t]) : z[4 * sl] + gw.b2[t];
                        s_gate[c * K + ch] = T(sigmoid_f<SP>(zz));
                    }
                }
            }
            wave_lds_sync();
        }
    };
    if constexpr (GM == 3) {
        half_t* rw = s_rw + kpart * (NIMG * 4 * 48);
        if (lane < 48) {
#pragma unroll
            for (int c = 0; c < 4; ++c) {
                float r = 0.f;
                if (c < ncrop && lane < se.RP)
                    r = se_fused_r(se.rpart + (size_t(crop_lo + c) * se.np) * se.RP + lane, se.np, se.RP, se.inv_hw,
                                   lane < se.R ? se.b1[lane] : 0.f, lane < se.R);
                const half_t hi = half_t(r);
                rw[c * 48 + lane] = hi;
                if constexpr (SP) rw[4 * 48 + c * 48 + lane] = half_t(r - float(hi));
            }
        }
        wave_lds_sync();
    }

    VT an[NLD];
    WF w0[KGS][NT], w1[KGS][NT];
    GW g0, g1;
    issue_a(kpart, an);
    issue_w(kpart, w0);
    issue_g(kpart, g0);
    if constexpr (GM == 1) {
        VT* dst = reinterpret_cast<VT*>(s_gate);
#pragma unroll
        for (int jj = 0; jj < GV; ++jj) {
            const int i = int(threadIdx.x) + jj * 256;
            if (i < ncrop * K / SV) dst[i] = gv[jj];
        }
        lds_barrier();
    }
    if constexpr (GM == 2) se_fused_to_lds<T, 256>(se, crop_lo, ncrop, K, s_gate, s_r);
    gate_group(kpart, g0);
    stage(an);
    for (int gi = kpart; gi < NG; gi += 8) {
        issue_a(gi + 4, an);
        issue_w(gi + 4, w1);
        issue_g(gi + 4, g1);
        compute(gi, w0);
        gate_group(gi + 4, g1);
        stage(an);
        if (gi + 4 < NG) {
            issue_a(gi + 8, an);
            issue_w(gi + 8, w0);
            issue_g(gi + 8, g0);
            compute(gi + 4, w1);
            gate_group(gi + 8, g0);
            stage(an);
        }
    }
    lds_barrier();
    splitk_combine_store<T, B2, RES, ACT, SP>(acc, s_red, kpart, lane, mt, nt0, M, N, NTILES, bias, res, out, wsi);
}

template <typename T, int NT, int GM, bool RES, int ACT, bool SP = false>
__global__ __launch_bounds__(256) void whenet_pw_tile_kernel(const T* __restrict__ A, const T* __restrict__ Wp,
                                                             const float* __restrict__ bias,
                                                             const T* __restrict__ gate,
                                                             const T* __restrict__ res, T* __restrict__ out, int M,
                                                             int K, int N, int KS, int NTILES, int HW, int MT,
                                                             int NCH, const SeFuse se, float wsi) {
    constexpr bool GATE = GM != 0;
    constexpr int TGK = 256;
    __shared__ __attribute__((aligned(16))) T s_gate[GATE ? 2 * TGK : 8];
    __shared__ float s_r[GM == 2 ? 2 * 12 : 4];
    using OPS = PwOps<T, SP>;
    constexpr int V = OPS::V;
    constexpr int SV = Vec<T>::V;
    using VT = typename Vec<T>::type;
    constexpr int UK = SP ? 2 : 4;
    constexpr int WT = SP ? 2 * NT : NT;
    constexpr int STAGE_VECS = UK * WT * 64;
    constexpr int CPT = (STAGE_VECS + 255) / 256;
    constexpr int SW = IsF32<T>::value ? 32 : 64;
    constexpr int TPS = SW / 32;
    constexpr int CW = SW / 8;
    constexpr int SROW = SW + 4;
    constexpr int EPI_FLOATS = 4 * 32 * SROW;
    constexpr int W_FLOATS = 2 * STAGE_VECS * 4;
    __shared__ __attribute__((aligned(16))) float smem[(EPI_FLOATS > W_FLOATS) ? EPI_FLOATS : W_FLOATS];
    VT* s_w = reinterpret_cast<VT*>(smem);

    const int id = blockIdx.x;
    const int q = id >> 3;
    const int nch = q % NCH;
    const int mt = (id & 7) + 8 * (q / NCH);
    if (mt >= MT) return;

    const int tid = threadIdx.x;
    const int lane = tid & 63;
    const int wave = tid >> 6;
    const int m0 = (mt * 4 + wave) * 32;
    const int nt0 = nch * NT;
    const int g = lane >> 5;
    const int row = m0 + (lane & 31);
    const bool rvalid = row < M;
    const int rowc = rvalid ? row : (M - 1);

    const T* ap = A + size_t(rowc) * K + g * V;
    const int crop_lo = (mt * 128) / HW;
    const T* gp = GATE ? s_gate + (rowc / HW - crop_lo) * K + g * V : nullptr;
    const VT* wsrc = reinterpret_cast<const VT*>(Wp) + size_t(nt0) * 64;

    float16v acc[NT];
#pragma unroll
    for (int t = 0; t < NT; ++t)
#pragma unroll
        for (int r = 0; r < 16; ++r) acc[t][r] = 0.0f;

    const bool ktail = K % (2 * V) != 0 && g == 1;
    using AR = typename OPS::A;
    using PR = typename OPS::P;
    auto load_raw = [&](int ks) -> AR {
        const int kc = ks < KS ? ks : KS - 1;
        AR a = OPS::load_a(ap + (ktail && kc == KS - 1 ? -g * V : 0) + kc * 2 * V);
        if (ktail && kc == KS - 1) a = OPS::zero_a();
        return a;
    };
    auto gated = [&](AR a, int ks) -> PR {
        if constexpr (GATE)
            if (ks < KS) OPS::gate(a, gp + ks * 2 * V);
        return OPS::prep(a);
    };

    VT wreg[CPT];
    static_assert(STAGE_VECS % 256 == 0, "every lane stages whole vectors");
    const size_t w_lo = size_t(KS) * NTILES * 64;
    auto fetch_w = [&](int grp) {
#pragma unroll
        for (int c = 0; c < CPT; ++c) {
            const int i = c * 256 + tid;
            const int u = i / (WT * 64);
            const int j = i - u * (WT * 64);
            const int ks = grp * UK + u;
            const int tj = j >> 6;
            const int tl = SP && tj >= NT ? tj - NT : tj;
            const int jc = nt0 + tl < NTILES ? tl * 64 + (j & 63) : (j & 63);
            wreg[c] = wsrc[(SP && tj >= NT ? w_lo : 0) + size_t(ks < KS ? ks : KS - 1) * NTILES * 64 + jc];
        }
    };
    auto store_w = [&](int buf) {
#pragma unroll
        for (int c = 0; c < CPT; ++c) {
            const int i = c * 256 + tid;
            if (i < STAGE_VECS) s_w[buf * STAGE_VECS + i] = wreg[c];
        }
    };

    const int G = (KS + UK - 1) / UK;
    AR araw[UK];
    PR areg[UK];
    fetch_w(0);
#pragma unroll
    for (int u = 0; u < UK; ++u) araw[u] = load_raw(u);
    const int row_last = (mt * 128 + 128 < M ? mt * 128 + 128 : M) - 1;
    if constexpr (GM == 1) {
        const int cnt = (row_last / HW - crop_lo + 1) * K / SV;
        const VT* src = reinterpret_cast<const VT*>(gate + size_t(crop_lo) * K);
        for (int i = tid; i < cnt; i += 256) reinterpret_cast<VT*>(s_gate)[i] = src[i];
    }
    if constexpr (GM == 2)
        se_fused_to_lds<T, 256>(se, crop_lo, row_last / HW - crop_lo + 1, K, s_gate, s_r);
    store_w(0);
    __syncthreads();
#pragma unroll
    for (int u = 0; u < UK; ++u) areg[u] = gated(araw[u], u);
    for (int grp = 0; grp < G; ++grp) {
        AR anext[UK];
        fetch_w(grp + 1);
#pragma unroll
        for (int u = 0; u < UK; ++u) anext[u] = load_raw((grp + 1) * UK + u);
        const VT* wl = s_w + (grp & 1) * STAGE_VECS + lane;
#pragma unroll
        for (int u = 0; u < UK; ++u) {
            if (grp * UK + u < KS) {
#pragma unroll
                for (int t = 0; t < NT; ++t)
                    if (nt0 + t < NTILES) {
                        typename OPS::W wf;
                        if constexpr (SP) {
                            wf.hi = __builtin_bit_cast(half8, wl[(u * WT + t) * 64]);
                            wf.lo = __builtin_bit_cast(half8, wl[(u * WT + NT + t) * 64]);
                        } else {
                            wf.v = wl[(u * WT + t) * 64];
                        }
                        OPS::step(wf, areg[u], acc[t]);
                    }
            }
        }
        store_w((grp + 1) & 1);
#pragma unroll
        for (int u = 0; u < UK; ++u) areg[u] = gated(anext[u], (grp + 1) * UK + u);
        lds_barrier();
    }

    float* s_e = smem + wave * 32 * SROW;
#pragma unroll
    for (int t0 = 0; t0 < NT; t0 += TPS) {
        int vc = N - (nt0 + t0) * 32;
        vc = (vc > SW ? SW : vc);
        vc = (vc > (NT - t0) * 32 ? (NT - t0) * 32 : vc) / CW;
        const int vcs = vc > 0 ? vc : 1;
        const float rvc = __builtin_amdgcn_rcpf(float(vcs));
        float4v bvs[TPS][4];
#pragma unroll
        for (int tt = 0; tt < TPS; ++tt)
#pragma unroll
            for (int qq = 0; qq < 4; ++qq) {
                const int n = (nt0 + t0 + tt) * 32 + 8 * qq + 4 * g;
                bvs[tt][qq] = *reinterpret_cast<const float4v*>(bias + (n < N ? n : 0));
            }
        int sr[4], sch[4];
        VT rvs[4];
#pragma unroll
        for (int i = 0; i < 4; ++i) {
            const int idx = lane + 64 * i;
            const int r = int((float(idx) + 0.5f) * rvc);
            sr[i] = r;
            sch[i] = idx - r * vcs;
            if constexpr (RES) {
                int rowc2 = m0 + (r < 32 ? r : 31);
                rowc2 = rowc2 < M ? rowc2 : M - 1;
                const int nc = vc > 0 ? (nt0 + t0) * 32 + sch[i] * CW : 0;
                rvs[i] = *reinterpret_cast<const VT*>(res + size_t(rowc2) * N + nc);
            }
        }
#pragma unroll
        for (int tt = 0; tt < TPS; ++tt) {
            const int t = t0 + tt;
            if (t < NT && nt0 + t < NTILES) {
#pragma unroll
                for (int qq = 0; qq < 4; ++qq) {
                    const int n = (nt0 + t) * 32 + 8 * qq + 4 * g;
                    float4v y;
#pragma unroll
                    for (int r = 0; r < 4; ++r) {
                        float v = SP ? fmaf(acc[t < NT ? t : 0][4 * qq + r], wsi, bvs[tt][qq][r]) : acc[t < NT ? t : 0][4 * qq + r] + bvs[tt][qq][r];
                        if constexpr (ACT == ACT_SWISH) v = conv_swish<T>(v);
                        y[r] = (n < N) ? v : 0.f;
                    }
                    *reinterpret_cast<float4v*>(s_e + (lane & 31) * SROW + tt * 32 + 8 * qq + 4 * g) = y;
                }
            }
        }
        lds_barrier();
#pragma unroll
        for (int i = 0; i < 4; ++i) {
            const int idx = lane + 64 * i;
            if (i * 64 >= 32 * vc) break;
            const int r = sr[i], ch = sch[i];
            const int n = (nt0 + t0) * 32 + ch * CW;
            const int rowg = m0 + r;
            if (idx < 32 * vc && rowg < M) {
                float y[CW];
#pragma unroll
                for (int c4 = 0; c4 < CW; c4 += 4) {
                    const float4v v = *reinterpret_cast<const float4v*>(s_e + r * SROW + ch * CW + c4);
#pragma unroll
                    for (int j = 0; j < 4; ++j) y[c4 + j] = v[j];
                }
                if constexpr (RES) {
#pragma unroll
                    for (int j = 0; j < CW; ++j) y[j] += float(rvs[i][j]);
                }
                *reinterpret_cast<VT*>(out + size_t(rowg) * N + n) = float_to_vec<T>(y);
            }
        }
        lds_barrier();
    }
}

template <typename T, bool GATE, bool RES, int ACT>
__global__ __launch_bounds__(256) void whenet_pw_check_kernel(const T* __restrict__ A, const float* __restrict__ Wd,
                                                              const float* __restrict__ bias,
                                                              const T* __restrict__ gate,
                                                              const T* __restrict__ res, T* __restrict__ out, int M,
                                                              int K, int N, int HW) {
    const int n4 = N / 4;
    const size_t idx = size_t(blockIdx.x) * 256 + threadIdx.x;
    if (idx >= size_t(M) * n4) return;
    const int m = int(idx / n4);
    const int n0 = int(idx - size_t(m) * n4) * 4;
    const T* ap = A + size_t(m) * K;
    const T* gp = GATE ? gate + size_t(m / HW) * K : nullptr;
    float acc[4] = {0.f, 0.f, 0.f, 0.f};
    for (int k = 0; k < K; ++k) {
        float a = float(ap[k]);
        if constexpr (GATE) a = float(T(a * float(gp[k])));
        const float4v w = *reinterpret_cast<const float4v*>(Wd + size_t(k) * N + n0);
#pragma unroll
        for (int r = 0; r < 4; ++r) acc[r] = fmaf(a, w[r], acc[r]);
    }
#pragma unroll
    for (int r = 0; r < 4; ++r) {
        float y = acc[r] + bias[n0 + r];
        if constexpr (ACT == ACT_SWISH) y = conv_swish<T>(y);
        if constexpr (RES) y += float(res[size_t(m) * N + n0 + r]);
        out[size_t(m) * N + n0 + r] = T(y);
    }
}

bool use_split2(int M, int NTILES) { return ceil_div(M, 64) * ceil_div(NTILES, 2) >= 128; }

bool use_staged(const PwArgs& a, bool exact_f32) {
    return a.staged && !exact_f32 && (a.K >= 1152 || (a.K >= 672 && a.HW >= 196));
}

struct PwChoice {
    int kind;
    int NT, NCH;
};

PwChoice choose_pw(const PwArgs& a, int num_cus) {
    const int cus = num_cus > 0 ? num_cus : 256;
    if (a.K >= 320) return PwChoice{1, 1, a.NTILES};
    const int MT = ceil_div(a.M, 128);
    const int nt_cap = (a.K * 4 <= a.N) ? 3 : 6;
    int NT = 1;
    for (int cand = (a.NTILES < nt_cap ? a.NTILES : nt_cap); cand >= 1; --cand) {
        const int nch = ceil_div(a.NTILES, cand);
        if (MT * nch >= 2 * cus || cand == 1) {
            NT = ceil_div(a.NTILES, nch);
            break;
        }
    }
    return PwChoice{2, NT, ceil_div(a.NTILES, NT)};
}

template <typename T, int B2, int GM, bool RES, int ACT, bool SP>
void launch_splitk(const PwArgs& a, hipStream_t stream) {
    const int MT = ceil_div(a.M, 32 * B2), NCH = ceil_div(a.NTILES, B2);
    if (GM == 3 || use_staged(a, IsF32<T>::value && !SP)) {
        hipLaunchKernelGGL((whenet_pw_splitk_staged_kernel<T, B2, GM, RES, ACT, SP>), dim3(8 * ceil_div(MT, 8) * NCH), dim3(256), 0,
                           stream, static_cast<const T*>(a.a), static_cast<const T*>(SP ? a.wps : a.wp), a.bias,
                           static_cast<const T*>(a.gate), static_cast<const T*>(a.res), static_cast<T*>(a.out), a.M, a.K,
                           a.N, SP ? a.KSs : a.KS, a.NTILES, a.HW, MT, NCH, a.se, a.wsi);
        return;
    }
    if constexpr (GM != 3)
        hipLaunchKernelGGL((whenet_pw_splitk_kernel<T, B2, GM, RES, ACT, SP>), dim3(8 * ceil_div(MT, 8) * NCH), dim3(256), 0,
                           stream, static_cast<const T*>(a.a), static_cast<const T*>(SP ? a.wps : a.wp), a.bias,
                           static_cast<const T*>(a.gate), static_cast<const T*>(a.res), static_cast<T*>(a.out), a.M, a.K,
                           a.N, SP ? a.KSs : a.KS, a.NTILES, a.HW, MT, NCH, a.se, a.wsi);
}

template <typename T, int NT, int GM, bool RES, int ACT, bool SP>
void launch_tile(const PwArgs& a, int MT, int NCH, hipStream_t stream) {
    const int blocks = 8 * ceil_div(MT, 8) * NCH;
    hipLaunchKernelGGL((whenet_pw_tile_kernel<T, NT, GM, RES, ACT, SP>), dim3(blocks), dim3(256), 0, stream,
                       static_cast<const T*>(a.a), static_cast<const T*>(SP ? a.wps : a.wp), a.bias, static_cast<const T*>(a.gate),
                       static_cast<const T*>(a.res), static_cast<T*>(a.out), a.M, a.K, a.N, SP ? a.KSs : a.KS, a.NTILES, a.HW, MT,
                       NCH, a.se, a.wsi);
}

template <typename T, int GM, bool RES, int ACT, bool SP = false>
void launch_variant(const PwArgs& a, int impl, int num_cus, hipStream_t stream) {
    if (impl == 1) {
        WHENET_REQUIRE(GM != 2, WHENET_EINVAL, "pointwise: the check kernel takes the gate from global memory (se_fuse=0)");
        const size_t work = size_t(a.M) * (a.N / 4);
        hipLaunchKernelGGL((whenet_pw_check_kernel<T, GM != 0, RES, ACT>), dim3(unsigned((work + 255) / 256)), dim3(256),
                           0, stream, static_cast<const T*>(a.a), a.wdense, a.bias, static_cast<const T*>(a.gate),
                           static_cast<const T*>(a.res), static_cast<T*>(a.out), a.M, a.K, a.N, a.HW);
        return;
    }
    const PwChoice ch = choose_pw(a, num_cus);
    if (ch.kind == 1) {
        WHENET_REQUIRE(a.K % (2 * PwOps<T, SP>::V) == 0, WHENET_EINVAL, "pointwise: a deep contraction is a whole number of k-steps");
        if (use_split2(a.M, a.NTILES)) launch_splitk<T, 2, GM, RES, ACT, SP>(a, stream);
        else launch_splitk<T, 1, GM, RES, ACT, SP>(a, stream);
        return;
    }
    const int MT = ceil_div(a.M, 128);
    switch (ch.NT) {
        case 1: launch_tile<T, 1, GM, RES, ACT, SP>(a, MT, ch.NCH, stream); break;
        case 2: launch_tile<T, 2, GM, RES, ACT, SP>(a, MT, ch.NCH, stream); break;
        case 3: launch_tile<T, 3, GM, RES, ACT, SP>(a, MT, ch.NCH, stream); break;
        case 4: launch_tile<T, 4, GM, RES, ACT, SP>(a, MT, ch.NCH, stream); break;
        case 5: launch_tile<T, 5, GM, RES, ACT, SP>(a, MT, ch.NCH, stream); break;
        default: launch_tile<T, 6, GM, RES, ACT, SP>(a, MT, ch.NCH, stream); break;
    }
}

template <typename T, bool SP = false>
void launch_dtype(const PwArgs& a, int impl, int num_cus, hipStream_t stream) {
    const bool res = a.res != nullptr;
    const int gm = a.se.rpart != nullptr ? (a.se.w2p != nullptr ? 3 : 2) : (a.gate != nullptr ? 1 : 0);
    if (gm == 0 && !res && a.act == ACT_SWISH) launch_variant<T, 0, false, ACT_SWISH, SP>(a, impl, num_cus, stream);
    else if (gm == 1 && !res && a.act == ACT_NONE) launch_variant<T, 1, false, ACT_NONE, SP>(a, impl, num_cus, stream);
    else if (gm == 1 && res && a.act == ACT_NONE) launch_variant<T, 1, true, ACT_NONE, SP>(a, impl, num_cus, stream);
    else if (gm == 2 && !res && a.act == ACT_NONE) launch_variant<T, 2, false, ACT_NONE, SP>(a, impl, num_cus, stream);
    else if (gm == 2 && res && a.act == ACT_NONE) launch_variant<T, 2, true, ACT_NONE, SP>(a, impl, num_cus, stream);
    else if (gm == 3 && a.act == ACT_NONE) {
        WHENET_REQUIRE(impl == 0 && a.K >= 320 && a.K % 32 == 0 && (sizeof(T) == 2 || SP) && a.se.KSr >= 1 && a.se.KSr <= 3 &&
                           a.se.RP <= 48, WHENET_EINVAL, "pointwise: the matrix-core squeeze-excite form is outside its limits");
        if constexpr (sizeof(T) == 2 || SP) {
            if (res) {
                if (use_split2(a.M, a.NTILES)) launch_splitk<T, 2, 3, true, ACT_NONE, SP>(a, stream);
                else launch_splitk<T, 1, 3, true, ACT_NONE, SP>(a, stream);
            } else {
                if (use_split2(a.M, a.NTILES)) launch_splitk<T, 2, 3, false, ACT_NONE, SP>(a, stream);
                else launch_splitk<T, 1, 3, false, ACT_NONE, SP>(a, stream);
            }
        }
    }
    else throw Error(WHENET_EINVAL, "pointwise: unsupported epilogue combination");
}

}

void launch_pw(const PwArgs& a, int dtype, int impl, int num_cus, hipStream_t stream) {
    WHENET_REQUIRE(a.N % 4 == 0 && a.M > 0, WHENET_EINVAL, "pointwise: bad shape");
    const bool gated = a.gate != nullptr || a.se.rpart != nullptr;
    WHENET_REQUIRE(!(a.gate != nullptr && a.se.rpart != nullptr), WHENET_EINVAL, "pointwise: gate AND fused squeeze-excite");
    WHENET_REQUIRE(!gated || a.K < 320 || (a.K <= 1152 && a.K % 16 == 0 && a.HW >= 49), WHENET_EINVAL,
                   "pointwise: gated deep contraction outside the staged-gate limits (K <= 1152, K % 16 == 0, HW >= 49)");
    WHENET_REQUIRE(!gated || a.K >= 320 || (a.K <= 256 && a.HW >= 196), WHENET_EINVAL,
                   "pointwise: gated shallow contraction outside the staged-gate limits (K <= 256, HW >= 196)");
    WHENET_REQUIRE(a.se.rpart == nullptr || (a.se.RP % 4 == 0 && a.se.RP <= 48 && a.se.np >= 1 &&
                                             (a.K >= 320 || (a.K <= 256 && a.HW >= 196 && a.se.RP <= 12))),
                   WHENET_EINVAL, "pointwise: fused squeeze-excite outside its limits");
    const bool split = a.split && impl == 0;
    WHENET_REQUIRE(!a.split || (dtype == WHENET_F32 && a.wps != nullptr && a.KSs == ceil_div(a.K, 16)), WHENET_EINVAL,
                   "pointwise: the split-product form needs float32 storage and the split weight images");
    if (dtype == WHENET_F16) launch_dtype<half_t>(a, impl, num_cus, stream);
    else if (split) launch_dtype<float, true>(a, impl, num_cus, stream);
    else launch_dtype<float>(a, impl, num_cus, stream);
    WHENET_HIP_CHECK(hipGetLastError());
}

std::string kernel_name_pw(const PwArgs& a, int dtype, int impl, int num_cus) {
    const char* t = dtype == WHENET_F16 ? "_Float16" : "float";
    const char* gate = a.se.rpart ? (a.se.w2p ? "3" : "2") : (a.gate ? "1" : "0");
    const char* res = a.res ? "true" : "false";
    char buf[96];
    if (impl == 1) {
        std::snprintf(buf, sizeof(buf), "whenet_pw_check_kernel<%s, %s, %s, %d>", t, a.gate ? "true" : "false", res, a.act);
    } else {
        const PwChoice ch = choose_pw(a, num_cus);
        if (ch.kind == 1) {
            const int b2 = use_split2(a.M, a.NTILES) ? 2 : 1;
            const bool st = (a.se.rpart && a.se.w2p) || use_staged(a, dtype == WHENET_F32 && !a.split);
            std::snprintf(buf, sizeof(buf), "whenet_pw_splitk%s_kernel<%s, %d, %s, %s, %d%s>", st ? "_staged" : "", t, b2, gate, res, a.act,
                          a.split ? ", true" : (st ? ", false" : ""));
        }
        else std::snprintf(buf, sizeof(buf), "whenet_pw_tile_kernel<%s, %d, %s, %s, %d%s>", t, ch.NT, gate, res, a.act, a.split ? ", true" : "");
    }
    return buf;
}

}
```

Before: 161,500.

## Add 16-channel blocked activation layout between project and 7x7 front/head kernels

Introduces an optional channel-blocked (16-channel groups per crop) activation layout for f16 in the 7x7 stage. The split-K pointwise project kernel can now write its output and read its skip in this layout, and the front7 and head7 kernels can read it directly, which lets front7 skip its LDS staging path. The layout is on by default for blocks 12-16. The aim is more contiguous input loads for the consumer kernels; the cost is extra index arithmetic in the pointwise epilogue and scattered stores there.

```diff
diff --git a/headposeestimation-whenet_amd/csrc/capi.cpp b/headposeestimation-whenet_amd/csrc/capi.cpp
--- a/headposeestimation-whenet_amd/csrc/capi.cpp
+++ b/headposeestimation-whenet_amd/csrc/capi.cpp
@@ -282,7 +282,7 @@
                 h->fanout_chunk = int(value);
             } else if (k == "fanout_stage") {
                 WHENET_REQUIRE(value >= -1 && value <= 3, WHENET_EINVAL,
-                               "fanout_stage must be -1 (calibrate 0 against 1), 0 (pinned staging), 1 (the runtime's pageable path) or 2 (registered, default)");
+                               "fanout_stage must be -1 (calibrate 0 against 1), 0 (pinned staging), 1 (the runtime's pageable path), 2 (registered, default) or 3 (probe: registered, a copy stream per engine)");
                 h->fanout_stage = int(value);
                 h->fanout_calib_calls = 0;
                 h->fanout_calib_rate[0] = h->fanout_calib_rate[1] = 0.0;
diff --git a/headposeestimation-whenet_amd/csrc/engine.cpp b/headposeestimation-whenet_amd/csrc/engine.cpp
--- a/headposeestimation-whenet_amd/csrc/engine.cpp
+++ b/headposeestimation-whenet_amd/csrc/engine.cpp
@@ -213,7 +213,7 @@
         drop_graphs();
     } else if (key == "se_fuse") {
         WHENET_REQUIRE(value >= 0 && value <= 3, WHENET_EINVAL,
-                       "se_fuse must be 0 (never), 1 (where the prologue form pays), 2 (prologue form on every block) or 3 (1 + the matrix-core form on blocks 7-16, default)");
+                       "se_fuse must be 0 (never), 1 (where the prologue form pays, default), 2 (prologue form on every block) or 3 (1 + the matrix-core form on blocks 7-16)");
         se_fuse_ = int(value);
         sync();
         drop_graphs();
@@ -255,6 +255,12 @@
         drop_graphs();
     } else if (key == "stem_fuse") {
         stem_fuse_ = value != 0;
+        sync();
+        drop_graphs();
+    } else if (key == "act_layout") {
+        WHENET_REQUIRE(value >= 0 && value <= 2, WHENET_EINVAL,
+                       "act_layout must be 0 (NHWC everywhere), 1 (16-channel blocks per layer, default) or 2 (16-channel blocks wherever supported)");
+        act_layout_ = int(value);
         sync();
         drop_graphs();
     } else if (key == "poison") {
@@ -456,19 +462,43 @@
            stemdw_supported(dtype_, b.dw.plan, b.spec.k, b.spec.s, b.spec.h_in, b.spec.cexp());
 }
 
+bool Engine::head_fused() const {
+    return head_fuse_ && pw_impl_ == 0 && split_heads_ && head7_supported(dtype_, head_.K, head_.N, 49) &&
+           partial_per_crop_ >= size_t(heads_split()) * N_LOGITS;
+}
+
+bool Engine::act_blocked(int index) const {
+    if (act_layout_ == 0 || dtype_ != WHENET_F16 || pw_impl_ != 0 || single_stage_call_) return false;
+    if (index < 1 || index > int(blocks_.size())) return false;
+    const DevBlock& b = blocks_[size_t(index - 1)];
+    if (block_schedule(b).use_mb7 || b.project.K < 320 || b.spec.cout % 16 != 0) return false;
+    if (index == int(blocks_.size())) {
+        if (!head_fused()) return false;
+    } else {
+        const DevBlock& c = blocks_[size_t(index)];
+        const BlockSchedule cs = block_schedule(c);
+        if (cs.use_mb7 || !cs.use_f7) return false;
+        if (c.spec.has_skip() && c.project.K < 320) return false;
+    }
+    static constexpr bool WINS[17] = {false, false, false, false, false, false, false, false, false, false, false, false,
+                                      true, true, true, true, true};
+    return act_layout_ == 2 || (index <= 16 && WINS[index]);
+}
+
 void* Engine::enqueue_blocks(int first, int last, const View& v, void* cur, int n, hipStream_t s, LaunchRecorder* rec,
                              bool b1_dw_done) {
     const bool fold = fold12_active() && first <= 1 && last >= 2;
     for (int i = first; i <= last; ++i) {
         void* nxt = (cur == v.x0) ? v.x1 : v.x0;
-        enqueue_block(blocks_[size_t(i - 1)], v, cur, nxt, n, s, rec, fold && i <= 2 ? i : 0, b1_dw_done && i == 1);
+        enqueue_block(blocks_[size_t(i - 1)], v, cur, nxt, n, s, rec, fold && i <= 2 ? i : 0, b1_dw_done && i == 1,
+                      i > first && act_blocked(i - 1), i < last || last == int(blocks_.size()) ? act_blocked(i) : false);
         cur = nxt;
     }
     return cur;
 }
 
 void Engine::enqueue_block(const DevBlock& b, const View& v, const void* in, void* out, int n, hipStream_t s,
-                           LaunchRecorder* rec, int fold, bool dw_done) {
+                           LaunchRecorder* rec, int fold, bool dw_done, bool in_blocked, bool out_blocked) {
     Rec R{rec, s, repeat_};
     const BlockSpec& sp = b.spec;
     const std::string p = "b" + std::to_string(sp.index);
@@ -482,6 +512,8 @@
     WHENET_REQUIRE(fold == 0 || (fold == 1 && !fused && sp.index == 1) ||
                        (fold == 2 && sp.index == 2 && (use_f2 || (split_ && fused && !bs.use_f2s && !bs.use_f7))), WHENET_EINVAL,
                    "fold12: block outside the folded pair");
+    WHENET_REQUIRE(!(in_blocked || out_blocked) || (dtype_ == WHENET_F16 && !bs.use_mb7 && (!in_blocked || bs.use_f7)),
+                   WHENET_EINVAL, "act_layout: a kernel of this block does not know the blocked layout");
     if (bs.use_mb7) {
         WHENET_REQUIRE(fold == 0, WHENET_EINVAL, "mb7: block outside the 7 x 7 stage");
         Mb7Args a{};
@@ -532,6 +564,7 @@
         a.wsi = b.expand.wsi;
         a.n = n;
         a.xcd_grouped = xcd_grouped(2, n);
+        a.x_blocked = in_blocked;
         a.plan = front7_plan_for(dtype_, sp.cin, cexp, n);
         R(p + "/front", "front", kernel_name_front7(dtype_, sp.k, a.plan, a.split).c_str(), double(n) * (hw_in * sp.cin + hw_out * cexp) * es,
           2.0 * n * (double(hw_in) * sp.cin * cexp + double(hw_out) * sp.k * sp.k * cexp), [&] { launch_front7(a, s); });
@@ -742,6 +775,8 @@
         set_split(a, b.project);
         a.HW = hw_out;
         a.act = ACT_NONE;
+        a.out_blocked = out_blocked;
+        a.res_blocked = in_blocked && sp.has_skip();
         R(p + "/project", "pw", kernel_name_pw(a, dtype_, pw_impl_, num_cus_).c_str(),
           double(a.M) * (a.K + a.N + (sp.has_skip() ? a.N : 0)) * es, 2.0 * a.M * a.K * a.N,
           [&] { launch_pw(a, dtype_, pw_impl_, num_cus_, s); });
@@ -777,8 +812,7 @@
           [&] { launch_stem(a, dtype_, s); });
     }
     void* cur = enqueue_blocks(1, int(blocks_.size()), v, v.x0, n, s, rec, stemdw);
-    const bool fuse_head = head_fuse_ && pw_impl_ == 0 && split_heads_ && head7_supported(dtype_, head_.K, head_.N, 49) &&
-                           partial_per_crop_ >= size_t(heads_split()) * N_LOGITS;
+    const bool fuse_head = head_fused();
     if (fuse_head) {
         Head7Args a{};
         a.dtype = dtype_;
@@ -794,6 +828,7 @@
         a.wsi = head_.wsi;
         a.n = n;
         a.xcd_grouped = xcd_grouped(4, n);
+        a.x_blocked = act_blocked(int(blocks_.size()));
         R("head", "pw", kernel_name_head7(dtype_, n, a.split).c_str(), double(n) * (49.0 * a.K * es + a.N * 4.0), 2.0 * n * 49.0 * a.K * a.N,
           [&] { launch_head7(a, s); });
         HeadsArgs hargs{};
diff --git a/headposeestimation-whenet_amd/csrc/engine.h b/headposeestimation-whenet_amd/csrc/engine.h
--- a/headposeestimation-whenet_amd/csrc/engine.h
+++ b/headposeestimation-whenet_amd/csrc/engine.h
@@ -167,11 +167,14 @@
     void enqueue_forward(const View& v, const uint8_t* d_in, int n, float* d_ypr, int32_t* d_amax, float* d_logits,
                          hipStream_t s, LaunchRecorder* rec, const float* d_in_f32 = nullptr);
     void enqueue_block(const DevBlock& b, const View& v, const void* in, void* out, int n, hipStream_t s,
-                       LaunchRecorder* rec, int fold = 0, bool dw_done = false);
+                       LaunchRecorder* rec, int fold = 0, bool dw_done = false, bool in_blocked = false, bool out_blocked = false);
     void* enqueue_blocks(int first, int last, const View& v, void* cur, int n, hipStream_t s, LaunchRecorder* rec,
                          bool b1_dw_done = false);
     bool stem_fuse_active() const;
     bool fold12_active() const;
+    bool head_fused() const;
+    bool act_blocked(int index) const;
+    int act_layout_ = 1;
     struct BlockSchedule {
         bool fused = false, use_f2 = false, use_f2s = false, use_f7 = false, se_in_front = false, se_fused = false, se_mfma = false;
         bool use_mb7 = false;
diff --git a/headposeestimation-whenet_amd/csrc/front7.hip b/headposeestimation-whenet_amd/csrc/front7.hip
--- a/headposeestimation-whenet_amd/csrc/front7.hip
+++ b/headposeestimation-whenet_amd/csrc/front7.hip
@@ -25,6 +25,7 @@
     int off_w, off_stage, off_red, off_sum;
     float wsi;
     int chunks, ngroups, xcd;
+    int xblk;
 };
 
 template <int K, int KS, int G, int CC, int NTHR>
@@ -66,6 +67,7 @@
             }
         }
     }
+    const bool xblk = p.xblk != 0;
     auto a_offset = [&](int strip) -> unsigned {
         int R = strip * 4 + (lm >> 3);
         R = R < nrow ? R : nrow - 1;
@@ -75,16 +77,28 @@
         gc = gc < nlast ? gc : nlast;
         int px = lm & 7;
         px = px < 7 ? px : 6;
+        if (xblk) return unsigned(gc * 49 * Cin + (row * 7 + px) * 16 + g * 8) * 2u;
         return unsigned((gc * 49 + row * 7 + px) * Cin + g * 8) * 2u;
     };
     const unsigned char* xb = reinterpret_cast<const unsigned char*>(p.x);
     half8 a[KS];
+    auto load_rows = [&](unsigned off) {
+        if (xblk) {
+#pragma unroll
+            for (int ks = 0; ks < KS; ++ks) a[ks] = *reinterpret_cast<const half8*>(xb + off + ks * (49 * 32));
+        } else {
+#pragma unroll
+            for (int ks = 0; ks < KS; ++ks) a[ks] = *reinterpret_cast<const half8*>(xb + off + ks * 32);
+        }
+    };
     constexpr bool SPLIT = nstrip * NT <= NWAVE;
     int strip = SPLIT ? (wave < nstrip * NT ? wave % nstrip : nstrip) : wave;
     const int t_lo = SPLIT ? wave / nstrip : 0, t_hi = SPLIT ? t_lo + 1 : NT;
     constexpr bool STG = !SPLIT && nstrip <= NWAVE && nstrip * 4032 <= (G + 3) / 4 * NCB * ROWS * 64 * 16 && KS % 4 == 0;
+    bool direct = true;
+    if constexpr (STG) direct = xblk;
     if (strip < nstrip) {
-        if constexpr (STG) {
+        if constexpr (STG) if (!direct) {
             constexpr int PX = 28, SEG = KS / 4;
             constexpr int rowb = KS * 32;
             unsigned char* sa = E + wave * 4032;
@@ -114,11 +128,8 @@
 #pragma unroll
                 for (int u = 0; u < 4; ++u) a[t * 4 + u] = *reinterpret_cast<const half8*>(sa + pf * 144 + u * 32 + g * 16);
             }
-        } else {
-            const unsigned off = a_offset(strip);
-#pragma unroll
-            for (int ks = 0; ks < KS; ++ks) a[ks] = *reinterpret_cast<const half8*>(xb + off + ks * 32);
-        }
+        }
+        if (direct) load_rows(a_offset(strip));
     }
     float bias_t[NT];
 #pragma unroll
@@ -165,9 +176,7 @@
             }
         }
         if (more) {
-            const unsigned off = a_offset(strip + NWAVE);
-#pragma unroll
-            for (int ks = 0; ks < KS; ++ks) a[ks] = *reinterpret_cast<const half8*>(xb + off + ks * 32);
+            load_rows(a_offset(strip + NWAVE));
         }
     }
     STAMP(2);
@@ -631,6 +640,7 @@
         attr.done[dev].store(true, std::memory_order_release);
     }
     p.chunks = pl.chunks;  p.ngroups = ceil_div(a.n, pl.G);  p.xcd = a.xcd_grouped ? 1 : 0;
+    p.xblk = a.x_blocked ? 1 : 0;
     hipLaunchKernelGGL(kern, dim3(unsigned(p.chunks) * unsigned(p.ngroups)), dim3(NTHR), pl.lds_bytes, stream, p);
     WHENET_HIP_CHECK(hipGetLastError());
 }
@@ -668,6 +678,7 @@
 void launch_front7(const Front7Args& a, hipStream_t stream) {
     WHENET_REQUIRE(front7_supported(a.k, 1, HW7, a.Cin) && a.w1t != nullptr && a.R >= 1 && a.R <= 64 && a.n >= 1, WHENET_EINVAL,
                    "front7: 7 x 7 maps, 3x3 / 5x5 stride-1 kernels, Cin = 192, squeeze-excite reduce conv in the kernel");
+    WHENET_REQUIRE(!a.x_blocked || a.dtype == WHENET_F16, WHENET_EINVAL, "front7: the blocked input layout exists for binary16 only");
     const int key = ((a.k * 10 + a.plan.G) * 1000 + a.plan.CC) * 1000 + a.plan.threads;
     if (a.dtype == WHENET_F32) {
         switch (key) {
diff --git a/headposeestimation-whenet_amd/csrc/head7.hip b/headposeestimation-whenet_amd/csrc/head7.hip
--- a/headposeestimation-whenet_amd/csrc/head7.hip
+++ b/headposeestimation-whenet_amd/csrc/head7.hip
@@ -13,7 +13,7 @@
 template <int G, int NTHR>
 __global__ __launch_bounds__(NTHR) void whenet_head7_kernel(const half_t* __restrict__ x, const half_t* __restrict__ wep,
                                                             const float* __restrict__ bias, float* __restrict__ feat, int n,
-                                                            int NTILES, int N, int xcd) {
+                                                            int NTILES, int N, int xcd, int xblk) {
     constexpr int NWAVE = NTHR / 64;
     constexpr int nstrip = 2 * G;
     constexpr int KS = H7_KS, NT = H7_NT, NC = H7_NC;
@@ -54,9 +54,15 @@
         gc = gc < nlast ? gc : nlast;
         int px = (strip & 1) * 32 + lm;
         px = px < H7_HW ? px : H7_HW - 1;
-        const unsigned char* xr = reinterpret_cast<const unsigned char*>(x) + (size_t(gc) * H7_HW + px) * (H7_K * 2) + g * 16;
-#pragma unroll
-        for (int ks = 0; ks < KS; ++ks) a[ks] = *reinterpret_cast<const half8*>(xr + ks * 32);
+        if (xblk) {
+            const unsigned char* xr = reinterpret_cast<const unsigned char*>(x) + size_t(gc) * (H7_HW * H7_K * 2) + px * 32 + g * 16;
+#pragma unroll
+            for (int ks = 0; ks < KS; ++ks) a[ks] = *reinterpret_cast<const half8*>(xr + ks * (H7_HW * 32));
+        } else {
+            const unsigned char* xr = reinterpret_cast<const unsigned char*>(x) + (size_t(gc) * H7_HW + px) * (H7_K * 2) + g * 16;
+#pragma unroll
+            for (int ks = 0; ks < KS; ++ks) a[ks] = *reinterpret_cast<const half8*>(xr + ks * 32);
+        }
     }
     float bias_t[NT];
 #pragma unroll
@@ -235,7 +241,7 @@
     constexpr int NTHR = 512;
     const size_t lds = size_t(H7_KS) * H7_NT * 1024 + size_t(2 * G) * 2 * H7_NC * 4;
     hipLaunchKernelGGL((whenet_head7_kernel<G, NTHR>), dim3(unsigned(a.N / H7_NC) * unsigned(ceil_div(a.n, G))), dim3(NTHR), lds, stream,
-                       static_cast<const half_t*>(a.x), static_cast<const half_t*>(a.wep), a.bias, a.feat, a.n, a.NTILES, a.N, a.xcd_grouped ? 1 : 0);
+                       static_cast<const half_t*>(a.x), static_cast<const half_t*>(a.wep), a.bias, a.feat, a.n, a.NTILES, a.N, a.xcd_grouped ? 1 : 0, a.x_blocked ? 1 : 0);
     WHENET_HIP_CHECK(hipGetLastError());
 }
 
@@ -248,6 +254,7 @@
 void launch_head7(const Head7Args& a, hipStream_t stream) {
     WHENET_REQUIRE(head7_supported(a.dtype, a.K, a.N, 49) && a.n >= 1 && a.x && a.wep && a.bias && a.feat, WHENET_EINVAL,
                    "head7: the 320 -> N (multiple of 64) head conv on 7 x 7 maps");
+    WHENET_REQUIRE(!a.x_blocked || a.dtype == WHENET_F16, WHENET_EINVAL, "head7: the blocked input layout exists for binary16 only");
     if (a.dtype == WHENET_F16) {
         if (a.n <= 16) launch_h7<2>(a, stream);
         else launch_h7<4>(a, stream);
diff --git a/headposeestimation-whenet_amd/csrc/kernels.h b/headposeestimation-whenet_amd/csrc/kernels.h
--- a/headposeestimation-whenet_amd/csrc/kernels.h
+++ b/headposeestimation-whenet_amd/csrc/kernels.h
@@ -96,6 +96,7 @@
     int KSs = 0;
     float wsi = 1.0f;
     bool staged = true;
+    bool out_blocked = false, res_blocked = false;
 };
 void launch_pw(const PwArgs& a, int dtype, int impl, int num_cus, hipStream_t stream);
 
@@ -126,6 +127,7 @@
     const void* weps = nullptr;
     float wsi = 1.0f;
     bool xcd_grouped = false;
+    bool x_blocked = false;
 };
 bool head7_supported(int dtype, int K, int N, int HW);
 void launch_head7(const Head7Args& a, hipStream_t stream);
@@ -282,6 +284,7 @@
     const void* weps = nullptr;
     float wsi = 1.0f;
     bool xcd_grouped = false;
+    bool x_blocked = false;
 };
 void launch_front7(const Front7Args& a, hipStream_t stream);
 std::string kernel_name_front7(int dtype, int k, const Front7Plan& p, bool split = false);
diff --git a/headposeestimation-whenet_amd/csrc/pw.hip b/headposeestimation-whenet_amd/csrc/pw.hip
--- a/headposeestimation-whenet_amd/csrc/pw.hip
+++ b/headposeestimation-whenet_amd/csrc/pw.hip
@@ -14,7 +14,7 @@
 template <typename T, int B2, bool RES, int ACT, bool SP>
 __device__ __forceinline__ void splitk_combine_store(float16v (&acc)[B2][B2], float* s_red, int kpart, int lane, int mt, int nt0, int M,
                                                      int N, int NTILES, const float* __restrict__ bias, const T* __restrict__ res,
-                                                     T* __restrict__ out, float wsi) {
+                                                     T* __restrict__ out, float wsi, int HW, int lay) {
     using OT = T __attribute__((ext_vector_type(4)));
     constexpr int MB = B2, NT = B2;
     constexpr int NACC = MB * NT * 16, SL = NACC / 4;
@@ -23,6 +23,19 @@
     const int own_tile = f0 >> 4, own_mb = own_tile / NT, own_t = own_tile % NT;
     const int own_row = (mt * MB + own_mb) * 32 + (lane & 31);
     const bool own_valid = own_row < M && nt0 + own_t < NTILES;
+    const size_t row_base = size_t(own_row) * N;
+    size_t blk_base = row_base;
+    if (lay != 0) {
+        int crop = int(float(own_row) * __builtin_amdgcn_rcpf(float(HW)));
+        int pix = own_row - crop * HW;
+        if (pix < 0) { --crop; pix += HW; }
+        if (pix >= HW) { ++crop; pix -= HW; }
+        blk_base = size_t(crop) * size_t(N) * HW + size_t(pix) * 16;
+    }
+    const bool out_blk = (lay & 1) != 0, res_blk = (lay & 2) != 0;
+    const size_t out_base = out_blk ? blk_base : row_base, res_base = res_blk ? blk_base : row_base;
+    const unsigned out_s16 = out_blk ? unsigned(HW) * 16u : 16u, res_s16 = res_blk ? unsigned(HW) * 16u : 16u;
+    auto elem_off = [&](size_t base, unsigned s16, int n0) -> size_t { return base + size_t(unsigned(n0 >> 4) * s16 + unsigned(n0 & 15)); };
     OT rv[SL / 4];
     float4v bv[SL / 4];
 #pragma unroll
@@ -31,7 +44,7 @@
         const int n0 = (nt0 + own_t) * 32 + 8 * qq + 4 * g;
         const bool ok = own_valid && n0 < N;
         bv[i4] = ok ? *reinterpret_cast<const float4v*>(bias + n0) : float4v{0.f, 0.f, 0.f, 0.f};
-        if constexpr (RES) rv[i4] = ok ? *reinterpret_cast<const OT*>(res + size_t(own_row) * N + n0) : OT{};
+        if constexpr (RES) rv[i4] = ok ? *reinterpret_cast<const OT*>(res + elem_off(res_base, res_s16, n0)) : OT{};
     }
     float own[SL];
 #pragma unroll
@@ -82,7 +95,7 @@
             if constexpr (RES) y += float(rv[i4][r]);
             o[r] = T(y);
         }
-        *reinterpret_cast<OT*>(out + size_t(own_row) * N + n0) = o;
+        *reinterpret_cast<OT*>(out + elem_off(out_base, out_s16, n0)) = o;
     }
     STAMP(4);
 }
@@ -91,7 +104,7 @@
 __global__ __launch_bounds__(256, B2 == 2 ? 2 : 3) void whenet_pw_splitk_kernel(
     const T* __restrict__ A, const T* __restrict__ Wp, const float* __restrict__ bias, const T* __restrict__ gate,
     const T* __restrict__ res, T* __restrict__ out, int M, int K, int N, int KS, int NTILES, int HW, int MT, int NCH,
-    const SeFuse se, float wsi) {
+    const SeFuse se, float wsi, int lay) {
     constexpr bool GATE = GM != 0;
     using OPS = PwOps<T, SP>;
     constexpr int V = OPS::V;
@@ -210,14 +223,14 @@
     }
     STAMP(2);
 
-    splitk_combine_store<T, B2, RES, ACT, SP>(acc, s_red, kpart, lane, mt, nt0, M, N, NTILES, bias, res, out, wsi);
+    splitk_combine_store<T, B2, RES, ACT, SP>(acc, s_red, kpart, lane, mt, nt0, M, N, NTILES, bias, res, out, wsi, HW, lay);
 }
 
 template <typename T, int B2, int GM, bool RES, int ACT, bool SP = false>
 __global__ __launch_bounds__(256, B2 == 2 ? 2 : 3) void whenet_pw_splitk_staged_kernel(
     const T* __restrict__ A, const T* __restrict__ Wp, const float* __restrict__ bias, const T* __restrict__ gate,
     const T* __restrict__ res, T* __restrict__ out, int M, int K, int N, int KS, int NTILES, int HW, int MT, int NCH,
-    const SeFuse se, float wsi) {
+    const SeFuse se, float wsi, int lay) {
     constexpr bool GATE = GM != 0;
     using OPS = PwOps<T, SP>;
     constexpr int V = OPS::V;
@@ -462,7 +475,7 @@
         }
     }
     lds_barrier();
-    splitk_combine_store<T, B2, RES, ACT, SP>(acc, s_red, kpart, lane, mt, nt0, M, N, NTILES, bias, res, out, wsi);
+    splitk_combine_store<T, B2, RES, ACT, SP>(acc, s_red, kpart, lane, mt, nt0, M, N, NTILES, bias, res, out, wsi, HW, lay);
 }
 
 template <typename T, int NT, int GM, bool RES, int ACT, bool SP = false>
@@ -742,18 +755,19 @@
 template <typename T, int B2, int GM, bool RES, int ACT, bool SP>
 void launch_splitk(const PwArgs& a, hipStream_t stream) {
     const int MT = ceil_div(a.M, 32 * B2), NCH = ceil_div(a.NTILES, B2);
+    const int lay = (a.out_blocked ? 1 : 0) | (a.res_blocked ? 2 : 0);
     if (GM == 3 || use_staged(a, IsF32<T>::value && !SP)) {
         hipLaunchKernelGGL((whenet_pw_splitk_staged_kernel<T, B2, GM, RES, ACT, SP>), dim3(8 * ceil_div(MT, 8) * NCH), dim3(256), 0,
                            stream, static_cast<const T*>(a.a), static_cast<const T*>(SP ? a.wps : a.wp), a.bias,
                            static_cast<const T*>(a.gate), static_cast<const T*>(a.res), static_cast<T*>(a.out), a.M, a.K,
-                           a.N, SP ? a.KSs : a.KS, a.NTILES, a.HW, MT, NCH, a.se, a.wsi);
+                           a.N, SP ? a.KSs : a.KS, a.NTILES, a.HW, MT, NCH, a.se, a.wsi, lay);
         return;
     }
     if constexpr (GM != 3)
         hipLaunchKernelGGL((whenet_pw_splitk_kernel<T, B2, GM, RES, ACT, SP>), dim3(8 * ceil_div(MT, 8) * NCH), dim3(256), 0,
                            stream, static_cast<const T*>(a.a), static_cast<const T*>(SP ? a.wps : a.wp), a.bias,
                            static_cast<const T*>(a.gate), static_cast<const T*>(a.res), static_cast<T*>(a.out), a.M, a.K,
-                           a.N, SP ? a.KSs : a.KS, a.NTILES, a.HW, MT, NCH, a.se, a.wsi);
+                           a.N, SP ? a.KSs : a.KS, a.NTILES, a.HW, MT, NCH, a.se, a.wsi, lay);
 }
 
 template <typename T, int NT, int GM, bool RES, int ACT, bool SP>
@@ -831,6 +845,10 @@
     WHENET_REQUIRE(a.se.rpart == nullptr || (a.se.RP % 4 == 0 && a.se.RP <= 48 && a.se.np >= 1 &&
                                              (a.K >= 320 || (a.K <= 256 && a.HW >= 196 && a.se.RP <= 12))),
                    WHENET_EINVAL, "pointwise: fused squeeze-excite outside its limits");
+    WHENET_REQUIRE(!(a.out_blocked || a.res_blocked) ||
+                       (dtype == WHENET_F16 && impl == 0 && a.K >= 320 && a.N % 16 == 0 && a.HW >= 1 && a.M % a.HW == 0 &&
+                        (!a.res_blocked || a.res != nullptr)),
+                   WHENET_EINVAL, "pointwise: blocked output / skip outside the binary16 split-K kernels (K >= 320, N % 16 == 0)");
     const bool split = a.split && impl == 0;
     WHENET_REQUIRE(!a.split || (dtype == WHENET_F32 && a.wps != nullptr && a.KSs == ceil_div(a.K, 16)), WHENET_EINVAL,
                    "pointwise: the split-product form needs float32 storage and the split weight images");
```

After: 163,300 (median of 6 runs). +1.1%, better.
